# neevparikh/rpt

Hardware: AMD Instinct MI355X
Metric: Msamples/sec (higher is better)
Workload: dtype f32; 1 GPU; C3 lampshade-in-fog path trace 1024x1024x256spp; scene=examples/volumetric_pathtrace_lampshade.rs, parallelism=tile-shard x1, streams=2

## Files before the change

### include/rpt_hip.h

```cpp
#ifndef RPT_HIP_H
#define RPT_HIP_H

#include <stdint.h>

#ifdef __cplusplus
extern "C" {
#endif

#define RPT_OK 0
#define RPT_ERR_INVALID (-1)
#define RPT_ERR_STATE (-2)
#define RPT_ERR_DEVICE (-3)
#define RPT_ERR_UNSUPPORTED (-4)

typedef struct rpt_scene rpt_scene;

enum { RPT_SHAPE_SPHERE = 0, RPT_SHAPE_CUBE = 1, RPT_SHAPE_PLANE = 2, RPT_SHAPE_MESH = 3,
       RPT_SHAPE_GROUP = 4,
       RPT_SHAPE_MONOMIAL = 5  };

typedef struct rpt_shape_desc {
    int32_t kind;
    int32_t has_transform;
    double transform[16];
// ... 59 lines not shown
                            int32_t* object, double* normal);

int rpt_scene_stats(rpt_scene*, uint64_t out[16]);
int rpt_get_counters(rpt_scene*, uint64_t out[8]);
int rpt_debug_section_counters(rpt_scene*, uint64_t out[56]);
int rpt_scan_cull_counters(rpt_scene*, uint64_t out[16]);
int rpt_scan_cull_groups(rpt_scene*, float out_boxes[36], uint64_t out_masks[5], uint32_t* n_groups, uint32_t* enabled);
int rpt_get_timing(rpt_scene*, double* render_ms, double* resolve_ms, int32_t* grid_blocks);
int rpt_get_timing_mean(rpt_scene*, double* render_ms, double* resolve_ms, int32_t* launches);
int rpt_render_chunking(uint32_t iterations, uint32_t* chunk_spp, uint32_t* n_chunks);
int rpt_scene_render_chunking(rpt_scene*, uint32_t iterations, uint32_t* chunk_spp, uint32_t* n_chunks);
int rpt_set_option(const char* name, int64_t value);
int rpt_scene_set_option(rpt_scene*, const char* name, int64_t value);

typedef struct rpt_buffer rpt_buffer;
rpt_buffer* rpt_buffer_create(int device, uint32_t width, uint32_t height, uint32_t filter_radius);
void rpt_buffer_destroy(rpt_buffer*);
int rpt_buffer_add_samples(rpt_buffer*, const double* rgb );
int rpt_buffer_add_samples_device(rpt_buffer*, const void* d_rgb, void* hip_stream);
int rpt_buffer_image(rpt_buffer*, uint8_t* out_rgb8 );
int rpt_buffer_variance(rpt_buffer*, double* out);
int rpt_buffer_batches(rpt_buffer*, uint32_t* n);
int rpt_render_into_buffer(rpt_scene*, const rpt_camera*, const rpt_render_params*, uint32_t iterations,
                           uint64_t seed, uint32_t sample_offset, rpt_buffer*);

enum { RPT_PHOTON_MAP = 0, RPT_PHOTON_POINT_BEAM = 1, RPT_PHOTON_BEAM_BEAM = 2 };
int rpt_photon_map_build(rpt_scene*, uint64_t photon_count, int32_t kind, double watts, uint64_t seed);
#define RPT_PHOTON_RECORD_BYTES 48
int rpt_photon_shoot(rpt_scene*, uint64_t photon_count, int32_t kind, double watts, uint64_t seed,
                     uint32_t shard_rank, uint32_t shard_count, uint64_t n_out[2]);
int rpt_photon_records(rpt_scene*, int32_t which , void** d_records, uint64_t* n);
int rpt_photon_map_from_records(rpt_scene*, uint64_t photon_count, int32_t kind, const void* d_surface,
                                uint64_t n_surface, const void* d_volume, uint64_t n_volume);
int rpt_photon_map_stats(rpt_scene*, uint64_t out[8]);
int rpt_photon_map_download(rpt_scene*, int32_t which, float* out, uint64_t capacity_photons);
int rpt_photon_render_sample(rpt_scene*, const rpt_camera*, const rpt_render_params*, uint64_t gather_size,
                             uint64_t gather_size_volume, uint32_t num_samples, uint64_t seed,
                             uint32_t sample_offset, double* out_rgb);
int rpt_photon_render_sample_device(rpt_scene*, const rpt_camera*, const rpt_render_params*, uint64_t gather_size,
                                    uint64_t gather_size_volume, uint32_t num_samples, uint64_t seed,
                                    uint32_t sample_offset, void* d_out_rgb, void* hip_stream);

typedef struct rpt_comm rpt_comm;
#define RPT_COMM_ID_BYTES 128
int rpt_comm_unique_id(void* id_out);
int rpt_comm_create(const void* id, int rank, int n_ranks, int device, rpt_comm** out);
void rpt_comm_destroy(rpt_comm*);
int rpt_comm_rank(const rpt_comm*, int* rank, int* n_ranks);
#define RPT_GATHER_LOOPBACK 1u
int rpt_gather_frame_device(rpt_comm*, uint32_t width, uint32_t height, const void* d_shard, void* d_frame,
                            uint32_t flags, void* hip_stream);
int rpt_allgather_records_device(rpt_comm*, const void* d_local, uint64_t n_local, void* d_out, uint64_t capacity,
                                 uint64_t* n_per_rank, uint64_t* n_total, void* hip_stream);
int rpt_frame_pack_layout(uint32_t width, uint32_t height, uint32_t n_ranks, uint64_t* tile_offsets);
int rpt_frame_pack_device(uint32_t width, uint32_t height, uint32_t rank, uint32_t n_ranks, const void* d_frame,
                          void* d_packed, void* hip_stream);
int rpt_frame_unpack_device(uint32_t width, uint32_t height, uint32_t rank, uint32_t n_ranks, const void* d_packed,
                            void* d_frame, void* hip_stream);

int rpt_debug_epsilon_counters(rpt_scene*, uint64_t out[12]);

int rpt_debug_rng_u32(uint64_t seed, uint32_t pixel, uint32_t sample, uint32_t n, uint32_t* out);
int rpt_debug_material_sample_f(const rpt_material*, uint64_t n, const float* normals, const float* wos,
                                uint64_t seed, float* wi, float* pdf, int32_t* some);
int rpt_debug_material_bsdf(const rpt_material*, uint64_t n, const float* normals, const float* wos,
                            const float* wis, float* out_rgb);
int rpt_debug_radix_sort(uint64_t n, const uint64_t* keys, uint64_t* keys_out, uint32_t* order_out);
int rpt_debug_exclusive_scan2(uint64_t n, const uint32_t* a, const uint32_t* b, uint32_t* out_a, uint32_t* out_b, uint64_t totals[2]);
int rpt_debug_photon_positions64(rpt_scene*, double* out, uint64_t capacity);
int rpt_debug_photon_selections(rpt_scene*, uint32_t* out, uint64_t capacity_words, uint64_t dims[3]);
int rpt_debug_camera_rays(const rpt_camera*, const rpt_render_params*, uint64_t seed, uint32_t sample,
                          float* origins, float* dirs);
int rpt_debug_camera_sample(const rpt_camera*, const rpt_render_params*, uint64_t seed, uint32_t sample,
                            float* origins, float* dirs, uint32_t* next_word);
int rpt_debug_camera_sample_f64(const rpt_camera*, const rpt_render_params*, uint64_t seed, uint32_t sample,
                                double* origins, double* dirs, uint32_t* next_word);
int rpt_debug_light_sample(rpt_scene*, uint32_t light, uint64_t n, const float* positions, uint64_t seed, float* v, float* nrm,
                           float* pdf, float* intensity, float* wi, float* dist, uint32_t* next_word);
int rpt_debug_light_sample_f64(rpt_scene*, uint32_t light, uint64_t n, const double* positions, uint64_t seed, double* v, double* nrm,
                               double* pdf, double* intensity, double* wi, double* dist, uint32_t* next_word);
int rpt_debug_env_color(rpt_scene*, uint64_t n, const float* dirs, float* rgb);
int rpt_debug_env_color_f64(rpt_scene*, uint64_t n, const double* dirs, double* rgb);
int rpt_debug_medium_distance(rpt_scene*, uint64_t n, uint64_t seed, float* dmed, float* t_limit);

int rpt_debug_bounce(const rpt_material* m, uint32_t max_bounces, uint32_t depth, int32_t in_medium, int32_t medium_event,
                     float albedo_med, const float* medium_color, uint64_t n, const float* normals, const float* rds, uint64_t seed,
                     int32_t* flag, float* wi, float* k, uint32_t* next_word);
int rpt_debug_material_f64(const rpt_material* m, uint64_t n, const double* normals, const double* wos, uint64_t seed, int32_t* some,
                           double* wi, double* pdf, double* f, uint32_t* next_word);
int rpt_debug_material_bsdf_f64(const rpt_material* m, uint64_t n, const double* normals, const double* wos, const double* wis,
                                double* f);
#ifdef __cplusplus
}
#endif
#endif
```

### rpt_amd/_lib.py

```python
import ctypes as C
import os
import sys

_HERE = os.path.dirname(os.path.abspath(__file__))
LIB_PATH = os.environ.get("RPT_LIB", os.path.join(_HERE, "librpt_hip.so"))


class RptError(RuntimeError):
    """Raised for every non-zero return code of the C ABI (message from rpt_last_error)."""


class ShapeDesc(C.Structure):
    pass


ShapeDesc._fields_ = [
    ("kind", C.c_int32),
    ("has_transform", C.c_int32),
    ("transform", C.c_double * 16),
    ("plane_normal", C.c_double * 3),
    ("plane_value", C.c_double),
    ("tris", C.POINTER(C.c_double)),
    ("n_tris", C.c_uint64),
    ("children", C.POINTER(ShapeDesc)),
# ... 40 lines not shown
    ("rpt_device_count", C.c_int, []),
    ("rpt_last_error", C.c_char_p, []),
    ("rpt_shard_tiles", C.c_int64, [C.c_uint32, C.c_uint32, C.c_uint32, C.c_uint32, _P, C.c_uint64]),
    ("rpt_scene_create", _P, []),
    ("rpt_scene_destroy", None, [_P]),
    ("rpt_scene_add_object", C.c_int, [_P, C.POINTER(ShapeDesc), C.POINTER(MaterialDesc)]),
    ("rpt_scene_add_light_point", C.c_int, [_P, _D3, _D3]),
    ("rpt_scene_add_light_ambient", C.c_int, [_P, _D3]),
    ("rpt_scene_add_light_directional", C.c_int, [_P, _D3, _D3]),
    ("rpt_scene_add_light_object", C.c_int, [_P, C.POINTER(ShapeDesc), C.POINTER(MaterialDesc)]),
    ("rpt_scene_add_medium", C.c_int, [_P, C.c_int32, C.c_double, C.c_double]),
    ("rpt_scene_set_environment_color", C.c_int, [_P, _D3]),
    ("rpt_scene_set_environment_hdri", C.c_int, [_P, C.c_uint32, C.c_uint32, _D3]),
    ("rpt_scene_commit", C.c_int, [_P, C.c_int]),
    ("rpt_render_sample", C.c_int,
     [_P, C.POINTER(CameraDesc), C.POINTER(RenderParams), C.c_uint32, C.c_uint64, C.c_uint32, _P]),
    ("rpt_render_sample_device", C.c_int,
     [_P, C.POINTER(CameraDesc), C.POINTER(RenderParams), C.c_uint32, C.c_uint64, C.c_uint32, _P, _P]),
    ("rpt_intersect_batch", C.c_int, [_P, C.c_uint64, _P, _P, _P, _P, _P]),
    ("rpt_intersect_batch_f64", C.c_int, [_P, C.c_uint64, _P, _P, _P, _P, _P]),
    ("rpt_intersect_segments", C.c_int, [_P, C.c_uint64, _P, _P, _P, _P, _P]),
    ("rpt_scan_cull_counters", C.c_int, [_P, C.POINTER(C.c_uint64)]),
    ("rpt_scan_cull_groups", C.c_int, [_P, C.POINTER(C.c_float), C.POINTER(C.c_uint64), C.POINTER(C.c_uint32), C.POINTER(C.c_uint32)]),
    ("rpt_scene_stats", C.c_int, [_P, C.POINTER(C.c_uint64)]),
    ("rpt_get_counters", C.c_int, [_P, C.POINTER(C.c_uint64)]),
    ("rpt_debug_section_counters", C.c_int, [_P, C.POINTER(C.c_uint64)]),
    ("rpt_get_timing", C.c_int, [_P, C.POINTER(C.c_double), C.POINTER(C.c_double), C.POINTER(C.c_int32)]),
    ("rpt_get_timing_mean", C.c_int, [_P, C.POINTER(C.c_double), C.POINTER(C.c_double), C.POINTER(C.c_int32)]),
    ("rpt_render_chunking", C.c_int, [C.c_uint32, C.POINTER(C.c_uint32), C.POINTER(C.c_uint32)]),
    ("rpt_scene_render_chunking", C.c_int, [_P, C.c_uint32, C.POINTER(C.c_uint32), C.POINTER(C.c_uint32)]),
    ("rpt_set_option", C.c_int, [C.c_char_p, C.c_int64]),
    ("rpt_scene_set_option", C.c_int, [_P, C.c_char_p, C.c_int64]),
    ("rpt_buffer_create", _P, [C.c_int, C.c_uint32, C.c_uint32, C.c_uint32]),
    ("rpt_buffer_destroy", None, [_P]),
    ("rpt_buffer_add_samples", C.c_int, [_P, _P]),
    ("rpt_buffer_add_samples_device", C.c_int, [_P, _P, _P]),
    ("rpt_buffer_image", C.c_int, [_P, _P]),
    ("rpt_buffer_variance", C.c_int, [_P, C.POINTER(C.c_double)]),
    ("rpt_buffer_batches", C.c_int, [_P, C.POINTER(C.c_uint32)]),
    ("rpt_render_into_buffer", C.c_int,
     [_P, C.POINTER(CameraDesc), C.POINTER(RenderParams), C.c_uint32, C.c_uint64, C.c_uint32, _P]),
    ("rpt_photon_map_build", C.c_int, [_P, C.c_uint64, C.c_int32, C.c_double, C.c_uint64]),
    ("rpt_photon_shoot", C.c_int,
     [_P, C.c_uint64, C.c_int32, C.c_double, C.c_uint64, C.c_uint32, C.c_uint32, C.POINTER(C.c_uint64)]),
    ("rpt_photon_records", C.c_int, [_P, C.c_int32, C.POINTER(C.c_void_p), C.POINTER(C.c_uint64)]),
    ("rpt_photon_map_from_records", C.c_int, [_P, C.c_uint64, C.c_int32, _P, C.c_uint64, _P, C.c_uint64]),
    ("rpt_photon_map_stats", C.c_int, [_P, C.POINTER(C.c_uint64)]),
    ("rpt_photon_map_download", C.c_int, [_P, C.c_int32, _P, C.c_uint64]),
    ("rpt_photon_render_sample", C.c_int,
     [_P, C.POINTER(CameraDesc), C.POINTER(RenderParams), C.c_uint64, C.c_uint64, C.c_uint32, C.c_uint64, C.c_uint32, _P]),
    ("rpt_photon_render_sample_device", C.c_int,
     [_P, C.POINTER(CameraDesc), C.POINTER(RenderParams), C.c_uint64, C.c_uint64, C.c_uint32, C.c_uint64, C.c_uint32, _P, _P]),
    ("rpt_comm_unique_id", C.c_int, [_P]),
    ("rpt_comm_create", C.c_int, [_P, C.c_int, C.c_int, C.c_int, C.POINTER(C.c_void_p)]),
    ("rpt_comm_destroy", None, [_P]),
    ("rpt_comm_rank", C.c_int, [_P, C.POINTER(C.c_int), C.POINTER(C.c_int)]),
    ("rpt_gather_frame_device", C.c_int, [_P, C.c_uint32, C.c_uint32, _P, _P, C.c_uint32, _P]),
    ("rpt_allgather_records_device", C.c_int, [_P, _P, C.c_uint64, _P, C.c_uint64, C.POINTER(C.c_uint64), C.POINTER(C.c_uint64), _P]),
    ("rpt_frame_pack_layout", C.c_int, [C.c_uint32, C.c_uint32, C.c_uint32, C.POINTER(C.c_uint64)]),
    ("rpt_frame_pack_device", C.c_int, [C.c_uint32, C.c_uint32, C.c_uint32, C.c_uint32, _P, _P, _P]),
    ("rpt_frame_unpack_device", C.c_int, [C.c_uint32, C.c_uint32, C.c_uint32, C.c_uint32, _P, _P, _P]),
    ("rpt_debug_epsilon_counters", C.c_int, [_P, C.POINTER(C.c_uint64)]),
    ("rpt_debug_rng_u32", C.c_int, [C.c_uint64, C.c_uint32, C.c_uint32, C.c_uint32, _P]),
    ("rpt_debug_material_sample_f", C.c_int,
     [C.POINTER(MaterialDesc), C.c_uint64, _P, _P, C.c_uint64, _P, _P, _P]),
    ("rpt_debug_material_bsdf", C.c_int, [C.POINTER(MaterialDesc), C.c_uint64, _P, _P, _P, _P]),
    ("rpt_debug_radix_sort", C.c_int, [C.c_uint64, _P, _P, _P]),
    ("rpt_debug_exclusive_scan2", C.c_int, [C.c_uint64, _P, _P, _P, _P, C.POINTER(C.c_uint64)]),
    ("rpt_debug_photon_positions64", C.c_int, [_P, _P, C.c_uint64]),
    ("rpt_debug_photon_selections", C.c_int, [_P, _P, C.c_uint64, C.POINTER(C.c_uint64)]),
    ("rpt_debug_camera_rays", C.c_int,
     [C.POINTER(CameraDesc), C.POINTER(RenderParams), C.c_uint64, C.c_uint32, _P, _P]),
    ("rpt_debug_light_sample", C.c_int, [_P, C.c_uint32, C.c_uint64, _P, C.c_uint64, _P, _P, _P, _P, _P, _P, _P]),
    ("rpt_debug_light_sample_f64", C.c_int, [_P, C.c_uint32, C.c_uint64, _P, C.c_uint64, _P, _P, _P, _P, _P, _P, _P]),
    ("rpt_debug_env_color", C.c_int, [_P, C.c_uint64, _P, _P]),
    ("rpt_debug_env_color_f64", C.c_int, [_P, C.c_uint64, _P, _P]),
    ("rpt_debug_medium_distance", C.c_int, [_P, C.c_uint64, C.c_uint64, _P, _P]),
    ("rpt_debug_camera_sample", C.c_int,
     [C.POINTER(CameraDesc), C.POINTER(RenderParams), C.c_uint64, C.c_uint32, _P, _P, _P]),
    ("rpt_debug_camera_sample_f64", C.c_int,
     [C.POINTER(CameraDesc), C.POINTER(RenderParams), C.c_uint64, C.c_uint32, _P, _P, _P]),
    ("rpt_debug_bounce", C.c_int, [C.POINTER(MaterialDesc), C.c_uint32, C.c_uint32, C.c_int32, C.c_int32, C.c_float, _P,
                                   C.c_uint64, _P, _P, C.c_uint64, _P, _P, _P, _P]),
    ("rpt_debug_material_f64", C.c_int, [C.POINTER(MaterialDesc), C.c_uint64, _P, _P, C.c_uint64, _P, _P, _P, _P, _P]),
    ("rpt_debug_material_bsdf_f64", C.c_int, [C.POINTER(MaterialDesc), C.c_uint64, _P, _P, _P, _P]),
]

_lib = None


def vp(a):
    return a.ctypes.data_as(C.c_void_p)


def load():
    global _lib
    if _lib is not None:
        return _lib
    if not os.path.exists(LIB_PATH):
        raise RptError(
            f"{LIB_PATH} is missing: build it with `python -c 'import __graft_entry__ as g; g.build()'` "
            "(hipcc --offload-arch=gfx950).  There is no CPU fallback.")
    if "torch" not in sys.modules and os.environ.get("RPT_IMPORT_TORCH", "0") == "1":
        import torch
    lib = C.CDLL(LIB_PATH, mode=C.RTLD_GLOBAL)
    for name, res, args in SYMBOLS:
        fn = getattr(lib, name)
        fn.restype = res
        fn.argtypes = args
    _lib = lib
    return lib


def check(rc):
    if rc < 0:
        msg = load().rpt_last_error()
        raise RptError(f"rpt error {rc}: {msg.decode() if msg else ''}")
    return rc
```

### rpt_amd/api.py

```python
import ctypes as C
import math
import weakref

import numpy as np

from . import _lib
from ._lib import RptError, vp as _vp

def shard_pixels(width, height, rank, count):
    lib = _lib.load()
    n = _lib.check(lib.rpt_shard_tiles(width, height, rank, count, None, 0))
    tiles = np.zeros(max(n, 1), dtype=np.uint32)
    _lib.check(lib.rpt_shard_tiles(width, height, rank, count, tiles.ctypes.data_as(C.c_void_p), n))
    tiles_x = (width + 31) // 32
    ys, xs = np.mgrid[0:32, 0:32]
    out = []
    for t in tiles[:n]:
        x = (int(t) % tiles_x) * 32 + xs
        y = (int(t) // tiles_x) * 32 + ys
        m = (x < width) & (y < height)
        out.append((y[m] * width + x[m]).astype(np.uint32))
    return np.sort(np.concatenate(out)) if out else np.zeros(0, dtype=np.uint32)


# ... 808 lines not shown
            self.gather_size_volume_, int(num_samples), C.c_uint64(self.seed_), self._sample_offset,
            C.c_void_p(d_out_ptr), C.c_void_p(stream_ptr)))
        self._sample_offset += int(num_samples)

    def photon_render(self, photon_count, kind):
        self.photon_map_build(photon_count, kind)
        buffer = Buffer(self.width_, self.height_, self.filter_)
        self._sample_offset = 0
        buffer.add_samples(self.photon_sample_array(self.num_samples_))
        return buffer.image()

    def photon_point_query_beam_render(self, photon_count):
        return self.photon_render(photon_count, Renderer.PHOTON_POINT_BEAM)

    def photon_beam_query_beam_render(self, photon_count):
        return self.photon_render(photon_count, Renderer.PHOTON_BEAM_BEAM)

    def photon_map_render(self, photon_count):
        return self.photon_render(photon_count, Renderer.PHOTON_MAP)

    def counters(self):
        out = (C.c_uint64 * 8)()
        _lib.check(_lib.load().rpt_get_counters(self.scene._handle, out))
        names = ["samples", "rays", "vertices", "wave_trips", "prim_tests", "bvh_nodes", "bvh_tris", "stack_overflows"]
        return dict(zip(names, [int(v) for v in out]))

    def get_closest_hit(self, origins, dirs):
        lib = _lib.load()
        h = self.scene._commit(self.device_)
        o = np.ascontiguousarray(origins, dtype=np.float32).reshape(-1, 3)
        d = np.ascontiguousarray(dirs, dtype=np.float32).reshape(-1, 3)
        n = o.shape[0]
        t = np.empty(n, dtype=np.float32)
        obj = np.empty(n, dtype=np.int32)
        nrm = np.empty((n, 3), dtype=np.float32)
        _lib.check(lib.rpt_intersect_batch(h, n, o.ctypes.data_as(C.c_void_p), d.ctypes.data_as(C.c_void_p),
                                           t.ctypes.data_as(C.c_void_p), obj.ctypes.data_as(C.c_void_p),
                                           nrm.ctypes.data_as(C.c_void_p)))
        return t, obj, nrm

    def get_closest_hit_f64(self, origins, dirs):
        lib = _lib.load()
        h = self.scene._commit(self.device_)
        o = np.ascontiguousarray(origins, dtype=np.float64).reshape(-1, 3)
        d = np.ascontiguousarray(dirs, dtype=np.float64).reshape(-1, 3)
        n = o.shape[0]
        t = np.empty(n, dtype=np.float64)
        obj = np.empty(n, dtype=np.int32)
        nrm = np.empty((n, 3), dtype=np.float64)
        _lib.check(lib.rpt_intersect_batch_f64(h, n, o.ctypes.data_as(C.c_void_p), d.ctypes.data_as(C.c_void_p),
                                               t.ctypes.data_as(C.c_void_p), obj.ctypes.data_as(C.c_void_p),
                                               nrm.ctypes.data_as(C.c_void_p)))
        return t, obj, nrm

    def debug_light_sample(self, light_index, positions, seed=0, f64=False):
        lib = _lib.load()
        h = self.scene._commit(self.device_)
        ft = np.float64 if f64 else np.float32
        pos = np.ascontiguousarray(positions, dtype=ft).reshape(-1, 3)
        n = pos.shape[0]
        out = {"v": np.empty((n, 3), ft), "nrm": np.empty((n, 3), ft), "p": np.empty(n, ft), "intensity": np.empty((n, 3), ft),
               "wi": np.empty((n, 3), ft), "dist": np.empty(n, ft), "next_word": np.empty(n, np.uint32)}
        fn = lib.rpt_debug_light_sample_f64 if f64 else lib.rpt_debug_light_sample
        _lib.check(fn(h, light_index, n, pos.ctypes.data_as(C.c_void_p), seed,
                      *[out[k].ctypes.data_as(C.c_void_p) for k in ("v", "nrm", "p", "intensity", "wi", "dist", "next_word")]))
        return out

    def debug_env_color(self, dirs, f64=False):
        lib = _lib.load()
        h = self.scene._commit(self.device_)
        d = np.ascontiguousarray(dirs, dtype=np.float64 if f64 else np.float32).reshape(-1, 3)
        out = np.empty_like(d)
        fn = lib.rpt_debug_env_color_f64 if f64 else lib.rpt_debug_env_color
        _lib.check(fn(h, d.shape[0], d.ctypes.data_as(C.c_void_p), out.ctypes.data_as(C.c_void_p)))
        return out

    def debug_medium_distance(self, n, seed=0):
        lib = _lib.load()
        h = self.scene._commit(self.device_)
        dmed, lim = np.empty(n, np.float32), np.empty(n, np.float32)
        _lib.check(lib.rpt_debug_medium_distance(h, n, seed, dmed.ctypes.data_as(C.c_void_p), lim.ctypes.data_as(C.c_void_p)))
        return dmed, lim


def debug_bounce(material, normals, rds, max_bounces=3, depth=0, seed=0, in_medium=False, medium_event=False, albedo_med=0.0,
                 medium_color=(0.0, 0.0, 0.0)):
    nrm = np.ascontiguousarray(normals, dtype=np.float32).reshape(-1, 3)
    rd = np.ascontiguousarray(rds, dtype=np.float32).reshape(-1, 3)
    n = nrm.shape[0]
    if rd.shape[0] != n:
        raise ValueError("normals and rds differ in length")
    mcol = np.ascontiguousarray(medium_color, dtype=np.float32).reshape(3)
    out = {"flag": np.empty(n, np.int32), "wi": np.empty((n, 3), np.float32), "k": np.empty((n, 3), np.float32),
           "next_word": np.empty(n, np.uint32)}
    md = material_desc(material, _lib.MaterialDesc)
    _lib.check(_lib.load().rpt_debug_bounce(C.byref(md), max_bounces, depth, int(bool(in_medium)), int(bool(medium_event)),
                                            float(albedo_med), _vp(mcol), n, _vp(nrm), _vp(rd), seed,
                                            *[_vp(out[k]) for k in ("flag", "wi", "k", "next_word")]))
    return out


def debug_material_f64(material, normals, wos, seed=0):
    nrm = np.ascontiguousarray(normals, dtype=np.float64).reshape(-1, 3)
    wo = np.ascontiguousarray(wos, dtype=np.float64).reshape(-1, 3)
    n = nrm.shape[0]
    if wo.shape[0] != n:
        raise ValueError("normals and wos differ in length")
    out = {"some": np.empty(n, np.int32), "wi": np.empty((n, 3)), "pdf": np.empty(n), "f": np.empty((n, 3)),
           "next_word": np.empty(n, np.uint32)}
    md = material_desc(material, _lib.MaterialDesc)
    _lib.check(_lib.load().rpt_debug_material_f64(C.byref(md), n, _vp(nrm), _vp(wo), seed,
                                                  *[_vp(out[k]) for k in ("some", "wi", "pdf", "f", "next_word")]))
    return out


def debug_material_bsdf_f64(material, normals, wos, wis):
    arrs = [np.ascontiguousarray(a, dtype=np.float64).reshape(-1, 3) for a in (normals, wos, wis)]
    n = arrs[0].shape[0]
    if any(a.shape[0] != n for a in arrs):
        raise ValueError("normals, wos and wis differ in length")
    f = np.empty((n, 3))
    md = material_desc(material, _lib.MaterialDesc)
    _lib.check(_lib.load().rpt_debug_material_bsdf_f64(C.byref(md), n, *[_vp(a) for a in arrs], _vp(f)))
    return f


def debug_camera_sample(camera, width, height, sample=0, seed=0, f64=False):
    ft = np.float64 if f64 else np.float32
    n = width * height
    out = {"o": np.empty((n, 3), ft), "d": np.empty((n, 3), ft), "next_word": np.empty(n, np.uint32)}
    prm = _lib.RenderParams(width, height, 0.0, 0, 0, 1)
    lib = _lib.load()
    fn = lib.rpt_debug_camera_sample_f64 if f64 else lib.rpt_debug_camera_sample
    _lib.check(fn(C.byref(camera_desc(camera, _lib.CameraDesc)), C.byref(prm), seed, sample,
                  *[_vp(out[k]) for k in ("o", "d", "next_word")]))
    return out
```

### rpt_amd/csrc/device_core.h

```cpp
#pragma once
#include <hip/hip_runtime.h>
#include "gpu_layout.h"

namespace rptg {

#define RPT_DEV __device__ __forceinline__

static constexpr float kPi = 3.14159265358979323846f;
static constexpr float kInvPi = 0.31830988618379067154f;
static constexpr float kInf = __builtin_huge_valf();

struct V {
    float x, y, z;
};
RPT_DEV V mk(float x, float y, float z) { return V{x, y, z}; }
RPT_DEV V operator+(V a, V b) { return V{a.x + b.x, a.y + b.y, a.z + b.z}; }
RPT_DEV V operator-(V a, V b) { return V{a.x - b.x, a.y - b.y, a.z - b.z}; }
RPT_DEV V operator-(V a) { return V{-a.x, -a.y, -a.z}; }
RPT_DEV V operator*(float s, V a) { return V{s * a.x, s * a.y, s * a.z}; }
RPT_DEV V operator*(V a, float s) { return V{s * a.x, s * a.y, s * a.z}; }
RPT_DEV V operator*(V a, V b) { return V{a.x * b.x, a.y * b.y, a.z * b.z}; }
RPT_DEV float dot(V a, V b) { return fmaf(a.x, b.x, fmaf(a.y, b.y, a.z * b.z)); }
RPT_DEV V cross(V a, V b) {
    return V{a.y * b.z - a.z * b.y, a.z * b.x - a.x * b.z, a.x * b.y - a.y * b.x};
}
RPT_DEV V fma3(float s, V a, V b) { return V{fmaf(s, a.x, b.x), fmaf(s, a.y, b.y), fmaf(s, a.z, b.z)}; }
RPT_DEV V fma3(V s, V a, V b) { return V{fmaf(s.x, a.x, b.x), fmaf(s.y, a.y, b.y), fmaf(s.z, a.z, b.z)}; }
RPT_DEV float rsq(float x) { return __builtin_amdgcn_rsqf(x); }
RPT_DEV float rcp(float x) { return __builtin_amdgcn_rcpf(x); }
RPT_DEV float sqrt1(float x) { return __builtin_amdgcn_sqrtf(x); }
RPT_DEV V normalize(V a) { return rsq(dot(a, a)) * a; }
RPT_DEV V vmin(V a, V b) { return V{fminf(a.x, b.x), fminf(a.y, b.y), fminf(a.z, b.z)}; }
RPT_DEV float max3(float a, float b, float c) { return fmaxf(fmaxf(a, b), c); }
RPT_DEV float min3(float a, float b, float c) { return fminf(fminf(a, b), c); }
RPT_DEV V xyz(const F4& f) { return V{f.x, f.y, f.z}; }
RPT_DEV float dot3w(const F4& r, V p) { return fmaf(r.x, p.x, fmaf(r.y, p.y, fmaf(r.z, p.z, r.w))); }
RPT_DEV float dot3(const F4& r, V p) { return fmaf(r.x, p.x, fmaf(r.y, p.y, r.z * p.z)); }
RPT_DEV bool is_zero(V a) { return a.x == 0.f && a.y == 0.f && a.z == 0.f; }

template <class T>
RPT_DEV T uload(const T* p) {
    static_assert(sizeof(T) % 16 == 0, "scene records are 16-byte multiples");
    typedef uint32_t u4v __attribute__((ext_vector_type(4)));
    typedef const __attribute__((address_space(4))) u4v* CP;
    CP q = (CP)(uintptr_t)p;
    u4v raw[sizeof(T) / 16];
#pragma unroll
    for (unsigned i = 0; i < sizeof(T) / 16; i++) raw[i] = q[i];
    T out;
    __builtin_memcpy(&out, raw, sizeof(T));
    return out;
}

typedef const __attribute__((address_space(4))) SceneView* KernargView;
RPT_DEV KernargView kernarg_scene() {
    KernargView kv = (KernargView)__builtin_amdgcn_kernarg_segment_ptr();
    asm volatile("" : "+s"(kv));
    return kv;
}
template <class T>
RPT_DEV T kernarg_load(const __attribute__((address_space(4))) T* p) {
    static_assert(sizeof(T) % 4 == 0, "kernel-argument structs are dword multiples");
    typedef const __attribute__((address_space(4))) uint32_t* Q;
    Q q = (Q)p;
    uint32_t raw[sizeof(T) / 4];
#pragma unroll
    for (unsigned i = 0; i < sizeof(T) / 4; i++) raw[i] = q[i];
    T out;
    __builtin_memcpy(&out, raw, sizeof(T));
    return out;
}
template <class T>
RPT_DEV const __attribute__((address_space(4))) T* kernarg_args() {
    typedef const __attribute__((address_space(4))) T* P;
    P p = (P)__builtin_amdgcn_kernarg_segment_ptr();
    asm volatile("" : "+s"(p));
    return p;
}

RPT_DEV uint64_t mix64(uint64_t x) {
    x ^= x >> 30;
    x *= 0xBF58476D1CE4E5B9ULL;
    x ^= x >> 27;
    x *= 0x94D049BB133111EBULL;
    x ^= x >> 31;
    return x;
}
struct Rng {
    uint32_t s0, s1, s2, s3;
    RPT_DEV void seed(uint64_t a, uint32_t pixel, uint32_t sample) {
        const uint64_t G = 0x9E3779B97F4A7C15ULL;
        uint64_t z = a ^ ((uint64_t(sample) << 32) | uint64_t(pixel));
        uint64_t r0 = mix64(z + G), r1 = mix64(z + 2 * G);
        s0 = uint32_t(r0);
        s1 = uint32_t(r0 >> 32);
        s2 = uint32_t(r1);
        s3 = uint32_t(r1 >> 32);
    }
    RPT_DEV uint32_t next() {
        uint32_t r = s0 + s3;
        uint32_t t = s1 << 9;
        s2 ^= s0;
        s3 ^= s1;
        s1 ^= s2;
        s0 ^= s3;
        s2 ^= t;
        s3 = __builtin_rotateleft32(s3, 11);
        return r;
    }
    RPT_DEV float uniform() { return float(((next() >> 9) << 1) | 1u) * 0x1p-24f; }
    RPT_DEV float range(float a, float b) { return fmaf(b - a, uniform(), a); }
    RPT_DEV uint32_t index(uint32_t n) { return __umulhi(next(), n); }
    RPT_DEV void unit_disc(float& x, float& y) {
        for (;;) {
            x = range(-1.f, 1.f);
            y = range(-1.f, 1.f);
            if (fmaf(x, x, y * y) <= 1.f) return;
        }
    }
};


RPT_DEV bool sphere_closer(V ol, V dl, float tmin, float tbest, float& t);
RPT_DEV float hit_sphere(V ol, V dl, float tmin) {
    float t;
    return sphere_closer(ol, dl, tmin, __builtin_inff(), t) ? t : -1.f;
}
RPT_DEV bool sphere_closer(V ol, V dl, float tmin, float tbest, float& t) {
#pragma clang fp contract(off)
    float a = dot(dl, dl);
    float inv_a = rcp(a);
    float bb = dot(dl, ol) * inv_a;
    V l = fma3(-bb, dl, ol);
    float sq = sqrt1((1.f - dot(l, l)) * inv_a);
    float t0 = -bb - sq;
    t = (t0 < tmin) ? -bb + sq : t0;
    return t >= tmin && t < tbest;
}
RPT_DEV bool slabs_closer(float x1, float x2, float y1, float y2, float z1, float z2, float tmin, float tbest, float& t) {
#pragma clang fp contract(off)
    const float start = max3(fminf(x1, x2), fminf(y1, y2), fminf(z1, z2));
    const float end = min3(fmaxf(x1, x2), fmaxf(y1, y2), fmaxf(z1, z2));
    t = start < tmin ? end : start;
    return !(start > end) && !(end < tmin) && t < tbest;
}
RPT_DEV bool cube_closer(V ol, V dl, float tmin, float tbest, float& t) {
#pragma clang fp contract(off)
    float ix = rcp(dl.x), iy = rcp(dl.y), iz = rcp(dl.z);
    return slabs_closer((-0.5f - ol.x) * ix, (0.5f - ol.x) * ix, (-0.5f - ol.y) * iy, (0.5f - ol.y) * iy, (-0.5f - ol.z) * iz,
                        (0.5f - ol.z) * iz, tmin, tbest, t);
}
RPT_DEV bool aabb_closer(const F4& lo, const F4& hi, V o, V inv, float tmin, float tbest, float& t) {
#pragma clang fp contract(off)
    return slabs_closer((lo.x - o.x) * inv.x, (hi.x - o.x) * inv.x, (lo.y - o.y) * inv.y, (hi.y - o.y) * inv.y,
                        (lo.z - o.z) * inv.z, (hi.z - o.z) * inv.z, tmin, tbest, t);
}
RPT_DEV float hit_cube(V ol, V dl, float tmin) {
    float t;
    return cube_closer(ol, dl, tmin, __builtin_inff(), t) ? t : -1.f;
}
RPT_DEV float hit_plane(const F4& nv, V o, V d, float tmin) {
    float c = dot3(nv, d);
    if (fabsf(c) < 1e-8f) return -1.f;
    float t = (nv.w - dot3(nv, o)) * rcp(c);
    return (t >= tmin) ? t : -1.f;
}
RPT_DEV float hit_tri(const F4& pn, const F4& A, const F4& B, V o, V d, float tmin, float tmax) {
    float c = dot3(pn, d);
    float t = (pn.w - dot3(pn, o)) * rcp(c);
    V p = fma3(t, d, o);
    float v = dot3w(A, p), w = dot3w(B, p);
    float u = 1.f - v - w;
    bool ok = fabsf(c) >= 1e-8f && t >= tmin && t < tmax && u >= 0.f && v >= 0.f && w >= 0.f;
    return ok ? t : -1.f;
}
RPT_DEV float hit_aabb(const F4& lo, const F4& hi, V o, V inv, float tmin) {
    float t;
    return aabb_closer(lo, hi, o, inv, tmin, __builtin_inff(), t) ? t : -1.f;
}
RPT_DEV float hit_rect(const F4& a, float vmax, float oa, float ia, float ou, float du, float ov, float dv,
                       float tmin, float tmax) {
    float t = (a.x - oa) * ia;
    float pu = fmaf(t, du, ou), pv = fmaf(t, dv, ov);
    bool ok = t >= tmin && t < tmax && pu >= a.y && pu <= a.z && pv >= a.w && pv <= vmax;
    return ok ? t : -1.f;
}
RPT_DEV void hit_shell(const ShellScan& s, V o, V inv, float tmin, float& tbest, uint32_t& code) {
    float x1 = (s.lo.x - o.x) * inv.x, x2 = (s.hi.x - o.x) * inv.x;
    float y1 = (s.lo.y - o.y) * inv.y, y2 = (s.hi.y - o.y) * inv.y;
    float z1 = (s.lo.z - o.z) * inv.z, z2 = (s.hi.z - o.z) * inv.z;
    bool sx = x1 > x2, sy = y1 > y2, sz = z1 > z2;
    float xl = sx ? x2 : x1, xh = sx ? x1 : x2;
    float yl = sy ? y2 : y1, yh = sy ? y1 : y2;
    float zl = sz ? z2 : z1, zh = sz ? z1 : z2;
    float start = max3(xl, yl, zl), end = min3(xh, yh, zh);
    uint32_t in_x = sx ? s.face[1] : s.face[0], out_x = sx ? s.face[0] : s.face[1];
    uint32_t in_y = sy ? s.face[3] : s.face[2], out_y = sy ? s.face[2] : s.face[3];
    uint32_t in_z = sz ? s.face[5] : s.face[4], out_z = sz ? s.face[4] : s.face[5];
    uint32_t c_in = (xl > yl && xl > zl) ? in_x : (yl > zl ? in_y : in_z);
    uint32_t c_out = (xh < yh && xh < zh) ? out_x : (yh < zh ? out_y : out_z);
    bool box = start <= end;
    bool use_in = box && start >= tmin && c_in != CODE_MISS;
    bool use_out = box && end >= tmin && c_out != CODE_MISS;
    float t = use_in ? start : end;
    if ((use_in || use_out) && t < tbest) { tbest = t; code = use_in ? c_in : c_out; }
}
RPT_DEV void to_local(const XfScan& x, V o, V d, V& ol, V& dl) {
    ol = mk(dot3w(x.r0, o), dot3w(x.r1, o), dot3w(x.r2, o));
    dl = mk(dot3(x.r0, d), dot3(x.r1, d), dot3(x.r2, d));
}
RPT_DEV void to_local_y(const XfScan& x, V o, V d, V& ol, V& dl) {
    ol = mk(fmaf(x.r0.x, o.x, fmaf(x.r0.z, o.z, x.r0.w)), fmaf(x.r1.y, o.y, x.r1.w), fmaf(x.r2.x, o.x, fmaf(x.r2.z, o.z, x.r2.w)));
    dl = mk(fmaf(x.r0.x, d.x, x.r0.z * d.z), x.r1.y * d.y, fmaf(x.r2.x, d.x, x.r2.z * d.z));
}
RPT_DEV void aabb_pair_closer(const AabbScan& b0, const AabbScan& b1, uint32_t shared, V o, V inv, float tmin, float& tbest,
                              uint32_t& code, uint32_t i) {
#pragma clang fp contract(off)
    const float x1 = (b0.lo.x - o.x) * inv.x, x2 = (b0.hi.x - o.x) * inv.x;
    const float y1 = (b0.lo.y - o.y) * inv.y, y2 = (b0.hi.y - o.y) * inv.y;
    const float z1 = (b0.lo.z - o.z) * inv.z, z2 = (b0.hi.z - o.z) * inv.z;
    float xl = fminf(x1, x2), xh = fmaxf(x1, x2), yl = fminf(y1, y2), yh = fmaxf(y1, y2), zl = fminf(z1, z2), zh = fmaxf(z1, z2);
    float start = max3(xl, yl, zl), end = min3(xh, yh, zh);
    asm volatile("" : "+v"(start), "+v"(end));
    float t = start < tmin ? end : start;
    if (!(start > end) && !(end < tmin) && t < tbest) { tbest = t; code = (K_AABB << 28) | i; }
    if (!(shared & 1u)) { const float u1 = (b1.lo.x - o.x) * inv.x, u2 = (b1.hi.x - o.x) * inv.x; xl = fminf(u1, u2); xh = fmaxf(u1, u2); }
    if (!(shared & 2u)) { const float u1 = (b1.lo.y - o.y) * inv.y, u2 = (b1.hi.y - o.y) * inv.y; yl = fminf(u1, u2); yh = fmaxf(u1, u2); }
    if (!(shared & 4u)) { const float u1 = (b1.lo.z - o.z) * inv.z, u2 = (b1.hi.z - o.z) * inv.z; zl = fminf(u1, u2); zh = fmaxf(u1, u2); }
    start = max3(xl, yl, zl), end = min3(xh, yh, zh);
    t = start < tmin ? end : start;
    if (!(start > end) && !(end < tmin) && t < tbest) { tbest = t; code = (K_AABB << 28) | (i + 1u); }
}
RPT_DEV bool mono_closer(V ol, V dl, const F4& hb, float tmin, float tbest, float& t) {
#pragma clang fp contract(off)
    const float ix = rcp(dl.x), iy = rcp(dl.y), iz = rcp(dl.z);
    const float x1 = (-1.f - ol.x) * ix, x2 = (1.f - ol.x) * ix;
    const float y1 = (hb.y - ol.y) * iy, y2 = (hb.z - ol.y) * iy;
    const float z1 = (-1.f - ol.z) * iz, z2 = (1.f - ol.z) * iz;
    const float b_min = max3(fminf(x1, x2), fminf(y1, y2), fminf(z1, z2));
    const float b_max = min3(fmaxf(x1, x2), fmaxf(y1, y2), fmaxf(z1, z2));
    const bool in_box = !(fmaxf(b_min, tmin) > fminf(b_max, tbest));
    if (__ballot(in_box) == 0ull) return false;
    if (!in_box) return false;
    const float h = hb.x;
    auto dist = [&](float s) {
        const float x = fmaf(s, dl.x, ol.x), y = fmaf(s, dl.y, ol.y), z = fmaf(s, dl.z, ol.z);
        const float r2 = fmaf(x, x, z * z);
        return fmaf(-h, r2 * r2, y);
    };
    const float c0 = fmaf(ol.x, ol.x, ol.z * ol.z), c1 = 2.f * fmaf(ol.x, dl.x, ol.z * dl.z), c2 = fmaf(dl.x, dl.x, dl.z * dl.z);
    const float A = 2.f * c0 * c1, B = 2.f * fmaf(c1, c1, 2.f * c0 * c2), Cq = 6.f * c1 * c2, Dq = 4.f * c2 * c2;
    const float d_tmin = dist(tmin);
    const bool maximize = d_tmin < 0.f;
    float t_max = 10000.f;
    if (maximize) {
        float cur = 0.5f * (b_min + b_max);
        for (int k = 0; k < 10; k++) {
            if (dist(cur) > 0.f) break;
            const float der = fmaf(-h, fmaf(cur, fmaf(cur, fmaf(cur, Dq, Cq), B), A), dl.y);
            const float der2 = -h * fmaf(cur, fmaf(cur, 3.f * Dq, 2.f * Cq), B);
            cur -= der / der2;
        }
        t_max = cur;
        if (t_max < tmin) return false;
    }
    if (maximize == (dist(t_max) < 0.f)) return false;
    float l = tmin, r = t_max;
    for (int k = 0; k < 60; k++) {
        const float m = (l + r) * 0.5f;
        if ((dist(m) >= 0.f) == maximize) r = m;
        else l = m;
    }
    if (r > tbest || !(fabsf(r) < __builtin_huge_valf())) return false;
    const float px = fmaf(r, dl.x, ol.x), pz = fmaf(r, dl.z, ol.z);
    if (fmaf(px, px, pz * pz) > 1.f) return false;
    t = r;
    return true;
}

RPT_DEV void slab2(const float lo[3], const float hi[3], V o, V inv, float& tn, float& tf) {
    float x1 = (lo[0] - o.x) * inv.x, x2 = (hi[0] - o.x) * inv.x;
    float y1 = (lo[1] - o.y) * inv.y, y2 = (hi[1] - o.y) * inv.y;
    float z1 = (lo[2] - o.z) * inv.z, z2 = (hi[2] - o.z) * inv.z;
    tn = max3(fminf(x1, x2), fminf(y1, y2), fminf(z1, z2));
    tf = min3(fmaxf(x1, x2), fmaxf(y1, y2), fmaxf(z1, z2));
}
struct AnyHit {
    float t_block;
    uint32_t tw_lo, tw_hi;
    RPT_DEV bool blocks(float t, uint32_t code) const { return t < t_block && !(code >= tw_lo && code <= tw_hi); }
};
template <bool COUNT, bool PRIMS, bool ANY = false, bool MONO = false>
RPT_DEV void bvh_traverse(const SceneView& sc, uint32_t root, V o, V d, float tmin, float& tbest, uint32_t& code,
                          uint32_t& inst, uint32_t* stk, uint32_t stride, uint32_t cap, uint32_t& c_nodes,
                          uint32_t& c_tris, AnyHit any = AnyHit{-kInf, 1u, 0u});

template <bool COUNT, bool MONO = false>
RPT_DEV void hit_prim(const SceneView& scene_, uint32_t pc, V o, V d, V inv, float tmin, float& tbest, uint32_t& code,
                      uint32_t& inst, uint32_t* stk, uint32_t stride, uint32_t cap, uint32_t& c_nodes,
                      uint32_t& c_tris) {
    const auto& sc = *kernarg_scene();
    const uint32_t kind = pc >> 28, i = pc & 0x0FFFFFFFu;
    float t = -1.f;
    if (MONO && kind == K_MONO) {
        const MonoScan m = sc.mono[i];
        V ol, dl;
        to_local(XfScan{m.r0, m.r1, m.r2}, o, d, ol, dl);
        if (mono_closer(ol, dl, m.h, tmin, tbest, t)) { tbest = t; code = pc; }
        return;
    }
    if (kind == K_INST) {
        const InstRec r = sc.inst[i];
        const V ol = mk(dot3w(r.r0, o), dot3w(r.r1, o), dot3w(r.r2, o));
        const V dl = mk(dot3(r.r0, d), dot3(r.r1, d), dot3(r.r2, d));
// ... 27 lines not shown
        t = hit_tri(tr.pn, tr.A, tr.B, o, d, tmin, tbest);
    }
    if (t >= 0.f && t < tbest) { tbest = t; code = pc; }
}

template <bool COUNT, bool PRIMS, bool ANY, bool MONO>
RPT_DEV void bvh_traverse(const SceneView& scene_, uint32_t root, V o, V d, float tmin, float& tbest, uint32_t& code,
                          uint32_t& inst, uint32_t* stk, uint32_t stride, uint32_t cap, uint32_t& c_nodes,
                          uint32_t& c_tris, AnyHit any) {
    const auto& sc = *kernarg_scene();
    const BvhNode* nodes = sc.nodes;
    const V inv = mk(rcp(d.x), rcp(d.y), rcp(d.z));
    const uint32_t kDone = 0xFFFFFFFFu;
    uint32_t sp = 0;
    uint32_t cur = root;
    while (cur != kDone) {
        while (!(cur & BVH_LEAF)) {
            const BvhNode nd = nodes[cur];
            if (COUNT) c_nodes++;
            float n0, f0, n1, f1;
            slab2(nd.lo0, nd.hi0, o, inv, n0, f0);
            slab2(nd.lo1, nd.hi1, o, inv, n1, f1);
            const bool h0 = fmaxf(n0, tmin) <= fminf(f0, tbest);
            const bool h1 = fmaxf(n1, tmin) <= fminf(f1, tbest);
            if (h0 && h1) {
                const bool first0 = n0 <= n1;
                if (sp < cap) { stk[sp * stride] = first0 ? nd.e1 : nd.e0; sp++; }
                else if (COUNT && sc.stack_overflows) atomicAdd(sc.stack_overflows, 1ull);
                cur = first0 ? nd.e0 : nd.e1;
            } else if (h0 || h1) {
                cur = h0 ? nd.e0 : nd.e1;
            } else if (sp) {
                sp--;
                cur = stk[sp * stride];
            } else {
                cur = kDone;
            }
        }
        if (cur != kDone) {
            const uint32_t first = cur & BVH_INDEX_MASK;
            const uint32_t count = ((cur >> 26) & 31u) + 1u;
            if (PRIMS && (cur & BVH_PRIMS)) {
                for (uint32_t i = 0; i < count; i++) {
                    if (COUNT) c_tris++;
                    hit_prim<COUNT, MONO>(scene_, sc.pleaf[first + i], o, d, inv, tmin, tbest, code, inst, stk + sp * stride, stride,
                                    cap - sp, c_nodes, c_tris);
                }
            } else {
                for (uint32_t i = 0; i < count; i++) {
                    const TriScan tr = sc.btri[first + i];
                    if (COUNT) c_tris++;
                    float t = hit_tri(tr.pn, tr.A, tr.B, o, d, tmin, tbest);
                    if (t >= 0.f) { tbest = t; code = (K_BVHTRI << 28) | (first + i); }
                }
            }
            if (ANY && code != CODE_MISS && any.blocks(tbest, code)) sp = 0;
            if (sp) {
                sp--;
                cur = stk[sp * stride];
            } else {
                cur = kDone;
            }
        }
    }
}

template <bool SHELL>
RPT_DEV bool interval_meets_box(const SceneView::ScanBox& b, V o, V inv, float tmin, float tbest) {
#pragma clang fp contract(off)
    const float x1 = (b.lo[0] - o.x) * inv.x, x2 = (b.hi[0] - o.x) * inv.x;
    const float y1 = (b.lo[1] - o.y) * inv.y, y2 = (b.hi[1] - o.y) * inv.y;
    const float z1 = (b.lo[2] - o.z) * inv.z, z2 = (b.hi[2] - o.z) * inv.z;
    float start, end;
    if (SHELL) {
        const bool sx = x1 > x2, sy = y1 > y2, sz = z1 > z2;
        start = max3(sx ? x2 : x1, sy ? y2 : y1, sz ? z2 : z1);
        end = min3(sx ? x1 : x2, sy ? y1 : y2, sz ? z1 : z2);
    } else {
        start = max3(fminf(x1, x2), fminf(y1, y2), fminf(z1, z2));
        end = min3(fmaxf(x1, x2), fmaxf(y1, y2), fmaxf(z1, z2));
    }
    return !(fmaxf(start, tmin) > fminf(end, tbest));
}
template <bool MASKED = false, bool MONO = false, bool TAIL = false>
RPT_DEV void scan_prims(const SceneView& scene, V o, V d, float tmin, float& tbest, uint32_t& code, uint64_t mask = ~0ull,
                        bool* tail_skipped = nullptr) {
    static_assert(!(TAIL && MASKED), "one cull at a time");
    const auto& sc = *kernarg_scene();
    (void)scene;
    uint32_t bit = 0;
    auto on = [&](uint32_t i) { return !MASKED || ((mask >> ((bit + i) & 63u)) & 1ull) != 0ull; };
    const uint64_t sph_yrot = MASKED ? 0ull : sc.sph_yrot, cub_yrot = MASKED ? 0ull : sc.cub_yrot;
    for (uint32_t i = 0; i < sc.n_sph; i++) {
        if (!on(i)) continue;
        const XfScan x = uload(&sc.sph[i]);
        V ol, dl;
        if (!MASKED && ((sph_yrot >> (i & 63u)) & 1ull)) to_local_y(x, o, d, ol, dl);
        else to_local(x, o, d, ol, dl);
        float t;
        if (sphere_closer(ol, dl, tmin, tbest, t)) { tbest = t; code = (K_SPHERE << 28) | i; }
    }
    bit += sc.n_sph;
    {
        uint32_t i = 0;
        if (!MASKED)
            for (; i + 1u < sc.n_cub; i += 2u) {
                const XfScan x0 = uload(&sc.cub[i]), x1 = uload(&sc.cub[i + 1u]);
                V ol0, dl0, ol1, dl1;
                float t0, t1;
                if (((cub_yrot >> (i & 63u)) & 3ull) == 3ull) {
                    to_local_y(x0, o, d, ol0, dl0);
                    to_local_y(x1, o, d, ol1, dl1);
                } else {
                    to_local(x0, o, d, ol0, dl0);
                    to_local(x1, o, d, ol1, dl1);
                }
                if (cube_closer(ol0, dl0, tmin, tbest, t0)) { tbest = t0; code = (K_CUBE << 28) | i; }
                if (cube_closer(ol1, dl1, tmin, tbest, t1)) { tbest = t1; code = (K_CUBE << 28) | (i + 1u); }
            }
        for (; i < sc.n_cub; i++) {
            if (!on(i)) continue;
            const XfScan x = uload(&sc.cub[i]);
            V ol, dl;
            if (!MASKED && ((cub_yrot >> (i & 63u)) & 1ull)) to_local_y(x, o, d, ol, dl);
            else to_local(x, o, d, ol, dl);
            float t;
            if (cube_closer(ol, dl, tmin, tbest, t)) { tbest = t; code = (K_CUBE << 28) | i; }
        }
    }
    bit += sc.n_cub;
    for (uint32_t i = 0; i < sc.n_pln; i++) {
        const F4 nv = uload(&sc.pln[i]).nv;
        float t = hit_plane(nv, o, d, tmin);
        if (t >= 0.f && t < tbest) { tbest = t; code = (K_PLANE << 28) | i; }
    }
    const uint32_t n_rect = sc.n_rect_x + sc.n_rect_y + sc.n_rect_z;
    if (sc.n_aabb + n_rect + sc.has_shell != 0) {
        const V inv = mk(rcp(d.x), rcp(d.y), rcp(d.z));
        if (sc.has_shell) hit_shell(uload(sc.shell), o, inv, tmin, tbest, code);
        if constexpr (TAIL) {
            if (sc.scan_cull) {
                const SceneView::ScanBox tb = kernarg_load(&sc.scan_tail);
                if (__ballot(interval_meets_box<false>(tb, o, inv, tmin, tbest)) == 0ull) {
                    if (tail_skipped) *tail_skipped = true;
                    return;
                }
            }
        }
        {
            uint32_t i = 0;
            if (!MASKED)
                for (; i + 1u < sc.n_aabb; i += 2u) {
                    const AabbScan b0 = uload(&sc.aabb[i]), b1 = uload(&sc.aabb[i + 1u]);
                    aabb_pair_closer(b0, b1, __float_as_uint(b0.hi.w), o, inv, tmin, tbest, code, i);
                }
            for (; i < sc.n_aabb; i++) {
                if (!on(i)) continue;
                const AabbScan b = uload(&sc.aabb[i]);
                float t;
                if (aabb_closer(b.lo, b.hi, o, inv, tmin, tbest, t)) { tbest = t; code = (K_AABB << 28) | i; }
            }
        }
        bit += sc.n_aabb;
        uint32_t i = 0;
        for (uint32_t e = sc.n_rect_x; i < e; i++) {
            if (!on(i)) continue;
            const RectScan r = uload(&sc.rect[i]);
            float t = hit_rect(r.a, r.b.x, o.x, inv.x, o.y, d.y, o.z, d.z, tmin, tbest);
            if (t >= 0.f) { tbest = t; code = (K_RECT << 28) | i; }
        }
        for (uint32_t e = sc.n_rect_x + sc.n_rect_y; i < e; i++) {
            if (!on(i)) continue;
            const RectScan r = uload(&sc.rect[i]);
            float t = hit_rect(r.a, r.b.x, o.y, inv.y, o.z, d.z, o.x, d.x, tmin, tbest);
            if (t >= 0.f) { tbest = t; code = (K_RECT << 28) | i; }
        }
        for (uint32_t e = n_rect; i < e; i++) {
            if (!on(i)) continue;
            const RectScan r = uload(&sc.rect[i]);
            float t = hit_rect(r.a, r.b.x, o.z, inv.z, o.x, d.x, o.y, d.y, tmin, tbest);
            if (t >= 0.f) { tbest = t; code = (K_RECT << 28) | i; }
        }
        bit += n_rect;
    } else {
        bit += sc.n_aabb + n_rect;
    }
    for (uint32_t i = 0; i < sc.n_tri; i++) {
        if (!on(i)) continue;
        const TriScan tr = uload(&sc.tri[i]);
        float t = hit_tri(tr.pn, tr.A, tr.B, o, d, tmin, tbest);
        if (t >= 0.f) { tbest = t; code = (K_TRI << 28) | i; }
    }
    if constexpr (MONO) {
        static_assert(!MASKED && !TAIL, "scan_mask_for_ball and the tail cull do not cover the monomial surfaces");
        for (uint32_t i = 0; i < sc.n_mono; i++) {
            const MonoScan m = uload(&sc.mono[i]);
            V ol, dl;
            to_local(XfScan{m.r0, m.r1, m.r2}, o, d, ol, dl);
            float t;
            if (mono_closer(ol, dl, m.h, tmin, tbest, t)) { tbest = t; code = (K_MONO << 28) | i; }
        }
    }
}
RPT_DEV uint64_t scan_mask_for_ball(const SceneView& scene_, bool live, V c, float r, bool* touched = nullptr) {
    const auto& sc = *kernarg_scene();
    const uint32_t n = sc.n_sph + sc.n_cub + sc.n_aabb + sc.n_rect_x + sc.n_rect_y + sc.n_rect_z + sc.n_tri;
    if (touched) *touched = n != 0u;
    if (n > 64u) return ~0ull;
    bool mine = false;
    const float r2 = r * r;
    uint64_t mask = 0ull;
    auto reaches = [&](const AabbScan& b) {
        const float dx = fmaxf(fmaxf(b.lo.x - c.x, c.x - b.hi.x), 0.f);
        const float dy = fmaxf(fmaxf(b.lo.y - c.y, c.y - b.hi.y), 0.f);
        const float dz = fmaxf(fmaxf(b.lo.z - c.z, c.z - b.hi.z), 0.f);
        const bool t = live && fmaf(dx, dx, fmaf(dy, dy, dz * dz)) <= r2;
        mine = mine || t;
        return __any(t);
    };
    uint32_t i = 0;
    for (; i + 4u <= n; i += 4u) {
        const AabbScan b0 = uload(&sc.pbox[i]), b1 = uload(&sc.pbox[i + 1u]), b2 = uload(&sc.pbox[i + 2u]), b3 = uload(&sc.pbox[i + 3u]);
        if (reaches(b0)) mask |= 1ull << i;
        if (reaches(b1)) mask |= 2ull << i;
        if (reaches(b2)) mask |= 4ull << i;
        if (reaches(b3)) mask |= 8ull << i;
    }
    for (; i < n; i++)
        if (reaches(uload(&sc.pbox[i]))) mask |= 1ull << i;
    if (touched) *touched = mine;
    return mask;
}
template <bool COUNT>
RPT_DEV void scan_primary(const SceneView& scene, V o, V d, float tmin, float& tbest, uint32_t& code, unsigned long long* cnt) {
    if constexpr (COUNT) {
        const auto& sc = *kernarg_scene();
        const SceneView::ScanBox bound = kernarg_load(&sc.scan_bound);
        const bool first = cnt && uint32_t(__builtin_ctzll(__ballot(true))) == (threadIdx.x & 63u);
        if (!(bound.lo[0] > bound.hi[0])) {
            const V inv = mk(rcp(d.x), rcp(d.y), rcp(d.z));
            const bool need = interval_meets_box<true>(bound, o, inv, tmin, tbest);
            const uint32_t n_need = uint32_t(__popcll(__ballot(need)));
            if (first) atomicAdd(&cnt[n_need == 0u ? 0 : n_need <= 2u ? 1 : n_need <= 4u ? 2 : n_need <= 8u ? 3 : 4], 1ull);
            if (n_need != 0u)
                for (uint32_t g = 0; g < sc.n_scan_groups; g++) {
                    const SceneView::ScanGroup grp = kernarg_load(&sc.scan_groups[g]);
                    const bool reach = need && interval_meets_box<false>(grp.box, o, inv, tmin, tbest);
                    if (__ballot(reach) == 0ull && first) atomicAdd(&cnt[5u + g], 1ull);
                }
        }
        bool skipped = false;
        scan_prims<false, false, true>(scene, o, d, tmin, tbest, code, ~0ull, &skipped);
        if (skipped && first) atomicAdd(&cnt[9], 1ull);
    } else {
        scan_prims<false, false, true>(scene, o, d, tmin, tbest, code);
    }
}

RPT_DEV bool mesh_roots_hit(const SceneView& scene_, V o, V d, float tmin, float tbest) {
    const auto& sc = *kernarg_scene();
    const V inv = mk(rcp(d.x), rcp(d.y), rcp(d.z));
    bool need = false;
    for (uint32_t i = 0; i < sc.n_mesh; i++) {
        const MeshRef m = uload(&sc.meshes[i]);
        const BvhNode nd = uload(&sc.nodes[m.root]);
        float n0, f0, n1, f1;
        slab2(nd.lo0, nd.hi0, o, inv, n0, f0);
        slab2(nd.lo1, nd.hi1, o, inv, n1, f1);
        need = need || fmaxf(n0, tmin) <= fminf(f0, tbest) || fmaxf(n1, tmin) <= fminf(f1, tbest);
    }
    return need;
}
template <bool COUNT, bool ANY>
RPT_DEV void walk_meshes(const SceneView& scene_, V o, V d, float tmin, float& tbest, uint32_t& code, uint32_t& inst,
                         uint32_t* stk, uint32_t stride, uint32_t& c_nodes, uint32_t& c_tris, AnyHit any, uint32_t cap = 32u) {
    const auto& sc = *kernarg_scene();
    for (uint32_t i = 0; i < sc.n_mesh; i++) {
        const MeshRef m = uload(&sc.meshes[i]);
        if (ANY && code != CODE_MISS && any.blocks(tbest, code)) break;
        bvh_traverse<COUNT, false, ANY>(scene_, m.root, o, d, tmin, tbest, code, inst, stk, stride, cap, c_nodes, c_tris, any);
    }
}
static const uint32_t kWalkDone = 0xFFFFFFFFu;
struct WalkState {
    uint32_t cur, sp, mesh;
// ... 225 lines not shown
RPT_DEV V mat_color(const Mat& m) { return (m.kind <= 1u) ? m.albedo : mk(0.f, 0.f, 0.f); }
RPT_DEV float mat_emit(const Mat& m) { return (m.kind <= 1u) ? m.emit : 0.f; }

RPT_DEV V rotate_from_y(V b, V v, bool pi_fallback_x) {
    float s2 = fmaf(b.x, b.x, b.z * b.z);
    if (s2 > 0x1p-104f) {
        float is = rsq(s2);
        float s = s2 * is;
        float kx = b.z * is, kz = -b.x * is;
        float kv = kx * v.x + kz * v.z;
        V kxv = mk(-kz * v.y, kz * v.x - kx * v.z, kx * v.y);
        float c = b.y;
        float omc = 1.f - c;
        return mk(fmaf(c, v.x, fmaf(s, kxv.x, omc * kv * kx)), fmaf(c, v.y, s * kxv.y),
                  fmaf(c, v.z, fmaf(s, kxv.z, omc * kv * kz)));
    }
    if (b.y < 0.f && pi_fallback_x) return mk(v.x, -v.y, -v.z);
    return v;
}
RPT_DEV V reflect_neg(V w, V n) { return fma3(2.f * dot(n, w), n, -w); }

RPT_DEV bool sample_f(const Mat& m, V n, V wo, Rng& rng, V& wi, float& pdf) {
    if (m.kind == M_LAMBERTIAN) {
        float r1 = rng.uniform(), r2 = rng.uniform();
        float ct = sqrt1(r2);
        float st = sqrt1(1.f - r2);
        pdf = ct * kInvPi;
        V dir = mk(st * __builtin_amdgcn_cosf(r1), ct, st * __builtin_amdgcn_sinf(r1));
        wi = normalize(rotate_from_y(n, dir, true));
        return true;
    } else if (m.kind == M_PHONG) {
        float r1 = rng.uniform(), r2 = rng.uniform();
        float ct = __powf(r2, rcp(m.shin + 1.f));
        float st = sqrt1(fmaxf(1.f - ct * ct, 0.f));
        pdf = (m.shin + 1.f) * (0.5f * kInvPi) * __powf(ct, m.shin);
        V dir = mk(st * __builtin_amdgcn_cosf(r1), ct, st * __builtin_amdgcn_sinf(r1));
        V refl = reflect_neg(wo, n);
        wi = normalize(rotate_from_y(normalize(refl), dir, false));
        return true;
    } else if (m.kind == M_MIRROR) {
        wi = reflect_neg(wo, normalize(n));
        pdf = 1.f;
        return true;
    } else {
        bool inside = dot(n, wo) < 0.f;
        V nn = inside ? -n : n;
        float ci = fminf(fmaxf(dot(wo, nn), 0.f), 1.f);
        float ni = inside ? m.ior : 1.f, nt = inside ? 1.f : m.ior;
        float r0 = (ni - nt) * rcp(ni + nt);
        r0 *= r0;
        float mm = 1.f - ci;
        float m2 = mm * mm;
        float sr = fminf(fmaxf(fmaf(1.f - r0, m2 * m2 * mm, r0), 0.f), 1.f);
        pdf = 1.f;
        if (rng.uniform() < sr) {
            wi = reflect_neg(wo, n);
            return true;
        }
        float eta = ni * rcp(nt);
        float k = 1.f - eta * eta * (1.f - ci * ci);
        if (k < 0.f) return false;
        float cost = sqrt1(k);
        wi = fma3(eta * ci - cost, nn, -eta * wo);
        return true;
    }
}
RPT_DEV V bsdf(const Mat& m, V n, V wo, V wi) {
    float nwi = dot(n, wi), nwo = dot(n, wo);
    if (__builtin_signbit(nwi) || __builtin_signbit(nwo)) return mk(0.f, 0.f, 0.f);
    if (m.kind == M_LAMBERTIAN) return kInvPi * m.albedo;
    if (m.kind == M_PHONG) {
        V r = -normalize(fma3(-2.f * dot(n, wi), n, wi));
        float c = fminf(fmaxf(dot(r, wo), 0.f), 1.f);
        float shin = m.shin;
        asm volatile("" : "+v"(shin));
        float pw = (c > 0.f) ? __powf(c, shin) : (shin == 0.f ? 1.f : 0.f);
        return ((shin + 2.f) * (0.5f * kInvPi) * pw) * m.albedo;
    }
    return mk(1.f, 1.f, 1.f);
}

template <bool UNIFORM> struct LightXfRows;
template <> struct LightXfRows<true> {
    LightXf x;
    RPT_DEV explicit LightXfRows(const LightXf* p) : x(uload(p)) {}
    RPT_DEV F4 fwd(int r) const { return x.fwd[r]; }
    RPT_DEV F4 inv(int r) const { return x.inv[r]; }
    RPT_DEV F4 nrm(int r) const { return x.nrm[r]; }
    RPT_DEV F4 lin(int r) const { return x.lin[r]; }
};
template <> struct LightXfRows<false> {
    const LightXf* p;
    RPT_DEV explicit LightXfRows(const LightXf* q) : p(q) {}
    RPT_DEV F4 fwd(int r) const { return p->fwd[r]; }
    RPT_DEV F4 inv(int r) const { return p->inv[r]; }
    RPT_DEV F4 nrm(int r) const { return p->nrm[r]; }
    RPT_DEV F4 lin(int r) const { return p->lin[r]; }
};
template <bool UNIFORM>
RPT_DEV void sample_light_leaf(const SceneView& scene_, uint32_t shape, uint32_t first, uint32_t count, const LightXf* xp,
                               V pos, Rng& rng, V& v, V& n, float& p, const LdsTables& tab = LdsTables{}) {
    const auto& sc = *kernarg_scene();
    V vl, nl;
    const LightXfRows<UNIFORM> x(xp);
    const bool xf = x.nrm(1).w != 0.f;
    const bool mesh = shape == LS_MESH;
    if (mesh) {
        uint32_t idx = rng.index(count);
        LightTri tr;
        if (first + idx < tab.n_ltris) {
            const F4* q = tab.ltris + 6u * (first + idx);
            tr.v1 = q[0]; tr.v2 = q[1]; tr.v3 = q[2]; tr.n1 = q[3]; tr.n2 = q[4]; tr.n3 = q[5];
        } else {
            tr = sc.ltris[first + idx];
        }
        uint32_t ku = rng.next() >> 9, kv = rng.next() >> 9;
        while (ku + kv >= (1u << 23)) {
            ku = rng.next() >> 9;
            kv = rng.next() >> 9;
        }
        const float u = float((ku << 1) | 1u) * 0x1p-24f, vv = float((kv << 1) | 1u) * 0x1p-24f;
        float w = 1.f - u - vv;
        vl = u * xyz(tr.v1) + vv * xyz(tr.v2) + w * xyz(tr.v3);
        nl = normalize(u * xyz(tr.n1) + vv * xyz(tr.n2) + w * xyz(tr.n3));
        p = tr.v1.w * rcp(float(count));
    } else if (shape == LS_SPHERE) {
        V tl = xf ? mk(dot3w(x.inv(0), pos), dot3w(x.inv(1), pos), dot3w(x.inv(2), pos)) : pos;
        float dx, dy;
        rng.unit_disc(dx, dy);
        float z = sqrt1(fmaxf(1.f - dx * dx - dy * dy, 0.f));
        V nn = normalize(tl);
        bool normal_x = fabsf(nn.x) >= 1.17549435e-38f && fabsf(nn.x) < kInf;
        V n1 = normal_x ? normalize(mk(nn.y, -nn.x, 0.f)) : normalize(mk(0.f, -nn.z, nn.y));
        V n2 = cross(n1, nn);
        vl = dx * n1 + dy * n2 + z * nn;
        nl = vl;
        p = z * kInvPi;
    } else {
        float a = rng.uniform() - 0.5f, b = rng.uniform() - 0.5f;
        uint32_t f = rng.index(6);
        switch (f) {
            case 0: vl = mk(a, b, 0.5f); nl = mk(0, 0, 1); break;
            case 1: vl = mk(a, b, -0.5f); nl = mk(0, 0, -1); break;
            case 2: vl = mk(a, 0.5f, b); nl = mk(0, 1, 0); break;
            case 3: vl = mk(a, -0.5f, b); nl = mk(0, -1, 0); break;
            case 4: vl = mk(0.5f, a, b); nl = mk(1, 0, 0); break;
            default: vl = mk(-0.5f, a, b); nl = mk(-1, 0, 0); break;
        }
        p = 1.f / 6.f;
    }
    if (xf) {
        n = normalize(mk(dot3(x.nrm(0), nl), dot3(x.nrm(1), nl), dot3(x.nrm(2), nl)));
        V ln = mk(dot3(x.lin(0), nl), dot3(x.lin(1), nl), dot3(x.lin(2), nl));
        float height = dot(ln, n);
        float base = x.nrm(0).w * rcp(height);
        v = mesh ? vl : mk(dot3w(x.fwd(0), vl), dot3w(x.fwd(1), vl), dot3w(x.fwd(2), vl));
        p = p * rcp(base);
    } else {
        v = vl;
        n = nl;
    }
}
template <bool GROUPS>
RPT_DEV void sample_light_shape(const SceneView& scene_, const Light& L, V pos, Rng& rng, V& v, V& n, float& p,
                                const LdsTables& tab = LdsTables{}) {
    const auto& sc = *kernarg_scene();
    if (!GROUPS || L.shape != LS_GROUP) {
        sample_light_leaf<true>(scene_, L.shape, L.first, L.count, &sc.lxf[L.xf], pos, rng, v, n, p, tab);
        return;
    }
    uint32_t shape = LS_GROUP, first = L.first, count = L.count, xfi = 0;
    float pick = 1.f;
    while (shape == LS_GROUP) {
        const uint32_t idx = rng.index(count);
        pick *= rcp(float(count));
        const LightPart part = sc.lparts[first + idx];
        shape = part.shape; first = part.first; count = part.count; xfi = part.xf;
    }
    sample_light_leaf<false>(scene_, shape, first, count, &sc.lxf[xfi], pos, rng, v, n, p, tab);
    p *= pick;
}
template <bool GROUPS>
RPT_DEV void illuminate_object(const SceneView& sc, const Light& L, V pos, Rng& rng, V& intensity, V& wi,
                               float& dist, const LdsTables& tab = LdsTables{}) {
    V v, n;
    float p;
    sample_light_shape<GROUPS>(sc, L, pos, rng, v, n, p, tab);
    V disp = v - pos;
    float len2 = dot(disp, disp);
    float ilen = rsq(len2);
    float cosine = fmaxf(-dot(disp, n), 0.f) * ilen;
    float surface_area = cosine * rcp(len2);
    intensity = (surface_area * rcp(p)) * xyz(L.color);
    wi = ilen * disp;
    dist = len2 * ilen;
}

RPT_DEV V env_color(const SceneView& scene_, V dir) {
    const auto& sc = *kernarg_scene();
    if (sc.hdri_w == 0) return mk(sc.env[0], sc.env[1], sc.env[2]);
    const V d = normalize(dir);
    const float azimuth = atan2f(d.z, d.x) + kPi;
    const float polar = acosf(fminf(fmaxf(d.y, -1.f), 1.f));
    const float x = azimuth * (0.5f * kInvPi) * float(sc.hdri_w - 1u);
    const float y = polar * kInvPi * float(sc.hdri_h - 1u);
    const uint32_t x0 = min(uint32_t(x), sc.hdri_w - 1u), y0 = min(uint32_t(y), sc.hdri_h - 1u);
    const float ax = x - float(x0), ay = y - float(y0);
    const uint32_t x1 = min(x0 + 1u, sc.hdri_w - 1u), y1 = min(y0 + 1u, sc.hdri_h - 1u);
    const V c00 = xyz(sc.hdri[y0 * sc.hdri_w + x0]), c01 = xyz(sc.hdri[y0 * sc.hdri_w + x1]);
    const V c10 = xyz(sc.hdri[y1 * sc.hdri_w + x0]), c11 = xyz(sc.hdri[y1 * sc.hdri_w + x1]);
    const V top = (1.f - ax) * c00 + ax * c01, bot = (1.f - ax) * c10 + ax * c11;
    return (1.f - ay) * top + ay * bot;
}

RPT_DEV float pixel_xn(uint32_t x, uint32_t w, float inv_dim) { return (float(2u * x + 1u) - float(w)) * inv_dim; }
RPT_DEV float pixel_yn(uint32_t y, uint32_t h, float inv_dim) { return (float(2u * (h - y) - 1u) - float(h)) * inv_dim; }
RPT_DEV void cast_ray(const CameraG& c, float x, float y, Rng& rng, V& o, V& d) {
    V right = mk(c.right[0], c.right[1], c.right[2]), up = mk(c.up[0], c.up[1], c.up[2]);
    o = mk(c.eye[0], c.eye[1], c.eye[2]);
    V nd = mk(c.ddir[0], c.ddir[1], c.ddir[2]) + x * right + y * up;
    if (c.aperture > 0.f) {
        V focal = fma3(c.focal_distance, normalize(nd), o);
        float dx, dy;
        rng.unit_disc(dx, dy);
        o = o + c.aperture * (dx * right + dy * up);
        nd = focal - o;
    }
    d = normalize(nd);
}

}
```

### rpt_amd/csrc/kernels.h

```cpp
#pragma once
#include <hip/hip_runtime_api.h>
#include <stddef.h>
#include <stdint.h>
#include "gpu_layout.h"

namespace rptg {

struct RenderArgs {
    SceneView sc;
    CameraG cam;
    uint32_t width, height;
    float inv_dim;
    uint32_t max_bounces;
    uint32_t iterations;
    uint32_t sample_offset;
    uint32_t chunk_spp;
    uint32_t n_chunks;
    uint64_t seed_mixed;
    const uint32_t* tiles;
    uint32_t n_tiles, tiles_x;
    uint32_t n_owned;
    uint32_t n_items;
    float* slab;
    float* slab2;
    unsigned long long* queue;
    unsigned long long* counters;
    uint32_t lds_stack;
    uint32_t defer_lanes;
    uint32_t defer_stop;
    uint32_t walk_leaf_quarters;
    uint32_t detach;
    uint32_t pull_batch;
    uint32_t detach_trigger;
    uint32_t stream_backlog;
    uint32_t stream_contexts;
    uint32_t n_twin_lights;
    uint32_t* stream_scratch;
};

static_assert(offsetof(RenderArgs, sc) == 0, "RenderArgs must begin with the SceneView");

struct KernelInfo {
    int vgprs, sgprs, lds, max_blocks_per_cu;
};

hipError_t launch_render(const RenderArgs& a, int n_blocks, hipStream_t stream);
hipError_t render_occupancy(bool medium, int bvh, int* blocks_per_cu, int detach = 0);
size_t stream_scratch_bytes_per_block();
int bvh_mode(const SceneView& sc);
hipError_t launch_buffer_add(uint32_t n_pixels, const double* d_batch, double* d_sum, double* d_sumsq, hipStream_t st);
hipError_t launch_buffer_image(uint32_t w, uint32_t h, uint32_t radius, uint32_t n_batches, const double* d_sum, uint8_t* d_out,
                               hipStream_t st);
hipError_t launch_buffer_variance(uint32_t n_pixels, uint32_t n_batches, const double* d_sum, const double* d_sumsq, double* d_out,
                                  hipStream_t st);
hipError_t launch_resolve(const RenderArgs& a, double scale, double* d_out, hipStream_t stream);
hipError_t launch_frame_pack(const double* d_frame, double* d_packed, const uint32_t* d_tiles, uint32_t n_tiles, uint32_t tiles_x,
                             uint32_t width, uint32_t height, hipStream_t st);
hipError_t launch_frame_unpack(const double* d_packed, double* d_frame, const uint32_t* d_tiles, uint32_t n_tiles, uint32_t tiles_x,
                               uint32_t width, uint32_t height, hipStream_t st);
__attribute__((weak)) hipError_t launch_intersect_segments(const SceneView& sc, uint64_t n, const float* d_o, const float* d_d, const float* d_tmax,
                                                           float* d_t, uint32_t* d_code, hipStream_t stream);
hipError_t launch_intersect(const SceneView& sc, uint64_t n, const float* d_o, const float* d_d, float* d_t,
                            int32_t* d_obj, float* d_n, bool bvh, hipStream_t stream);
hipError_t launch_debug_rng(uint64_t seed_mixed, uint32_t pixel, uint32_t sample, uint32_t n, uint32_t* d_out,
                            hipStream_t stream);
hipError_t launch_debug_sample_f(const Material& m, uint64_t n, const float* d_n, const float* d_wo,
                                 uint64_t seed_mixed, float* d_wi, float* d_pdf, int32_t* d_some, hipStream_t s);
hipError_t launch_debug_bsdf(const Material& m, uint64_t n, const float* d_n, const float* d_wo, const float* d_wi,
                             float* d_out, hipStream_t s);
__attribute__((weak)) hipError_t launch_debug_camera_sample(const CameraG& cam, uint32_t w, uint32_t h, float inv_dim, uint64_t seed_mixed,
                                                            uint32_t sample, float* d_o, float* d_d, uint32_t* d_next_word ,
                                                            hipStream_t s);
struct LightSampleArgs {
    uint32_t light;
    uint32_t pad_;
    uint64_t n;
    uint64_t seed_mixed;
    const float* pos;
    float *v, *nrm, *pdf;
    float *intensity, *wi, *dist;
    uint32_t* next_word;
};
__attribute__((weak)) hipError_t launch_debug_light_sample(const SceneView& sc, const LightSampleArgs& q, hipStream_t s);
__attribute__((weak)) hipError_t launch_debug_env_color(const SceneView& sc, uint64_t n, const float* d_dirs, float* d_rgb, hipStream_t s);
__attribute__((weak)) hipError_t launch_debug_medium_distance(const SceneView& sc, uint64_t n, uint64_t seed_mixed, float* d_dmed,
                                                              float* d_limit, hipStream_t s);
struct BounceArgs {
    Material m;
    uint32_t max_bounces, depth;
    uint32_t in_medium;
    uint32_t medium_event;
    float albedo_med;
    float mcol[3];
    uint64_t n;
    uint64_t seed_mixed;
    const float *nrm, *rd;
    int32_t* flag;
    float *wi, *k;
    uint32_t* next_word;
};
__attribute__((weak)) hipError_t launch_debug_bounce(const BounceArgs& q, hipStream_t s);

}
namespace rpt64 { struct Args; struct ShootArgs64; struct SurfArgs64; }
namespace rptg {
hipError_t launch_render_f64(const rpt64::Args& a, int n_blocks, hipStream_t stream);
hipError_t launch_resolve_f64(const rpt64::Args& a, double scale, double* d_out, hipStream_t stream);
hipError_t render_f64_occupancy(bool medium, int* blocks_per_cu);
hipError_t launch_photon_shoot_f64(const rpt64::ShootArgs64& a, int n_blocks, hipStream_t stream);
hipError_t launch_photon_surface_f64(const rpt64::SurfArgs64& a, int n_blocks, hipStream_t stream);
hipError_t launch_resolve_photon_f64(const rpt64::Args& a, const void* slab32, uint32_t n_chunks32, double scale_over_total, bool accumulate,
                                     double* d_out, hipStream_t stream);
}
```

### rpt_amd/csrc/kernels.hip

```cpp
#include "device_core.h"
#include "kernels.h"

namespace rptg {

RPT_DEV uint32_t mbcnt64(uint64_t m) {
    return __builtin_amdgcn_mbcnt_hi(uint32_t(m >> 32), __builtin_amdgcn_mbcnt_lo(uint32_t(m), 0u));
}
template <bool MONO = false>
RPT_DEV uint32_t code_object(const SceneView& sc, uint32_t code, uint32_t inst) {
    uint32_t kind = code >> 28, idx = code & 0x0FFFFFFFu;
    float w;
    if (MONO && kind == K_MONO) w = sc.mono_sh[idx].r0.w;
    else if (kind == K_INSTTRI) w = sc.inst[inst].n0.w;
    else if (kind == K_SPHERE) w = sc.sph_sh[idx].r0.w;
    else if (kind == K_CUBE) w = sc.cub_sh[idx].r0.w;
    else if (kind == K_PLANE) w = sc.pln_sh[idx].unit_n_obj.w;
    else if (kind == K_TRI) w = sc.tri_sh[idx].n1.w;
    else if (kind == K_AABB) w = sc.aabb[idx].lo.w;
    else if (kind == K_RECT) w = sc.rect_sh[idx].n_obj.w;
    else w = sc.btri_sh[idx].n1.w;
    return __float_as_uint(w);
}
RPT_DEV float ray_tmin(V o) { return 2e-5f * (1.f + max3(fabsf(o.x), fabsf(o.y), fabsf(o.z))); }

// ... 10 lines not shown
#endif
#ifndef RPT_MIN_WAVES_MESH
#define RPT_MIN_WAVES_MESH 4
#endif
#ifndef RPT_MIN_WAVES_SCENE_MESH
#define RPT_MIN_WAVES_SCENE_MESH 3
#endif
#ifndef RPT_MIN_WAVES_STREAM
#define RPT_MIN_WAVES_STREAM 4
#endif
#ifndef RPT_MIN_WAVES_SCAN
#define RPT_MIN_WAVES_SCAN 6
#endif
#ifndef RPT_MIN_WAVES_SCAN_GROUPS
#define RPT_MIN_WAVES_SCAN_GROUPS 5
#endif
static constexpr uint32_t kDetachStackRows = 20u;
static constexpr uint32_t kQCap = 32u;
static constexpr uint32_t kQFields = 11u;
static constexpr uint32_t kQWaveDwords = 16u + kQFields * kQCap;
static_assert(kQCap == 32u, "one mask bit per slot");
static constexpr uint32_t kTabDwords = (2u * 32u + 6u * 8u) * 4u;
static constexpr uint32_t kDetachPendBase = (kDetachStackRows + 5u) * 256u + kTabDwords;
static constexpr uint32_t kDetachAccBase = kDetachPendBase + 256u;
static constexpr uint32_t kDetachQBase = kDetachAccBase + 3u * 256u * 2u;
static constexpr uint32_t kDetachDwords = kDetachQBase + 4u * kQWaveDwords;
static_assert(kDetachAccBase % 2u == 0u, "the 64-bit accumulators are 8-byte aligned");
#ifndef RPT_STREAM_RING
#define RPT_STREAM_RING 512
#endif
static constexpr uint32_t kRingEntries = RPT_STREAM_RING;
static constexpr uint32_t kRingDwords = 12u;
static constexpr uint32_t kCtxMax = 6u;
static constexpr uint32_t kCtxFields = 20u;
static constexpr uint32_t kWaveScratchDwords = kRingEntries * kRingDwords + kCtxMax * kCtxFields * 64u;
typedef float f4v __attribute__((ext_vector_type(4)));
typedef uint32_t u4v __attribute__((ext_vector_type(4)));
static_assert(kDetachDwords * 4u * 4u <= 160u * 1024u, "four blocks per CU");
RPT_DEV unsigned long long to_fixed(float v) {
    v = fminf(fmaxf(v, 0.f), 4294967040.f);
    const uint32_t hi = uint32_t(v);
    const uint32_t lo = uint32_t((v - float(hi)) * 4294967296.f);
    return ((unsigned long long)hi << 32) | lo;
}
RPT_DEV float from_fixed(unsigned long long x) { return float(double(x) * 0x1p-32); }

static constexpr uint32_t kCullCounters = 64u;
#ifdef RPT_MARKERS
#define RPT_MARK(k) asm volatile("; SECT " #k ::: "memory")
#else
#define RPT_MARK(k)
#endif
#ifdef RPT_SECT_CLOCKS
#define SECT(k) do { } while (0)
#else
#define SECT(k)                                                                                  \
    do {                                                                                         \
        RPT_MARK(k);                                                                             \
        if (COUNT) {                                                                             \
            const uint64_t m_ = __ballot(true);                                                  \
            if (mbcnt64(m_) == 0) {                                                              \
                atomicAdd(&a.counters[8 + 2 * (k)], 1ull);                                       \
                atomicAdd(&a.counters[9 + 2 * (k)], (unsigned long long)__popcll(m_));           \
            }                                                                                    \
        }                                                                                        \
    } while (0)
#endif
#ifdef RPT_SECT_CLOCKS
#define SECTK(k)                                                                                 \
    do {                                                                                         \
        if (COUNT) {                                                                             \
            const uint64_t now_ = __builtin_amdgcn_s_memtime();                                  \
            if (mbcnt64(__ballot(true)) == 0) {                                                  \
                sect_lds_[threadIdx.x >> 6][2 * (k)] += 1ull;                                    \
                sect_lds_[threadIdx.x >> 6][2 * sect_prev_ + 1] += now_ - sect_clk_;             \
            }                                                                                    \
            sect_prev_ = (k);                                                                    \
            sect_clk_ = now_;                                                                    \
        }                                                                                        \
    } while (0)
#else
#define SECTK(k) SECT(k)
#endif
template <bool MEDIUM>
RPT_DEV void stage_distance(Rng& rng, float inv_sigma_t, float& dmed, float& t) {
    dmed = kInf;
    if (MEDIUM) {
        float xi = rng.range(0.f, 1.f);
        dmed = -__logf(xi) * inv_sigma_t;
    }
    t = (MEDIUM && dmed < 400.f) ? dmed * (1.f + 1e-6f) : kInf;
}
template <bool COUNT, bool MONO = false>
RPT_DEV void stage_event(const RenderArgs& a, const LdsTables& tab, V ro, V rd, uint32_t depth, bool medium, float dmed, float t,
                         uint32_t code, uint32_t inst, V& x, V& n, V& mcol, Mat& mat, V& E) {
    const SceneView& sc = a.sc;
    if (medium) {
        SECT(5);
        x = fma3(dmed, rd, ro);
        bool hi = sc.medium_kind == 1u && x.y > 250.f;
        mcol = hi ? mk(sc.medium_color_hi[0], sc.medium_color_hi[1], sc.medium_color_hi[2])
                  : mk(sc.medium_color[0], sc.medium_color[1], sc.medium_color[2]);
        E = (depth == 0) ? sc.medium_emission * mcol : mk(0, 0, 0);
    } else {
        uint32_t obj;
        SECT(6);
        finalize_hit<MONO>(sc, ro, rd, ray_tmin(ro), t, code, inst, n, obj);
        mat = load_mat(sc, obj, tab);
        x = fma3(t, rd, ro);
        E = (depth == 0) ? mat_emit(mat) * mat_color(mat) : mk(0, 0, 0);
    }
}
template <bool MONO = false>
RPT_DEV void stage_light_term(const SceneView& sc, const Light& L, float albedo_med, V rd, bool medium, float ts, uint32_t cs,
                              uint32_t is, float dist, V I, V wi, V n, V mcol, const Mat& mat, V& E) {
    const bool twin = (L.twin_lo <= L.twin_hi) ? (cs >= L.twin_lo && cs <= L.twin_hi)
                                               : (cs != CODE_MISS && code_object<MONO>(sc, cs, is) == uint32_t(L.twin_object));
    if (cs != CODE_MISS && ts >= dist * (1.f - 1e-3f) && twin) {
        if (medium) {
            E = fma3(albedo_med * sc.medium_phase, I * mcol, E);
        } else {
            V f = bsdf(mat, n, -normalize(rd), wi);
            E = fma3(dot(wi, n), f * I, E);
        }
    }
}
template <bool MEDIUM, bool COUNT>
RPT_DEV bool stage_bounce(const RenderArgs& a, float albedo_med, V rd, uint32_t depth, bool medium, V n, V mcol, const Mat& mat,
                          Rng& rng, V& wi, V& k) {
    bool bounce;
    SECT(10);
    if (medium) {
        SECT(11);
        bounce = rng.uniform() < 0.8f;
        if (bounce) {
            float ax = rng.range(-1.f, 1.f), ay = rng.range(-1.f, 1.f), az = rng.range(-1.f, 1.f);
            wi = normalize(mk(ax, ay, az));
            k = (albedo_med * 1.25f) * mcol;
        }
    } else {
        SECT(12);
        bounce = MEDIUM ? (rng.uniform() < 0.8f) : (depth < a.max_bounces);
        if (bounce) {
            float pdf;
            SECT(13);
            const V wo = -normalize(rd);
            bounce = sample_f(mat, n, wo, rng, wi, pdf);
            if (bounce) {
                V f = bsdf(mat, n, wo, wi);
                float wgt = fabsf(dot(wi, n)) * rcp(MEDIUM ? pdf * 0.8f : pdf);
                k = wgt * f;
            }
        }
    }
    return bounce && !is_zero(k);
}

template <bool MEDIUM, int BVH, bool COUNT, bool GROUPS = false, int DETACH = 0, bool MONO = false>
__global__ __launch_bounds__(256, BVH == 0 ? ((GROUPS || COUNT || MONO) ? RPT_MIN_WAVES_SCAN_GROUPS : RPT_MIN_WAVES_SCAN) : BVH == 3 ? RPT_MIN_WAVES_SCENE_MESH : BVH == 1 ? (DETACH == 2 ? RPT_MIN_WAVES_STREAM : RPT_MIN_WAVES_MESH) : RPT_MIN_WAVES)
void render_kernel(const RenderArgs a) {
#ifdef RPT_SECT_CLOCKS
    __shared__ unsigned long long sect_lds_[4][56];
    if ((threadIdx.x & 63u) < 56u) sect_lds_[threadIdx.x >> 6][threadIdx.x & 63u] = 0ull;
    uint64_t sect_clk_ = __builtin_amdgcn_s_memtime();
    uint32_t sect_prev_ = 27u;
#endif
    static_assert(DETACH == 0 || (MEDIUM && BVH == 1 && !GROUPS), "detached tree walks: per-mesh-tree kernels in a medium only");
    static_assert(DETACH == 0 || !MONO, "no detached tree walks in scenes with monomial surfaces");
    extern __shared__ uint32_t dyn_lds[];
    const SceneView& sc = a.sc;
    uint32_t* stk = BVH ? (dyn_lds + threadIdx.x) : nullptr;
    const uint32_t stride = 256;

    const float sigma_t = sc.sigma_a + sc.sigma_s;
    const float inv_sigma_t = MEDIUM ? 1.f / sigma_t : 0.f;
    const float albedo_med = MEDIUM ? sc.sigma_s / sigma_t : 0.f;

    Rng rng;
    rng.s0 = rng.s1 = rng.s2 = rng.s3 = 0;
    V ro = mk(0, 0, 0), rd = mk(0, 0, 1);
    V P = mk(0, 0, 0), Q = mk(1, 1, 1), Rc = mk(kInf, kInf, kInf);
    constexpr uint32_t kStackRows = BVH == 1 ? (DETACH ? kDetachStackRows : 21u) : 32u;
    constexpr uint32_t kStateBase = BVH ? kStackRows * 256u : 0u;
    uint32_t* const ls = dyn_lds + kStateBase + threadIdx.x;
    enum { S_SLAB = 0, S_END = 1, S_PIX = 2, S_XN = 3, S_YN = 4, S_S = 5, S_ACC = 6, S_P = 9, S_Q = 12, S_RC = 15, S_ROWS = 18 };
    static_assert(S_RC + 3 == S_ROWS, "the staged tables begin right behind the state rows");
    constexpr uint32_t kTabBase = kStateBase + (BVH == 0 ? uint32_t(S_ROWS) : 5u) * 256u;
    LdsTables tab;
    {
        const F4* const t4 = reinterpret_cast<const F4*>(dyn_lds + kTabBase);
        F4* const w4 = reinterpret_cast<F4*>(dyn_lds + kTabBase);
        const uint32_t nm = sc.n_obj <= kLdsMats ? sc.n_obj : 0u, nl = sc.n_ltris <= kLdsLtris ? sc.n_ltris : 0u;
        for (uint32_t i = threadIdx.x; i < 2u * nm; i += 256u) w4[i] = reinterpret_cast<const F4*>(sc.mats)[i];
        for (uint32_t i = threadIdx.x; i < 6u * nl; i += 256u) w4[2u * kLdsMats + i] = reinterpret_cast<const F4*>(sc.ltris)[i];
        __syncthreads();
        tab.mats = t4; tab.n_mats = nm;
        tab.ltris = t4 + 2u * kLdsMats; tab.n_ltris = nl;
    }
    auto in_lds = [](int k) { return BVH == 0 || k <= S_YN; };
    V acc_r = mk(0, 0, 0);
    uint32_t slab_idx_r = 0, s_r = 0, s_end_r = 0, pix_r = 0;
    float xn_r = 0.f, yn_r = 0.f;
    auto ldu = [&](int k, uint32_t reg) { return in_lds(k) ? ls[k * 256] : reg; };
    auto ldf = [&](int k, float reg) { return in_lds(k) ? __uint_as_float(ls[k * 256]) : reg; };
    auto stu = [&](int k, uint32_t& reg, uint32_t v) { if (in_lds(k)) ls[k * 256] = v; else reg = v; };
    auto stf = [&](int k, float& reg, float v) { if (in_lds(k)) ls[k * 256] = __float_as_uint(v); else reg = v; };
    volatile uint32_t* const ls_pend = dyn_lds + (DETACH ? kDetachPendBase : 0u);
    unsigned long long* const acc64 = reinterpret_cast<unsigned long long*>(dyn_lds + (DETACH ? kDetachAccBase : 0u));
// ... 788 lines not shown
                    acc_add(vmin(P, Rc));
                    need_path = true;
                }
                phase = PH_NEW;
            }
            const bool waiting = alive && phase >= PH_WAITP;
            const uint64_t wm = __ballot(waiting);
            const bool idle = __ballot(alive && !waiting && !(need_path && item_done)) == 0;
            if (wm != 0 && (uint32_t(__popcll(wm)) >= a.defer_lanes || idle)) {
                if (COUNT) c_wave[0] = c_wave[1] = 0;
                if (waiting) {
                    SECTK(15);
                    const bool shadow = phase == PH_WAITS;
                    const V qo = shadow ? v_x : ro, qd = shadow ? v_wi : rd;
                    AnyHit any{-kInf, 1u, 0u};
                    if (shadow) {
                        const uint32_t lo = sc.lights[v_li].twin_lo, hi = sc.lights[v_li].twin_hi;
                        any = AnyHit{lo <= hi ? v_dist * (1.f - 1e-3f) : -kInf, lo, hi};
                    }
                    walk_meshes_resumable<COUNT>(sc, qo, qd, ray_tmin(qo), q_t, q_code, stk, stride, walk,
                                                 idle ? 1u : a.defer_stop, any, c_nodes, c_btris, kStackRows, a.walk_leaf_quarters, c_wave);
                    if (walk.cur == kWalkDone) {
                        phase = shadow ? PH_HAVES : PH_HAVEP;
                        SECTK(16);
                        if ((q_code >> 28) == K_BVHTRI) { SECTK(17); }
                        if (shadow) { SECTK(18); }
                    }
                }
                if (COUNT) {
                    for (int k = 0; k < 2; k++) {
                        uint32_t v = c_wave[k];
                        for (int off = 32; off; off >>= 1) v = max(v, uint32_t(__shfl_xor(int(v), off)));
                        w_tot[k] += v;
                    }
                }
            }
            continue;
        }
        if (!alive || need_path) continue;

        if (COUNT) c_vertices++;
        SECTK(2);
        float dmed, t;
        stage_distance<MEDIUM>(rng, inv_sigma_t, dmed, t);
        const float tmin = ray_tmin(ro);
        uint32_t code = CODE_MISS, inst = 0;
        if constexpr (MEDIUM && BVH == 0 && !MONO)
            scan_primary<COUNT>(sc, ro, rd, tmin, t, code, COUNT ? a.counters + kCullCounters : nullptr);
        else
            closest_hit<BVH, COUNT, false, MONO>(sc, ro, rd, tmin, t, code, inst, stk, stride, c_nodes, c_btris);
        if (COUNT) c_rays++;
        SECTK(3);
        const bool hit = code != CODE_MISS;

        const bool ev_medium = MEDIUM && (dmed < (hit ? t : 400.f));
        const bool ev_surface = !ev_medium && hit;
        if (!ev_medium && !ev_surface) {
            SECTK(4);
            if constexpr (BVH == 0) {
                const V v = fma3(ldv(S_Q, Q), env_color(sc, rd), ldv(S_P, P));
                acc_add(MEDIUM ? v : vmin(v, ldv(S_RC, Rc)));
            } else {
                acc_add(vmin(fma3(Q, env_color(sc, rd), P), Rc));
            }
            need_path = true;
            continue;
        }

        V x, n = mk(0, 1, 0), mcol = mk(0, 0, 0), E;
        Mat mat = Mat{mk(0, 0, 0), 0.f, 0u, 0.f, 0.f};
        stage_event<COUNT, MONO>(a, tab, ro, rd, depth, ev_medium, dmed, t, code, inst, x, n, mcol, mat, E);

        for (uint32_t li = 0; li < sc.n_lights; li++) {
            const Light L = uload(&sc.lights[li]);
            if (L.kind == L_AMBIENT) {
                E = fma3(xyz(L.color), ev_medium ? mcol : mat_color(mat), E);
            } else if (L.kind == L_OBJECT) {
                V I, wi;
                float dist;
                SECTK(7);
                illuminate_object<GROUPS>(sc, L, x, rng, I, wi, dist, tab);
                if (L.twin_object >= 0) {
                    SECTK(8);
                    float ts = dist * (1.f + 1e-3f);
                    uint32_t cs = CODE_MISS, is = 0;
                    const bool range = L.twin_lo <= L.twin_hi;
                    closest_hit<BVH, COUNT, BVH != 0, MONO>(sc, x, wi, ray_tmin(x), ts, cs, is, stk, stride, c_nodes, c_btris,
                                                     AnyHit{range ? dist * (1.f - 1e-3f) : -kInf, L.twin_lo, L.twin_hi});
                    if (COUNT) c_rays++;
                    SECTK(9);
                    stage_light_term<MONO>(sc, L, albedo_med, rd, ev_medium, ts, cs, is, dist, I, wi, n, mcol, mat, E);
                }
            }
        }

        V wi = mk(0, 0, 1), k = mk(0, 0, 0);
        const bool cont = stage_bounce<MEDIUM, COUNT>(a, albedo_med, rd, depth, ev_medium, n, mcol, mat, rng, wi, k);
        SECTK(14);
        if constexpr (BVH == 0) {
            const V q = ldv(S_Q, Q);
            const V pn = fma3(q, E, ldv(S_P, P));
            if (cont) {
                stv(S_P, P, pn);
                if (!MEDIUM) stv(S_RC, Rc, vmin(ldv(S_RC, Rc), fma3(100.f, q, pn)));
                stv(S_Q, Q, q * k);
                ro = x;
                rd = wi;
                depth++;
            } else {
                acc_add(MEDIUM ? pn : vmin(pn, ldv(S_RC, Rc)));
                need_path = true;
            }
        } else {
            P = fma3(Q, E, P);
            if (cont) {
                if (!MEDIUM) Rc = vmin(Rc, fma3(100.f, Q, P));
                Q = Q * k;
                ro = x;
                rd = wi;
                depth++;
            } else {
                acc_add(vmin(P, Rc));
                need_path = true;
            }
        }
    }

    if (COUNT) {
#ifdef RPT_SECT_CLOCKS
        if ((threadIdx.x & 63u) < 56u) atomicAdd(&a.counters[8 + (threadIdx.x & 63u)], sect_lds_[threadIdx.x >> 6][threadIdx.x & 63u]);
#endif
        atomicAdd(&a.counters[0], (unsigned long long)c_samples);
        atomicAdd(&a.counters[1], (unsigned long long)c_rays);
        atomicAdd(&a.counters[2], (unsigned long long)c_vertices);
        if ((threadIdx.x & 63u) == 0) atomicAdd(&a.counters[3], (unsigned long long)c_trips);
        if ((threadIdx.x & 63u) == 0) { atomicAdd(&a.counters[46], (unsigned long long)w_tot[0]); atomicAdd(&a.counters[47], (unsigned long long)w_tot[1]); }
        atomicAdd(&a.counters[5], (unsigned long long)c_nodes);
        if (c_nodes_primary) atomicAdd(&a.counters[61], (unsigned long long)c_nodes_primary);
        atomicAdd(&a.counters[6], (unsigned long long)c_btris);
    }
}

__global__ __launch_bounds__(256) void resolve_kernel(const RenderArgs a, double scale, double* __restrict__ out) {
    uint32_t p = blockIdx.x * 256u + threadIdx.x;
    if (p >= a.n_owned) return;
    uint32_t x, y;
    item_pixel(a, p, x, y);
    if (x >= a.width || y >= a.height) return;
    double r = 0.0, g = 0.0, b = 0.0;
    const float4* slab = reinterpret_cast<const float4*>(a.slab);
    for (uint32_t c = 0; c < a.n_chunks; c++) {
        float4 v = slab[size_t(c) * a.n_owned + p];
        r += double(v.x);
        g += double(v.y);
        b += double(v.z);
        if (a.slab2) {
            const float4 w = reinterpret_cast<const float4*>(a.slab2)[size_t(c) * a.n_owned + p];
            r += double(w.x);
            g += double(w.y);
            b += double(w.z);
        }
    }
    size_t o = (size_t(y) * a.width + x) * 3;
    double inv = scale / double(a.iterations);
    out[o] = r * inv;
    out[o + 1] = g * inv;
    out[o + 2] = b * inv;
}

__global__ __launch_bounds__(256) void buffer_add_kernel(uint32_t n_pixels, const double* __restrict__ batch,
                                                         double* __restrict__ sum, double* __restrict__ sumsq) {
    uint32_t p = blockIdx.x * 256u + threadIdx.x;
    if (p >= n_pixels) return;
    double r = batch[3 * size_t(p)], g = batch[3 * size_t(p) + 1], b = batch[3 * size_t(p) + 2];
// ... 104 lines not shown
    r.seed(seed_mixed, uint32_t(i), 0);
    V w = mk(0, 0, 0);
    float p = 0.f;
    bool ok = sample_f(mat_from(m), mk(nrm[3 * i], nrm[3 * i + 1], nrm[3 * i + 2]),
                       mk(wo[3 * i], wo[3 * i + 1], wo[3 * i + 2]), r, w, p);
    wi[3 * i] = w.x; wi[3 * i + 1] = w.y; wi[3 * i + 2] = w.z;
    pdf[i] = p;
    some[i] = ok ? 1 : 0;
}
__global__ void debug_bsdf_kernel(const Material m, uint64_t n, const float* nrm, const float* wo, const float* wi,
                                  float* out) {
    uint64_t i = uint64_t(blockIdx.x) * blockDim.x + threadIdx.x;
    if (i >= n) return;
    V f = bsdf(mat_from(m), mk(nrm[3 * i], nrm[3 * i + 1], nrm[3 * i + 2]), mk(wo[3 * i], wo[3 * i + 1], wo[3 * i + 2]),
               mk(wi[3 * i], wi[3 * i + 1], wi[3 * i + 2]));
    out[3 * i] = f.x; out[3 * i + 1] = f.y; out[3 * i + 2] = f.z;
}
__global__ void debug_camera_kernel(const CameraG cam, uint32_t w, uint32_t h, float inv_dim, uint64_t seed_mixed, uint32_t sample,
                                    float* o, float* d, uint32_t* next_word) {
    uint32_t i = blockIdx.x * blockDim.x + threadIdx.x;
    if (i >= w * h) return;
    uint32_t x = i % w, y = i / w;
    float xn = pixel_xn(x, w, inv_dim);
    float yn = pixel_yn(y, h, inv_dim);
    Rng r;
    r.seed(seed_mixed, i, sample);
    float dx = r.range(-inv_dim, inv_dim);
    float dy = r.range(-inv_dim, inv_dim);
    V ro, rd;
    cast_ray(cam, xn + dx, yn + dy, r, ro, rd);
    o[3 * i] = ro.x; o[3 * i + 1] = ro.y; o[3 * i + 2] = ro.z;
    d[3 * i] = rd.x; d[3 * i + 1] = rd.y; d[3 * i + 2] = rd.z;
    if (next_word) next_word[i] = r.next();
}
template <bool GROUPS>
__global__ __launch_bounds__(256) void debug_light_sample_kernel(const SceneView sc, const LightSampleArgs q) {
    __shared__ F4 lds_ltris[6u * kLdsLtris];
    LdsTables tab;
    {
        const uint32_t nl = sc.n_ltris <= kLdsLtris ? sc.n_ltris : 0u;
        for (uint32_t i = threadIdx.x; i < 6u * nl; i += 256u) lds_ltris[i] = reinterpret_cast<const F4*>(sc.ltris)[i];
        __syncthreads();
        tab.ltris = lds_ltris; tab.n_ltris = nl;
    }
    const uint64_t i = uint64_t(blockIdx.x) * 256u + threadIdx.x;
    if (i >= q.n) return;
    const Light L = uload(&sc.lights[q.light]);
    const V pos = mk(q.pos[3 * i], q.pos[3 * i + 1], q.pos[3 * i + 2]);
    Rng r;
    r.seed(q.seed_mixed, uint32_t(i), 0);
    Rng r2 = r;
    V v, n, I, wi;
    float p, dist;
    sample_light_shape<GROUPS>(sc, L, pos, r, v, n, p, tab);
    illuminate_object<GROUPS>(sc, L, pos, r2, I, wi, dist, tab);
    q.v[3 * i] = v.x; q.v[3 * i + 1] = v.y; q.v[3 * i + 2] = v.z;
    q.nrm[3 * i] = n.x; q.nrm[3 * i + 1] = n.y; q.nrm[3 * i + 2] = n.z;
    q.pdf[i] = p;
    q.intensity[3 * i] = I.x; q.intensity[3 * i + 1] = I.y; q.intensity[3 * i + 2] = I.z;
    q.wi[3 * i] = wi.x; q.wi[3 * i + 1] = wi.y; q.wi[3 * i + 2] = wi.z;
    q.dist[i] = dist;
    q.next_word[i] = r2.next();
}
__global__ __launch_bounds__(256) void debug_env_color_kernel(const SceneView sc, uint64_t n, const float* __restrict__ dirs,
                                                              float* __restrict__ rgb) {
    const uint64_t i = uint64_t(blockIdx.x) * 256u + threadIdx.x;
    if (i >= n) return;
    const V c = env_color(sc, mk(dirs[3 * i], dirs[3 * i + 1], dirs[3 * i + 2]));
    rgb[3 * i] = c.x; rgb[3 * i + 1] = c.y; rgb[3 * i + 2] = c.z;
}
__global__ __launch_bounds__(256) void debug_medium_distance_kernel(const SceneView sc, uint64_t n, uint64_t seed_mixed,
                                                                    float* __restrict__ dmed, float* __restrict__ limit) {
    const uint64_t i = uint64_t(blockIdx.x) * 256u + threadIdx.x;
    if (i >= n) return;
    const float sigma_t = sc.sigma_a + sc.sigma_s;
    const float inv_sigma_t = 1.f / sigma_t;
    Rng r;
    r.seed(seed_mixed, uint32_t(i), 0);
    float d, t;
    stage_distance<true>(r, inv_sigma_t, d, t);
    dmed[i] = d;
    limit[i] = t;
}
template <bool MEDIUM>
__global__ __launch_bounds__(256) void debug_bounce_kernel(const RenderArgs a, const BounceArgs q) {
    const uint64_t i = uint64_t(blockIdx.x) * 256u + threadIdx.x;
    if (i >= q.n) return;
    Rng r;
    r.seed(q.seed_mixed, uint32_t(i), 0);
    V wi = mk(0.f, 0.f, 0.f), k = mk(0.f, 0.f, 0.f);
    const bool go = stage_bounce<MEDIUM, false>(a, q.albedo_med, mk(q.rd[3 * i], q.rd[3 * i + 1], q.rd[3 * i + 2]), q.depth,
                                                MEDIUM && q.medium_event != 0u, mk(q.nrm[3 * i], q.nrm[3 * i + 1], q.nrm[3 * i + 2]),
                                                mk(q.mcol[0], q.mcol[1], q.mcol[2]), mat_from(q.m), r, wi, k);
    q.flag[i] = go ? 1 : 0;
    q.wi[3 * i] = wi.x; q.wi[3 * i + 1] = wi.y; q.wi[3 * i + 2] = wi.z;
    q.k[3 * i] = k.x; q.k[3 * i + 1] = k.y; q.k[3 * i + 2] = k.z;
    q.next_word[i] = r.next();
}

static constexpr size_t kStackBytes = 32u * 256u * sizeof(uint32_t);
static constexpr size_t kTabBytes = (2u * 32u + 6u * 8u) * 16u;
static constexpr size_t kStateBytes = 18u * 256u * sizeof(uint32_t) + kTabBytes;
static constexpr size_t kStateBytesBvh = 5u * 256u * sizeof(uint32_t) + kTabBytes;
static constexpr size_t kMeshTreeBytes = (21u + 5u) * 256u * sizeof(uint32_t) + kTabBytes;
static constexpr size_t kDetachBytes = kDetachDwords * sizeof(uint32_t);
static_assert(kTabBytes == kTabDwords * 4u, "one table layout");

template <bool M, int B, bool C>
static hipError_t launch_render_t(const RenderArgs& a, int n_blocks, hipStream_t stream) {
    const size_t lds = B == 1 ? kMeshTreeBytes : B ? kStackBytes + kStateBytesBvh : kStateBytes;
    if (a.sc.n_mono) {
        if (a.sc.n_lparts) hipLaunchKernelGGL((render_kernel<M, B, false, true, 0, true>), dim3(n_blocks), dim3(256), lds, stream, a);
        else hipLaunchKernelGGL((render_kernel<M, B, false, false, 0, true>), dim3(n_blocks), dim3(256), lds, stream, a);
        return hipGetLastError();
    }
    if constexpr (M && B == 1) {
#ifdef RPT_EXPERIMENTS
        if (a.detach == 2 && !a.sc.n_lparts) {
            hipLaunchKernelGGL((render_kernel<true, 1, C, false, 2>), dim3(n_blocks), dim3(256), kDetachBytes, stream, a);
            return hipGetLastError();
        }
#endif
        if (a.detach && !a.sc.n_lparts) {
            hipLaunchKernelGGL((render_kernel<true, 1, C, false, 1>), dim3(n_blocks), dim3(256), kDetachBytes, stream, a);
            return hipGetLastError();
        }
    }
    if (a.sc.n_lparts) hipLaunchKernelGGL((render_kernel<M, B, false, true>), dim3(n_blocks), dim3(256), lds, stream, a);
    else hipLaunchKernelGGL((render_kernel<M, B, C>), dim3(n_blocks), dim3(256), lds, stream, a);
    return hipGetLastError();
}
template <bool M, bool C>
static hipError_t launch_render_b(const RenderArgs& a, int bvh, int n_blocks, hipStream_t stream) {
    if (bvh == 3) return launch_render_t<M, 3, C>(a, n_blocks, stream);
    if (bvh == 2) return launch_render_t<M, 2, C>(a, n_blocks, stream);
    if (bvh == 1) return launch_render_t<M, 1, C>(a, n_blocks, stream);
    return launch_render_t<M, 0, C>(a, n_blocks, stream);
}
int bvh_mode(const SceneView& sc) { return sc.scene_bvh ? ((sc.mesh_deferred && sc.n_mesh) ? 3 : 2) : (sc.n_nodes ? 1 : 0); }
hipError_t launch_render(const RenderArgs& a, int n_blocks, hipStream_t stream) {
    const bool m = a.sc.has_medium != 0, c = a.counters != nullptr;
    const int b = bvh_mode(a.sc);
    if (m) return c ? launch_render_b<true, true>(a, b, n_blocks, stream) : launch_render_b<true, false>(a, b, n_blocks, stream);
    return c ? launch_render_b<false, true>(a, b, n_blocks, stream) : launch_render_b<false, false>(a, b, n_blocks, stream);
}
size_t stream_scratch_bytes_per_block() { return size_t(kWaveScratchDwords) * 4u * 4u; }
hipError_t render_occupancy(bool medium, int bvh, int* blocks_per_cu, int detach) {
#ifdef RPT_EXPERIMENTS
    if (detach == 2 && medium && bvh == 1)
        return hipOccupancyMaxActiveBlocksPerMultiprocessor(blocks_per_cu, (const void*)render_kernel<true, 1, false, false, 2>, 256, kDetachBytes);
#endif
    if (detach && medium && bvh == 1)
        return hipOccupancyMaxActiveBlocksPerMultiprocessor(blocks_per_cu, (const void*)render_kernel<true, 1, false, false, 1>, 256, kDetachBytes);
    const void* f;
    if (bvh == 3) return hipOccupancyMaxActiveBlocksPerMultiprocessor(blocks_per_cu, medium ? (const void*)render_kernel<true, 3, false> : (const void*)render_kernel<false, 3, false>,
                                                                      256, kStackBytes + kStateBytesBvh);
    if (medium) f = bvh == 2 ? (const void*)render_kernel<true, 2, false> : bvh == 1 ? (const void*)render_kernel<true, 1, false> : (const void*)render_kernel<true, 0, false>;
    else f = bvh == 2 ? (const void*)render_kernel<false, 2, false> : bvh == 1 ? (const void*)render_kernel<false, 1, false> : (const void*)render_kernel<false, 0, false>;
    return hipOccupancyMaxActiveBlocksPerMultiprocessor(blocks_per_cu, f, 256, bvh == 1 ? kMeshTreeBytes : bvh ? kStackBytes + kStateBytesBvh : kStateBytes);
}
hipError_t launch_resolve(const RenderArgs& a, double scale, double* d_out, hipStream_t stream) {
    uint32_t blocks = (a.n_owned + 255u) / 256u;
    hipLaunchKernelGGL(resolve_kernel, dim3(blocks), dim3(256), 0, stream, a, scale, d_out);
    return hipGetLastError();
}
hipError_t launch_buffer_add(uint32_t n_pixels, const double* d_batch, double* d_sum, double* d_sumsq, hipStream_t st) {
    hipLaunchKernelGGL(buffer_add_kernel, dim3((n_pixels + 255) / 256), dim3(256), 0, st, n_pixels, d_batch, d_sum, d_sumsq);
    return hipGetLastError();
}
hipError_t launch_buffer_image(uint32_t w, uint32_t h, uint32_t radius, uint32_t n_batches, const double* d_sum, uint8_t* d_out,
                               hipStream_t st) {
    hipLaunchKernelGGL(buffer_image_kernel, dim3((w * h + 255) / 256), dim3(256), 0, st, w, h, radius, n_batches, d_sum, d_out);
    return hipGetLastError();
}
hipError_t launch_buffer_variance(uint32_t n_pixels, uint32_t n_batches, const double* d_sum, const double* d_sumsq, double* d_out,
                                  hipStream_t st) {
    hipLaunchKernelGGL(buffer_variance_kernel, dim3((n_pixels + 255) / 256), dim3(256), 0, st, n_pixels, n_batches, d_sum, d_sumsq,
                       d_out);
    return hipGetLastError();
}
hipError_t launch_frame_pack(const double* d_frame, double* d_packed, const uint32_t* d_tiles, uint32_t n_tiles, uint32_t tiles_x,
                             uint32_t width, uint32_t height, hipStream_t st) {
    if (!n_tiles) return hipSuccess;
    hipLaunchKernelGGL(frame_tiles_kernel<true>, dim3(n_tiles * 12u), dim3(256), 0, st, d_frame, d_packed, d_tiles, n_tiles, tiles_x, width, height);
    return hipGetLastError();
}
hipError_t launch_frame_unpack(const double* d_packed, double* d_frame, const uint32_t* d_tiles, uint32_t n_tiles, uint32_t tiles_x,
                               uint32_t width, uint32_t height, hipStream_t st) {
    if (!n_tiles) return hipSuccess;
    hipLaunchKernelGGL(frame_tiles_kernel<false>, dim3(n_tiles * 12u), dim3(256), 0, st, d_packed, d_frame, d_tiles, n_tiles, tiles_x, width, height);
    return hipGetLastError();
}
hipError_t launch_intersect(const SceneView& sc, uint64_t n, const float* d_o, const float* d_d, float* d_t,
                            int32_t* d_obj, float* d_n, bool bvh, hipStream_t stream) {
    uint32_t blocks = uint32_t((n + 255) / 256);
    if (sc.n_mono) {
        if (bvh) hipLaunchKernelGGL((intersect_kernel<2, true>), dim3(blocks), dim3(256), kStackBytes, stream, sc, n, d_o, d_d, d_t, d_obj, d_n);
        else hipLaunchKernelGGL((intersect_kernel<0, true>), dim3(blocks), dim3(256), 0, stream, sc, n, d_o, d_d, d_t, d_obj, d_n);
        return hipGetLastError();
    }
    if (bvh) hipLaunchKernelGGL(intersect_kernel<2>, dim3(blocks), dim3(256), kStackBytes, stream, sc, n, d_o, d_d, d_t, d_obj, d_n);
    else hipLaunchKernelGGL(intersect_kernel<0>, dim3(blocks), dim3(256), 0, stream, sc, n, d_o, d_d, d_t, d_obj, d_n);
    return hipGetLastError();
}
hipError_t launch_intersect_segments(const SceneView& sc, uint64_t n, const float* d_o, const float* d_d, const float* d_tmax, float* d_t,
                                     uint32_t* d_code, hipStream_t stream) {
    hipLaunchKernelGGL(intersect_segments_kernel, dim3(uint32_t((n + 255) / 256)), dim3(256), 0, stream, sc, n, d_o, d_d, d_tmax, d_t, d_code);
    return hipGetLastError();
}
hipError_t launch_debug_rng(uint64_t seed_mixed, uint32_t pixel, uint32_t sample, uint32_t n, uint32_t* d_out,
                            hipStream_t stream) {
    hipLaunchKernelGGL(debug_rng_kernel, dim3(1), dim3(64), 0, stream, seed_mixed, pixel, sample, n, d_out);
    return hipGetLastError();
}
hipError_t launch_debug_sample_f(const Material& m, uint64_t n, const float* d_n, const float* d_wo,
                                 uint64_t seed_mixed, float* d_wi, float* d_pdf, int32_t* d_some, hipStream_t s) {
    hipLaunchKernelGGL(debug_sample_f_kernel, dim3(uint32_t((n + 255) / 256)), dim3(256), 0, s, m, n, d_n, d_wo, seed_mixed,
                       d_wi, d_pdf, d_some);
    return hipGetLastError();
}
hipError_t launch_debug_bsdf(const Material& m, uint64_t n, const float* d_n, const float* d_wo, const float* d_wi,
                             float* d_out, hipStream_t s) {
    hipLaunchKernelGGL(debug_bsdf_kernel, dim3(uint32_t((n + 255) / 256)), dim3(256), 0, s, m, n, d_n, d_wo, d_wi, d_out);
    return hipGetLastError();
}
hipError_t launch_debug_camera_sample(const CameraG& cam, uint32_t w, uint32_t h, float inv_dim, uint64_t seed_mixed, uint32_t sample,
                                      float* d_o, float* d_d, uint32_t* d_next_word, hipStream_t s) {
    hipLaunchKernelGGL(debug_camera_kernel, dim3((w * h + 255) / 256), dim3(256), 0, s, cam, w, h, inv_dim, seed_mixed, sample, d_o, d_d,
                       d_next_word);
    return hipGetLastError();
}
hipError_t launch_debug_light_sample(const SceneView& sc, const LightSampleArgs& q, hipStream_t s) {
    const dim3 grid(uint32_t((q.n + 255) / 256));
    if (sc.n_lparts) hipLaunchKernelGGL(debug_light_sample_kernel<true>, grid, dim3(256), 0, s, sc, q);
    else hipLaunchKernelGGL(debug_light_sample_kernel<false>, grid, dim3(256), 0, s, sc, q);
    return hipGetLastError();
}
hipError_t launch_debug_env_color(const SceneView& sc, uint64_t n, const float* d_dirs, float* d_rgb, hipStream_t s) {
    hipLaunchKernelGGL(debug_env_color_kernel, dim3(uint32_t((n + 255) / 256)), dim3(256), 0, s, sc, n, d_dirs, d_rgb);
    return hipGetLastError();
}
hipError_t launch_debug_medium_distance(const SceneView& sc, uint64_t n, uint64_t seed_mixed, float* d_dmed, float* d_limit,
                                        hipStream_t s) {
    hipLaunchKernelGGL(debug_medium_distance_kernel, dim3(uint32_t((n + 255) / 256)), dim3(256), 0, s, sc, n, seed_mixed, d_dmed, d_limit);
    return hipGetLastError();
}
hipError_t launch_debug_bounce(const BounceArgs& q, hipStream_t s) {
    RenderArgs a{};
    a.max_bounces = q.max_bounces;
    const dim3 grid(uint32_t((q.n + 255) / 256));
    if (q.in_medium) hipLaunchKernelGGL(debug_bounce_kernel<true>, grid, dim3(256), 0, s, a, q);
    else hipLaunchKernelGGL(debug_bounce_kernel<false>, grid, dim3(256), 0, s, a, q);
    return hipGetLastError();
}

}
```

### rpt_amd/csrc/rpt_capi.cpp

```cpp
#include <hip/hip_runtime_api.h>

#include <algorithm>
#include <cfloat>
#include <cmath>
#include <cstdio>
#include <cstring>
#include <functional>
#include <limits>
#include <memory>
#include <mutex>
#include <string>
#include <unordered_map>
#include <vector>

#include "../../include/rpt_hip.h"
#include "host_internal.h"
#include "kernels.h"
#include "f64_layout.h"

using namespace rptg;

static thread_local std::string g_err;
namespace rpti {
int fail(int code, const std::string& msg) {
    g_err = msg;
    return code;
}
}
using rpti::fail;
namespace rpti {
uint64_t seed_mix(uint64_t seed) {
    uint64_t x = seed + 0x9E3779B97F4A7C15ULL;
    x ^= x >> 30;
    x *= 0xBF58476D1CE4E5B9ULL;
    x ^= x >> 27;
    x *= 0x94D049BB133111EBULL;
    x ^= x >> 31;
    return x;
}
}
#define HIP_TRY(expr)                                                                              \
    do {                                                                                           \
        hipError_t e__ = (expr);                                                                   \
        if (e__ != hipSuccess)                                                                     \
            return fail(RPT_ERR_DEVICE, std::string(#expr) + ": " + hipGetErrorString(e__));       \
    } while (0)

struct rpt_options {
    int64_t counters = 0;
    int64_t chunk_spp = 0;
    int64_t blocks_per_cu = 0;
    int64_t max_blocks = 0;
    int64_t timing = 0;
    int64_t room_shell = 1;
    int64_t scan_specialise = 1;
    int64_t scan_cull = 1;
    int64_t photon_skip = 0;
    int64_t photon_block_lists = 1;
    int64_t photon_coop_gather = 1;
    int64_t photon_split = 0;
    int64_t photon_parts = 4;
    int64_t instancing = 1;
    int64_t bvh_leaf_max = 4;
    int64_t bvh_max_depth = 20;
    int64_t bvh_sweep_below = 4096;
    int64_t defer_stop = 16;
    int64_t walk_leaf_quarters = 6;
    int64_t defer_lanes = 32;
    int64_t detach_shadows = 1;
    int64_t stream_backlog = 48;
    int64_t stream_contexts = 1;
    int64_t detach_lanes = 44;
    int64_t pull_batch = 2;
    int64_t detach_trigger = 28;
    int64_t scene_bvh_min = 64;
    int64_t scene_tree_meshes = 0;
    int64_t f64_cull = 1;
    int64_t f64_photon_slice = 0;
    int64_t f64_surf_batch = 8;
    int64_t epsilon_policy = 0;
};
static rpt_options g_defaults;
static std::mutex g_defaults_mutex;
static int set_option_in(rpt_options& o, const char* name, int64_t value) {
    if (!name) return fail(RPT_ERR_INVALID, "null option name");
    const std::string s(name);
    if (s == "counters") o.counters = value;
    else if (s == "chunk_spp") { if (value < 0) return fail(RPT_ERR_INVALID, "chunk_spp must be >= 0 (0 = auto)"); o.chunk_spp = value; }
    else if (s == "blocks_per_cu") o.blocks_per_cu = value;
    else if (s == "max_blocks") { if (value < 0 || value > (1 << 20)) return fail(RPT_ERR_INVALID, "max_blocks must be 0..2^20 (0 = no cap)"); o.max_blocks = value; }
    else if (s == "timing") o.timing = value;
    else if (s == "room_shell") o.room_shell = value;
    else if (s == "scan_specialise") o.scan_specialise = value;
    else if (s == "scan_cull") o.scan_cull = value;
    else if (s == "photon_skip") o.photon_skip = value;
    else if (s == "photon_block_lists") o.photon_block_lists = value;
    else if (s == "photon_parts") o.photon_parts = value;
    else if (s == "photon_split") {
#ifndef RPT_EXPERIMENTS
        if (value != 0) return fail(RPT_ERR_UNSUPPORTED, "photon_split: a rejected prototype, built with -DRPT_EXPERIMENTS only");
#endif
        o.photon_split = value;
    }
    else if (s == "photon_coop_gather") o.photon_coop_gather = value;
    else if (s == "instancing") o.instancing = value;
    else if (s == "defer_lanes") { if (value < 1 || value > 64) return fail(RPT_ERR_INVALID, "defer_lanes must be 1..64"); o.defer_lanes = value; }
    else if (s == "bvh_leaf_max") { if (value < 1 || value > 16) return fail(RPT_ERR_INVALID, "bvh_leaf_max must be 1..16"); o.bvh_leaf_max = value; }
    else if (s == "bvh_sweep_below") { if (value < 0) return fail(RPT_ERR_INVALID, "bvh_sweep_below must be >= 0"); o.bvh_sweep_below = value; }
    else if (s == "bvh_max_depth") { if (value < 1 || value > 20) return fail(RPT_ERR_INVALID, "bvh_max_depth must be 1..20"); o.bvh_max_depth = value; }
    else if (s == "walk_leaf_quarters") { if (value < 0 || value > 256) return fail(RPT_ERR_INVALID, "walk_leaf_quarters must be 0..256"); o.walk_leaf_quarters = value; }
    else if (s == "detach_shadows") {
        if (value < 0 || value > 2) return fail(RPT_ERR_INVALID, "detach_shadows must be 0, 1 or 2");
#ifndef RPT_EXPERIMENTS
        if (value == 2) return fail(RPT_ERR_UNSUPPORTED, "detach_shadows = 2 (streamed walks): a rejected prototype, built with -DRPT_EXPERIMENTS only");
#endif
        o.detach_shadows = value;
    }
    else if (s == "stream_contexts") { if (value < 1 || value > 6) return fail(RPT_ERR_INVALID, "stream_contexts must be 1..6"); o.stream_contexts = value; }
    else if (s == "stream_backlog") { if (value < 1 || value > 256) return fail(RPT_ERR_INVALID, "stream_backlog must be 1..256"); o.stream_backlog = value; }
    else if (s == "detach_lanes") { if (value < 1 || value > 96) return fail(RPT_ERR_INVALID, "detach_lanes must be 1..96"); o.detach_lanes = value; }
    else if (s == "pull_batch") { if (value < 1 || value > 64) return fail(RPT_ERR_INVALID, "pull_batch must be 1..64"); o.pull_batch = value; }
    else if (s == "detach_trigger") { if (value < 1 || value > 32) return fail(RPT_ERR_INVALID, "detach_trigger must be 1..32"); o.detach_trigger = value; }
    else if (s == "defer_stop") { if (value < 1 || value > 64) return fail(RPT_ERR_INVALID, "defer_stop must be 1..64"); o.defer_stop = value; }
    else if (s == "f64_cull") { if (value < 0 || value > 2) return fail(RPT_ERR_INVALID, "f64_cull must be 0, 1 or 2"); o.f64_cull = value; }
    else if (s == "f64_photon_slice") { if (value < 0 || value > (1 << 20)) return fail(RPT_ERR_INVALID, "f64_photon_slice must be 0..2^20"); o.f64_photon_slice = value; }
    else if (s == "f64_surf_batch") { if (value < 1 || value > 64) return fail(RPT_ERR_INVALID, "f64_surf_batch must be 1..64"); o.f64_surf_batch = value; }
    else if (s == "epsilon_policy") { if (value < 0 || value > 1) return fail(RPT_ERR_INVALID, "epsilon_policy must be 0 or 1"); o.epsilon_policy = value; }
    else if (s == "scene_tree_meshes") o.scene_tree_meshes = value;
    else if (s == "scene_bvh_min") { if (value < 0) return fail(RPT_ERR_INVALID, "scene_bvh_min must be >= 0"); o.scene_bvh_min = value; }
    else return fail(RPT_ERR_INVALID, "unknown option: " + s);
    return RPT_OK;
}

namespace {
struct D3 {
    double x, y, z;
};
inline D3 operator+(D3 a, D3 b) { return {a.x + b.x, a.y + b.y, a.z + b.z}; }
inline D3 operator-(D3 a, D3 b) { return {a.x - b.x, a.y - b.y, a.z - b.z}; }
inline D3 operator*(double s, D3 a) { return {s * a.x, s * a.y, s * a.z}; }
inline double dot(D3 a, D3 b) { return a.x * b.x + a.y * b.y + a.z * b.z; }
inline D3 cross(D3 a, D3 b) { return {a.y * b.z - a.z * b.y, a.z * b.x - a.x * b.z, a.x * b.y - a.y * b.x}; }
inline D3 normalize(D3 a) {
    double l = std::sqrt(dot(a, a));
    return {a.x / l, a.y / l, a.z / l};
}
inline D3 d3(const double* p) { return {p[0], p[1], p[2]}; }
inline double comp(const D3& v, int a) { return a == 0 ? v.x : (a == 1 ? v.y : v.z); }
inline F4 f4(D3 v, double w) { return F4{float(v.x), float(v.y), float(v.z), float(w)}; }
inline float bits_f(uint32_t u) {
    float f;
    std::memcpy(&f, &u, 4);
    return f;
}
inline uint32_t bits_u(float f) {
    uint32_t u;
    std::memcpy(&u, &f, 4);
    return u;
}

struct Xf {
    bool has = false;
    double M[4][4], Minv[4][4], L[3][3], N[3][3], det = 1.0;
    D3 point(D3 p) const { return {M[0][0] * p.x + M[0][1] * p.y + M[0][2] * p.z + M[0][3], M[1][0] * p.x + M[1][1] * p.y + M[1][2] * p.z + M[1][3], M[2][0] * p.x + M[2][1] * p.y + M[2][2] * p.z + M[2][3]}; }
    D3 normal(D3 n) const { return {N[0][0] * n.x + N[0][1] * n.y + N[0][2] * n.z, N[1][0] * n.x + N[1][1] * n.y + N[1][2] * n.z, N[2][0] * n.x + N[2][1] * n.y + N[2][2] * n.z}; }
};
bool invert4(const double a[4][4], double out[4][4]) {
    double w[4][8];
    for (int i = 0; i < 4; i++)
        for (int j = 0; j < 4; j++) {
            w[i][j] = a[i][j];
            w[i][4 + j] = i == j ? 1.0 : 0.0;
        }
    for (int c = 0; c < 4; c++) {
        int p = c;
        for (int r = c + 1; r < 4; r++)
            if (std::fabs(w[r][c]) > std::fabs(w[p][c])) p = r;
// ... 245 lines not shown
        if (swept) {
            float parent_cost = area(lo, hi) * float(count);
            if (best_cost >= parent_cost && count <= 8 && leaf_ok) return make_leaf();
            mid = sweep_mid;
        } else if (balanced) {
            int axis = 0;
            for (int a = 1; a < 3; a++)
                if (chi[a] - clo[a] > chi[axis] - clo[axis]) axis = a;
            mid = first + count / 2;
            std::nth_element(t.begin() + first, t.begin() + mid, t.begin() + first + count,
                             [axis](const BTri& p, const BTri& q) { return p.c[axis] < q.c[axis]; });
        } else if (best_axis < 0 || depth >= kMaxDepth) {
            if (count <= 16 && leaf_ok) return make_leaf();
            mid = first + count / 2;
        } else {
            float parent_cost = area(lo, hi) * float(count);
            if (best_cost >= parent_cost && count <= 8 && leaf_ok) return make_leaf();
            float ext = chi[best_axis] - clo[best_axis];
            float scale = float(kBins) / ext;
            auto it = std::partition(t.begin() + first, t.begin() + first + count, [&](const BTri& x) {
                int b = std::min(kBins - 1, int((x.c[best_axis] - clo[best_axis]) * scale));
                return b <= best_bin;
            });
            mid = uint32_t(it - t.begin());
            if (mid == first || mid == first + count) mid = first + count / 2;
        }
        uint32_t left = uint32_t(nodes.size());
        nodes.push_back(TmpNode{});
        nodes.push_back(TmpNode{});
        nodes[node].left_or_first = left;
        nodes[node].count = 0;
        build(left, first, mid - first, depth + 1);
        build(left + 1, mid, first + count - mid, depth + 1);
    }
};

template <class T>
struct DevBuf {
    T* p = nullptr;
    size_t n = 0;
};

}

struct rpt_scene {
    std::vector<HObject> objects;
    std::vector<HLight> lights;
    std::vector<HMedium> media;
    double env[3] = {0, 0, 0};
    uint32_t hdri_w = 0, hdri_h = 0;
    std::vector<float> hdri;
    std::vector<double> hdri64;
    bool committed = false;
    rpt_options opt;
    int device = 0;
    int n_cus = 256;
    SceneView view{};
    struct LaunchSet {
        rpti::DevMem d_slab;
        rpti::DevMem d_queue;
        rpti::DevMem d_stream;
        rpti::Event done;
        rpti::Event launched;
        hipStream_t stream = nullptr;
        bool used = false;
    };
    struct Device {
        rpti::DevMem arena;
        rpti::DevMem arena64;
        rpti::DevMem d_tiles;
        LaunchSet sets[2];
        rpti::DevMem d_counters;
        rpti::DevMem d_out;
        std::vector<rpti::Event> evs;
    } dev;
    int cur_set = 0;
    uint64_t last_counters[64] = {0};
    uint64_t last_cull[12] = {0};
    static constexpr size_t kTimedLaunches = 1024;
    size_t ev_count = 0;
    int last_blocks = 0;
    uint64_t prims_per_ray = 0;
    uint32_t n_twin_lights = 0;
    bool twins_scanned = false;
    uint64_t stats[16] = {0};
    void* photon = nullptr;
    rpt64::Scene view64{};
    double medium_color64[3] = {0, 0, 0}, medium_color_hi64[3] = {0, 0, 0};
    uint64_t last_counters64[64] = {0};
    std::unordered_map<uint64_t, std::vector<std::shared_ptr<const std::vector<double>>>> mesh_pool;
    uint32_t tk_w = 0, tk_h = 0, tk_rank = 0, tk_count = 0, n_tiles = 0, tiles_x = 0;
};

using MeshCallCache = std::unordered_map<const double*, std::pair<uint64_t, std::shared_ptr<const std::vector<double>>>>;
static std::shared_ptr<const std::vector<double>> intern_mesh(rpt_scene* s, const double* p, uint64_t n_tris,
                                                              MeshCallCache& seen) {
    auto it = seen.find(p);
    if (it != seen.end() && it->second.first == n_tris) return it->second.second;
    const size_t n = size_t(n_tris) * 18;
    uint64_t h = 0xCBF29CE484222325ULL ^ n;
    for (size_t i = 0; i < n; i++) {
        uint64_t w;
        std::memcpy(&w, p + i, 8);
        h = (h ^ w) * 0x100000001B3ULL;
        h ^= h >> 29;
    }
    auto& bucket = s->mesh_pool[h];
    for (auto& c : bucket)
        if (c->size() == n && std::memcmp(c->data(), p, n * 8) == 0) { seen[p] = {n_tris, c}; return c; }
    auto m = std::make_shared<const std::vector<double>>(p, p + n);
    bucket.push_back(m);
    seen[p] = {n_tris, m};
    return m;
}
static bool copy_shape(rpt_scene* s, MeshCallCache& seen, const rpt_shape_desc* d, HShape& out, std::string& why,
                       int depth = 0) {
    if (!d) { why = "null shape"; return false; }
    if (d->kind < 0 || d->kind > RPT_SHAPE_MONOMIAL) { why = "unknown shape kind"; return false; }
    if (d->kind == RPT_SHAPE_MONOMIAL && !std::isfinite(d->plane_normal[0])) { why = "MonomialSurface height must be finite"; return false; }
    out.d = *d;
    out.mesh.reset();
    out.children.clear();
    if (d->kind == RPT_SHAPE_MESH) {
        if (d->n_tris == 0 || !d->tris) { why = "mesh without triangles"; return false; }
        out.mesh = intern_mesh(s, d->tris, d->n_tris, seen);
    }
    if (d->kind == RPT_SHAPE_GROUP) {
        if (d->n_children == 0 || !d->children) { why = "group without children"; return false; }
        if (depth >= 16) { why = "groups nested too deeply"; return false; }
        out.children.resize(d->n_children);
        for (uint64_t i = 0; i < d->n_children; i++) {
            if (d->children[i].kind == RPT_SHAPE_PLANE) { why = "Plane is not Bounded and cannot be a KdTree child (src/kdtree.rs:12)"; return false; }
            if (!copy_shape(s, seen, d->children + i, out.children[i], why, depth + 1)) return false;
        }
    }
    out.d.tris = nullptr;
    out.d.children = nullptr;
    Xf x;
    if (!make_xf(*d, x)) { why = "singular transform"; return false; }
    return true;
}
static bool holds_monomial(const HShape& h) {
    if (h.d.kind == RPT_SHAPE_MONOMIAL) return true;
    for (const HShape& c : h.children)
        if (holds_monomial(c)) return true;
    return false;
}
static bool check_material(const rpt_material* m, std::string& why) {
    if (!m) { why = "null material"; return false; }
    if (m->kind < 0 || m->kind > RPT_MAT_TRANSMISSIVE) { why = "unknown material kind"; return false; }
    return true;
}

extern "C" {

const char* rpt_last_error(void) { return g_err.c_str(); }

int rpt_device_count(void) {
    int n = 0;
    if (hipGetDeviceCount(&n) != hipSuccess) return 0;
    return n;
}

int rpt_set_option(const char* name, int64_t value) {
    std::lock_guard<std::mutex> lock(g_defaults_mutex);
    return set_option_in(g_defaults, name, value);
// ... 575 lines not shown
        const size_t n_items_total = sph.size() + cub.size() + aabb.size() + tri.size() + mono.size() + insts.size() + meshes.size() +
                                     rect_axis[0].size() + rect_axis[1].size() + rect_axis[2].size();
        const bool will_bvh = n_items_total >= size_t(std::max<int64_t>(2, s->opt.scene_bvh_min)) || !insts.empty();
        {
            const float inf = std::numeric_limits<float>::infinity();
            float blo[3] = {inf, inf, inf}, bhi[3] = {-inf, -inf, -inf};
            for (int a = 0; a < 3; a++)
                for (const RectScan& r : rect_axis[a]) {
                    const float lo[3] = {r.a.x, r.a.y, r.a.w}, hi[3] = {r.a.x, r.a.z, r.b.x};
                    for (int k = 0; k < 3; k++) {
                        blo[(a + k) % 3] = std::min(blo[(a + k) % 3], lo[k]);
                        bhi[(a + k) % 3] = std::max(bhi[(a + k) % 3], hi[k]);
                    }
                }
            int face_of[3][2] = {{-1, -1}, {-1, -1}, {-1, -1}}, n_faces = 0;
            if (!will_bvh && s->opt.room_shell)
                for (int a = 0; a < 3; a++)
                    for (size_t i = 0; i < rect_axis[a].size(); i++) {
                        const RectScan& r = rect_axis[a][i];
                        const int u = (a + 1) % 3, w = (a + 2) % 3;
                        if (r.a.y != blo[u] || r.a.z != bhi[u] || r.a.w != blo[w] || r.b.x != bhi[w]) continue;
                        for (int side = 0; side < 2; side++)
                            if (r.a.x == (side ? bhi[a] : blo[a]) && face_of[a][side] < 0 && blo[a] < bhi[a]) {
                                face_of[a][side] = int(i);
                                n_faces++;
                                break;
                            }
                    }
            if (n_faces >= 3) {
                has_shell = true;
                shell.lo = F4{blo[0], blo[1], blo[2], 0.f};
                shell.hi = F4{bhi[0], bhi[1], bhi[2], 0.f};
                for (int k = 0; k < 8; k++) shell.face[k] = CODE_MISS;
                size_t n_scanned = 0;
                for (int a = 0; a < 3; a++) n_scanned += rect_axis[a].size();
                n_scanned -= size_t(n_faces);
                for (int a = 0; a < 3; a++) {
                    int order[2] = {0, 1};
                    if (face_of[a][0] >= 0 && face_of[a][1] >= 0 && face_of[a][0] < face_of[a][1]) { order[0] = 1; order[1] = 0; }
                    RectShade keep[2];
                    for (int k = 0; k < 2; k++) {
                        const int side = order[k];
                        if (face_of[a][side] < 0) continue;
                        keep[side] = rect_sh_axis[a][size_t(face_of[a][side])];
                        rect_axis[a].erase(rect_axis[a].begin() + face_of[a][side]);
                        rect_sh_axis[a].erase(rect_sh_axis[a].begin() + face_of[a][side]);
                    }
                    for (int side = 0; side < 2; side++)
                        if (face_of[a][side] >= 0) {
                            shell.face[2 * a + side] = (K_RECT << 28) | uint32_t(n_scanned + shell_sh.size());
                            shell_sh.push_back(keep[side]);
                        }
                }
            }
        }
        for (int a = 0; a < 3; a++) {
            rect.insert(rect.end(), rect_axis[a].begin(), rect_axis[a].end());
            rect_sh.insert(rect_sh.end(), rect_sh_axis[a].begin(), rect_sh_axis[a].end());
        }
        rect_sh.insert(rect_sh.end(), shell_sh.begin(), shell_sh.end());
    }
    void mark_twin_ranges() {
        for (Light& L : lights) {
            L.twin_lo = 1u;
            L.twin_hi = 0u;
            if (L.kind != L_OBJECT || L.twin_object < 0) continue;
            const uint32_t tw = uint32_t(L.twin_object);
            std::vector<uint32_t> codes;
            bool other = false;
            auto same = [&](float w) { return bits_u(w) == tw; };
            for (size_t i = 0; i < sph_sh.size(); i++) if (same(sph_sh[i].r0.w)) codes.push_back((K_SPHERE << 28) | uint32_t(i));
            for (size_t i = 0; i < cub_sh.size(); i++) if (same(cub_sh[i].r0.w)) codes.push_back((K_CUBE << 28) | uint32_t(i));
            for (size_t i = 0; i < pln_sh.size(); i++) if (same(pln_sh[i].unit_n_obj.w)) codes.push_back((K_PLANE << 28) | uint32_t(i));
            for (size_t i = 0; i < tri_sh.size(); i++) if (same(tri_sh[i].n1.w)) codes.push_back((K_TRI << 28) | uint32_t(i));
            for (size_t i = 0; i < aabb.size(); i++) if (same(aabb[i].lo.w)) codes.push_back((K_AABB << 28) | uint32_t(i));
            for (size_t i = 0; i < rect_sh.size(); i++) if (same(rect_sh[i].n_obj.w)) codes.push_back((K_RECT << 28) | uint32_t(i));
            for (const MeshRef& m : meshes) if (m.object == tw) other = true;
            for (const InstRec& r : insts) if (same(r.n0.w)) other = true;
            if (other || codes.empty()) continue;
            bool contiguous = true;
            for (size_t i = 1; i < codes.size(); i++) contiguous = contiguous && codes[i] == codes[i - 1] + 1u;
            if (contiguous) { L.twin_lo = codes.front(); L.twin_hi = codes.back(); }
        }

    }
    int build_scene_tree() {
        {
            std::vector<BTri> items;
            std::vector<uint32_t> codes;
            auto add_item = [&](const float lo[3], const float hi[3], uint32_t code) {
                BTri it;
                for (int a = 0; a < 3; a++) { it.lo[a] = lo[a]; it.hi[a] = hi[a]; it.c[a] = 0.5f * (lo[a] + hi[a]); }
                it.idx = uint32_t(codes.size());
                items.push_back(it);
                codes.push_back(code);
            };
            for (size_t i = 0; i < sph.size(); i++) add_item(box_sph[i].lo, box_sph[i].hi, (K_SPHERE << 28) | uint32_t(i));
            for (size_t i = 0; i < cub.size(); i++) add_item(box_cub[i].lo, box_cub[i].hi, (K_CUBE << 28) | uint32_t(i));
            for (size_t i = 0; i < aabb.size(); i++) {
                float lo[3] = {aabb[i].lo.x, aabb[i].lo.y, aabb[i].lo.z}, hi[3] = {aabb[i].hi.x, aabb[i].hi.y, aabb[i].hi.z};
                add_item(lo, hi, (K_AABB << 28) | uint32_t(i));
            }
            {
                size_t i = 0;
                for (int axis = 0; axis < 3; axis++)
                    for (size_t k = 0; k < rect_axis[axis].size(); k++, i++) {
                        const RectScan& r = rect[i];
                        float lo[3], hi[3];
                        lo[axis] = hi[axis] = r.a.x;
                        lo[(axis + 1) % 3] = r.a.y; hi[(axis + 1) % 3] = r.a.z;
                        lo[(axis + 2) % 3] = r.a.w; hi[(axis + 2) % 3] = r.b.x;
                        add_item(lo, hi, (K_RECT << 28) | uint32_t(i));
                    }
            }
            for (size_t i = 0; i < tri.size(); i++) add_item(box_tri[i].lo, box_tri[i].hi, (K_TRI << 28) | uint32_t(i));
            for (size_t i = 0; i < mono.size(); i++) add_item(box_mono[i].lo, box_mono[i].hi, (K_MONO << 28) | uint32_t(i));
            for (size_t i = 0; i < insts.size(); i++) add_item(box_inst[i].lo, box_inst[i].hi, (K_INST << 28) | uint32_t(i));
            std::vector<uint8_t> solo(items.size(), 0);
            const size_t n_counted = items.size() + meshes.size();
            mesh_deferred = !s->opt.scene_tree_meshes && !meshes.empty() && items.size() >= 2;
            if (!mesh_deferred)
                for (size_t i = 0; i < meshes.size(); i++) {
                    add_item(box_mesh[i].lo, box_mesh[i].hi, (K_BVHTRI << 28) | uint32_t(i));
                    solo.push_back(1);
                }
            if (n_counted >= size_t(std::max<int64_t>(2, s->opt.scene_bvh_min)) || !insts.empty()) {
                scene_bvh = true;
                std::vector<TmpNode> tmp;
                tmp.reserve(2 * items.size());
                for (int attempt = 0; attempt < 2; attempt++) {
                    tmp.assign(1, TmpNode{});
                    BvhBuilder b{items, tmp};
                    b.leaf_max = 2;
                    b.solo = &solo;
                    b.balanced = attempt == 1;
                    b.build(0, 0, uint32_t(items.size()), 0);
                    top_depth = b.max_depth + 1;
                    if (top_depth + mesh_depth <= 31) break;
                }
                if (top_depth + mesh_depth > 31)
                    return fail(RPT_ERR_UNSUPPORTED, "scene tree + mesh tree are deeper than the traversal stack (32 levels)");
                std::vector<uint32_t> remap(tmp.size(), 0);
                uint32_t n_inner = 0;
                for (size_t k = 0; k < tmp.size(); k++)
                    if (tmp[k].count == 0) remap[k] = n_inner++;
                top_root = uint32_t(nodes.size());
                std::vector<BvhNode> local(n_inner);
                auto entry = [&](uint32_t k) -> uint32_t {
                    const TmpNode& c = tmp[k];
                    if (c.count == 0) return top_root + remap[k];
                    const uint32_t c0 = codes[items[c.left_or_first].idx];
                    if ((c0 >> 28) == K_BVHTRI) return meshes[c0 & 0x0FFFFFFFu].root;
                    const uint32_t first = uint32_t(pleaf.size());
                    for (uint32_t i = 0; i < c.count; i++) pleaf.push_back(codes[items[c.left_or_first + i].idx]);
                    return BVH_LEAF | BVH_PRIMS | ((c.count - 1u) << 26) | first;
                };
                for (size_t k = 0; k < tmp.size(); k++) {
                    if (tmp[k].count != 0) continue;
                    BvhNode& w = local[remap[k]];
                    uint32_t l = tmp[k].left_or_first;
                    for (int a = 0; a < 3; a++) {
                        w.lo0[a] = tmp[l].lo[a]; w.hi0[a] = tmp[l].hi[a];
                        w.lo1[a] = tmp[l + 1].lo[a]; w.hi1[a] = tmp[l + 1].hi[a];
                    }
                    w.e0 = entry(l);
                    w.e1 = entry(l + 1);
// ... 182 lines not shown
        put(o_pbox, pbox.data(), pbox.size() * sizeof(AabbScan));
        put(o_pleaf, pleaf.data(), pleaf.size() * sizeof(uint32_t));
        put(o_shell, &shell, sizeof(ShellScan));
        put(o_inst, insts.data(), insts.size() * sizeof(InstRec));
        put(o_rect, rect.data(), rect.size() * sizeof(RectScan));  put(o_rects, rect_sh.data(), rect_sh.size() * sizeof(RectShade));
        put(o_nodes, nodes.data(), nodes.size() * sizeof(BvhNode));
        put(o_btri, btri.data(), btri.size() * sizeof(TriScan));   put(o_btris, btri_sh.data(), btri_sh.size() * sizeof(TriShade));
        put(o_mesh, meshes.data(), meshes.size() * sizeof(MeshRef));
        put(o_mats, mats.data(), mats.size() * sizeof(Material));
        put(o_lights, lights.data(), lights.size() * sizeof(Light));
        put(o_ltris, ltris.data(), ltris.size() * sizeof(LightTri));
        put(o_lxf, lxf.data(), lxf.size() * sizeof(LightXf));
        put(o_lparts, lparts.data(), lparts.size() * sizeof(LightPart));
        put(o_hdri, s->hdri.data(), s->hdri.size() * sizeof(float));
        put(o_mono, mono.data(), mono.size() * sizeof(MonoScan));  put(o_monos, mono_sh.data(), mono_sh.size() * sizeof(XfShade));
        HIP_TRY(s->dev.arena.reserve(off));
        HIP_TRY(hipMemcpy(s->dev.arena.get(), host.data(), off, hipMemcpyHostToDevice));
        char* base = s->dev.arena.get<char>();
        SceneView& v = s->view;
        v.sph = (const XfScan*)(base + o_sph);      v.sph_sh = (const XfShade*)(base + o_sphs);    v.n_sph = uint32_t(sph.size());
        v.cub = (const XfScan*)(base + o_cub);      v.cub_sh = (const XfShade*)(base + o_cubs);    v.n_cub = uint32_t(cub.size());
        v.pln = (const PlaneScan*)(base + o_pln);   v.pln_sh = (const PlaneShade*)(base + o_plns); v.n_pln = uint32_t(pln.size());
        v.tri = (const TriScan*)(base + o_tri);     v.tri_sh = (const TriShade*)(base + o_tris);   v.n_tri = uint32_t(tri.size());
        v.aabb = (const AabbScan*)(base + o_aabb);  v.n_aabb = uint32_t(aabb.size());
        v.rect = (const RectScan*)(base + o_rect);  v.rect_sh = (const RectShade*)(base + o_rects);
        v.n_rect_x = uint32_t(rect_axis[0].size()); v.n_rect_y = uint32_t(rect_axis[1].size()); v.n_rect_z = uint32_t(rect_axis[2].size());
        v.shell = (const ShellScan*)(base + o_shell); v.has_shell = has_shell ? 1u : 0u;
        v.pbox = (const AabbScan*)(base + o_pbox);
        v.nodes = (const BvhNode*)(base + o_nodes); v.btri = (const TriScan*)(base + o_btri);      v.btri_sh = (const TriShade*)(base + o_btris);
        v.meshes = (const MeshRef*)(base + o_mesh); v.n_mesh = uint32_t(meshes.size());
        v.pleaf = (const uint32_t*)(base + o_pleaf); v.n_nodes = uint32_t(nodes.size());
        v.scene_bvh = scene_bvh ? 1u : 0u;          v.top_root = top_root;
        v.mesh_deferred = (scene_bvh && mesh_deferred) ? 1u : 0u;
        v.inst = (const InstRec*)(base + o_inst);   v.n_inst = uint32_t(insts.size());
        v.mono = (const MonoScan*)(base + o_mono);  v.mono_sh = (const XfShade*)(base + o_monos);  v.n_mono = uint32_t(mono.size());
        v.scan_pad_ = 0;  v.sph_yrot = sph_yrot;  v.cub_yrot = cub_yrot;
        v.scan_always = scan_always;
        std::memset(v.scan_groups, 0, sizeof(v.scan_groups));
        for (size_t g = 0; g < scan_groups.size(); g++) {
            for (int a = 0; a < 3; a++) { v.scan_groups[g].box.lo[a] = scan_groups[g].lo[a]; v.scan_groups[g].box.hi[a] = scan_groups[g].hi[a]; }
            v.scan_groups[g].mask = scan_groups[g].mask;
        }
        for (int a = 0; a < 3; a++) { v.scan_bound.lo[a] = scan_lo[a]; v.scan_bound.hi[a] = scan_hi[a]; v.scan_tail.lo[a] = tail_lo[a]; v.scan_tail.hi[a] = tail_hi[a]; }
        v.n_scan_groups = uint32_t(scan_groups.size());
        v.scan_cull = scan_cull ? 1u : 0u;
        v.scan_pad2_[0] = v.scan_pad2_[1] = 0;
        v.mats = (const Material*)(base + o_mats);  v.n_obj = uint32_t(mats.size());
        v.lights = (const Light*)(base + o_lights); v.n_lights = uint32_t(lights.size());
        v.ltris = (const LightTri*)(base + o_ltris); v.lxf = (const LightXf*)(base + o_lxf);
        v.lparts = (const LightPart*)(base + o_lparts); v.n_lparts = uint32_t(lparts.size());
        v.n_ltris = uint32_t(ltris.size());
        v.has_medium = s->media.empty() ? 0u : 1u;
        v.medium_kind = 0;
        v.sigma_a = v.sigma_s = 0.f;
        v.medium_emission = 0.f;
        v.medium_phase = 0.f;
        for (int i = 0; i < 3; i++) v.medium_color[i] = v.medium_color_hi[i] = 0.f;
        if (!s->media.empty()) {
            const HMedium& m = s->media[0];
            v.medium_kind = uint32_t(m.kind);
            v.sigma_a = float(m.absorption);
            v.sigma_s = float(m.scattering);
            const double pi = 3.14159265358979323846;
            if (m.kind == RPT_MEDIUM_HOMOGENEOUS_ISOTROPIC) {
                D3 c = hex_color(0xD2B48C);
                v.medium_color[0] = v.medium_color_hi[0] = float(c.x);
                v.medium_color[1] = v.medium_color_hi[1] = float(c.y);
                v.medium_color[2] = v.medium_color_hi[2] = float(c.z);
                v.medium_emission = 0.f;
                v.medium_phase = float(1.0 / (4.0 * pi));
            } else {
                D3 lo = hex_color(0x0000FF), hi = hex_color(0xFF0000);
                v.medium_color[0] = float(lo.x); v.medium_color[1] = float(lo.y); v.medium_color[2] = float(lo.z);
                v.medium_color_hi[0] = float(hi.x); v.medium_color_hi[1] = float(hi.y); v.medium_color_hi[2] = float(hi.z);
                v.medium_emission = 10.f;
                v.medium_phase = float(1.0 / 4.0 * pi);
            }
        }
        for (int i = 0; i < 3; i++) v.env[i] = float(s->env[i]);
        v.hdri = (const F4*)(base + o_hdri);
        v.hdri_w = s->hdri_w;
        v.hdri_h = s->hdri_h;
        s->prims_per_ray = sph.size() + cub.size() + pln.size() + tri.size() + aabb.size() + rect.size() + (has_shell ? 1 : 0);
        s->twins_scanned = true;
        s->n_twin_lights = 0;
        for (const Light& L : lights) {
            if (L.kind == L_OBJECT && L.twin_object >= 0) s->n_twin_lights++;
            if (L.kind == L_OBJECT && L.twin_object >= 0 && !(L.twin_lo <= L.twin_hi)) s->twins_scanned = false;
        }
        s->stats[0] = sph.size(); s->stats[1] = cub.size(); s->stats[2] = pln.size(); s->stats[3] = tri.size();
        s->stats[4] = aabb.size(); s->stats[5] = rect_sh.size(); s->stats[6] = btri.size(); s->stats[7] = nodes.size();
        s->stats[8] = 48 * (sph.size() + cub.size() + tri.size()) + 16 * pln.size() + 32 * (aabb.size() + rect.size());
        s->stats[9] = off;
        s->stats[10] = scene_bvh ? (mesh_deferred ? 2 : 1) : 0;
        s->stats[11] = pleaf.size();
        s->stats[14] = has_shell ? shell_sh.size() : 0;
        s->stats[15] = uint64_t(top_depth + mesh_depth);
        s->stats[12] = insts.size();
        s->stats[13] = shared.size();

        for (auto& ls : s->dev.sets) {
            HIP_TRY(ls.d_queue.reserve(256));
            HIP_TRY(ls.done.create(hipEventDisableTiming));
            HIP_TRY(ls.launched.create(hipEventDisableTiming));
        }
        HIP_TRY(s->dev.d_counters.reserve(80 * sizeof(unsigned long long)));
        s->view.stack_overflows = s->dev.d_counters.get<unsigned long long>() + 7;
        s->device = device;
        s->committed = true;
        return RPT_OK;
    }
};
}

#pragma clang fp contract(off)
static int check_scene64(const rpt_scene* s) {
    std::function<int(const HShape&)> depth = [&](const HShape& h) {
        int d = 0;
        for (const HShape& c : h.children) d = std::max(d, depth(c));
        return d + (h.d.kind == RPT_SHAPE_GROUP ? 1 : 0);
    };
    for (const auto& o : s->objects)
        if (depth(o.shape) > int(rpt64::kMaxFrames))
            return fail(RPT_ERR_UNSUPPORTED, "epsilon_policy = 1 supports KdTree groups nested at most three deep");
    for (const auto& l : s->lights)
        if (l.kind == int(L_OBJECT) && depth(l.obj.shape) > int(rpt64::kMaxFrames))
            return fail(RPT_ERR_UNSUPPORTED, "epsilon_policy = 1 supports KdTree groups nested at most three deep");
    return RPT_OK;
}
static int fill_shape64(const HShape& hs, rpt64::Shape& o, std::vector<rpt64::Tri>& tris, std::vector<double>& tri_pdf,
                        std::unordered_map<const std::vector<double>*, uint32_t>* shared = nullptr) {
    std::memset(&o, 0, sizeof(o));
    o.kind = hs.d.kind;
    Xf x;
    if (!make_xf(hs.d, x)) return fail(RPT_ERR_INVALID, "singular transform");
    o.has_xf = x.has ? 1 : 0;
    for (int i = 0; i < 3; i++)
        for (int j = 0; j < 4; j++) { o.inv[i * 4 + j] = x.Minv[i][j]; o.fwd[i * 4 + j] = x.M[i][j]; }
    for (int i = 0; i < 3; i++)
        for (int j = 0; j < 3; j++) { o.lin[i * 3 + j] = x.L[i][j]; o.nrm[i * 3 + j] = x.N[i][j]; }
    o.det = x.det;
    for (int k = 0; k < 3; k++) o.plane[k] = hs.d.plane_normal[k];
    o.plane[3] = hs.d.plane_value;
    if (hs.d.kind == RPT_SHAPE_MESH) {
        const std::vector<double>& T = hs.T();
        const auto known = (shared && hs.mesh) ? shared->find(hs.mesh.get()) : decltype(shared->end()){};
        const bool have = shared && hs.mesh && known != shared->end();
        o.tri_first = have ? known->second : uint32_t(tris.size());
        o.tri_count = uint32_t(T.size() / 18);
        if (shared && hs.mesh && !have) (*shared)[hs.mesh.get()] = o.tri_first;
        for (int k = 0; k < 3; k++) { o.bmin[k] = std::numeric_limits<double>::infinity(); o.bmax[k] = -o.bmin[k]; }
        for (size_t t = 0; t < T.size() / 18; t++) {
            rpt64::Tri tr;
            std::memcpy(&tr, T.data() + t * 18, sizeof(tr));
            for (int v = 0; v < 3; v++)
                for (int k = 0; k < 3; k++) {
                    o.bmin[k] = std::min(o.bmin[k], T[t * 18 + v * 3 + k]);
                    o.bmax[k] = std::max(o.bmax[k], T[t * 18 + v * 3 + k]);
                }
            if (have) continue;
            tris.push_back(tr);
            const double e0[3] = {tr.v2[0] - tr.v1[0], tr.v2[1] - tr.v1[1], tr.v2[2] - tr.v1[2]};
            const double e1[3] = {tr.v3[0] - tr.v1[0], tr.v3[1] - tr.v1[1], tr.v3[2] - tr.v1[2]};
            const double cx = e0[1] * e1[2] - e0[2] * e1[1], cy = e0[2] * e1[0] - e0[0] * e1[2], cz = e0[0] * e1[1] - e0[1] * e1[0];
            const double area = 0.5 * std::sqrt(cx * cx + cy * cy + cz * cz);
            tri_pdf.push_back((1.0 / area) / double(o.tri_count));
// ... 990 lines not shown
    if (!launch_debug_camera_sample) return fail(RPT_ERR_UNSUPPORTED, "rpt_debug_camera_sample: built without the kernels");
    const size_t n = size_t(prm->width) * prm->height;
    rpti::DevMem d_o, d_d, d_w;
    HIP_TRY(hook_scratch(d_o, n * 12));
    HIP_TRY(hook_scratch(d_d, n * 12));
    if (next_word) HIP_TRY(hook_scratch(d_w, n * 4));
    HIP_TRY(launch_debug_camera_sample(camera_g(cam), prm->width, prm->height, inv_dim_of(prm), seed_mix(seed), sample, d_o.get<float>(),
                                       d_d.get<float>(), next_word ? d_w.get<uint32_t>() : nullptr, nullptr));
    HIP_TRY(hipMemcpy(origins, d_o.get(), n * 12, hipMemcpyDeviceToHost));
    HIP_TRY(hipMemcpy(dirs, d_d.get(), n * 12, hipMemcpyDeviceToHost));
    if (next_word) HIP_TRY(hipMemcpy(next_word, d_w.get(), n * 4, hipMemcpyDeviceToHost));
    return RPT_OK;
}
int rpt_debug_camera_rays(const rpt_camera* cam, const rpt_render_params* prm, uint64_t seed, uint32_t sample,
                          float* origins, float* dirs) {
    return rpt_debug_camera_sample(cam, prm, seed, sample, origins, dirs, nullptr);
}
extern "C++" int rpti::light_kind(rpt_scene* s, uint32_t light) { return light < s->lights.size() ? int(s->lights[light].kind) : -1; }
int rpt_debug_light_sample(rpt_scene* s, uint32_t light, uint64_t n, const float* positions, uint64_t seed, float* v, float* nrm,
                           float* pdf, float* intensity, float* wi, float* dist, uint32_t* next_word) {
    if (!s || !positions || !v || !nrm || !pdf || !intensity || !wi || !dist || !next_word) return fail(RPT_ERR_INVALID, "null argument");
    if (rpti::light_kind(s, light) != int(L_OBJECT)) return fail(RPT_ERR_INVALID, "rpt_debug_light_sample: not a Light::Object");
    if (!s->committed) return fail(RPT_ERR_STATE, "rpt_scene_commit must be called first");
    if (s->dev.arena64) return fail(RPT_ERR_STATE, "rpt_debug_light_sample: the scene was committed with epsilon_policy = 1 (rpt_debug_light_sample_f64)");
    if (!launch_debug_light_sample) return fail(RPT_ERR_UNSUPPORTED, "rpt_debug_light_sample: built without the kernels");
    if (n == 0) return RPT_OK;
    if (n > 0xFFFFFFFFull) return fail(RPT_ERR_INVALID, "rpt_debug_light_sample: the case number keys a 32-bit stream field");
    HIP_TRY(hipSetDevice(s->device));
    rpti::DevMem d_pos, d_out;
    HIP_TRY(hook_scratch(d_pos, n * 12));
    HIP_TRY(hook_scratch(d_out, n * 60));
    HIP_TRY(hipMemcpy(d_pos.get(), positions, n * 12, hipMemcpyHostToDevice));
    float* const o = d_out.get<float>();
    LightSampleArgs q{};
    q.light = light;
    q.n = n;
    q.seed_mixed = seed_mix(seed);
    q.pos = d_pos.get<float>();
    q.v = o; q.nrm = o + 3 * n; q.intensity = o + 6 * n; q.wi = o + 9 * n;
    q.pdf = o + 12 * n; q.dist = o + 13 * n;
    q.next_word = reinterpret_cast<uint32_t*>(o + 14 * n);
    HIP_TRY(launch_debug_light_sample(s->view, q, nullptr));
    HIP_TRY(hipMemcpy(v, q.v, n * 12, hipMemcpyDeviceToHost));
    HIP_TRY(hipMemcpy(nrm, q.nrm, n * 12, hipMemcpyDeviceToHost));
    HIP_TRY(hipMemcpy(intensity, q.intensity, n * 12, hipMemcpyDeviceToHost));
    HIP_TRY(hipMemcpy(wi, q.wi, n * 12, hipMemcpyDeviceToHost));
    HIP_TRY(hipMemcpy(pdf, q.pdf, n * 4, hipMemcpyDeviceToHost));
    HIP_TRY(hipMemcpy(dist, q.dist, n * 4, hipMemcpyDeviceToHost));
    HIP_TRY(hipMemcpy(next_word, q.next_word, n * 4, hipMemcpyDeviceToHost));
    return RPT_OK;
}
int rpt_debug_env_color(rpt_scene* s, uint64_t n, const float* dirs, float* rgb) {
    if (!s || !dirs || !rgb) return fail(RPT_ERR_INVALID, "null argument");
    if (!s->committed) return fail(RPT_ERR_STATE, "rpt_scene_commit must be called first");
    if (s->dev.arena64) return fail(RPT_ERR_STATE, "rpt_debug_env_color: the scene was committed with epsilon_policy = 1 (rpt_debug_env_color_f64)");
    if (!launch_debug_env_color) return fail(RPT_ERR_UNSUPPORTED, "rpt_debug_env_color: built without the kernels");
    if (n == 0) return RPT_OK;
    HIP_TRY(hipSetDevice(s->device));
    rpti::DevMem d_d, d_c;
    HIP_TRY(hook_scratch(d_d, n * 12));
    HIP_TRY(hook_scratch(d_c, n * 12));
    HIP_TRY(hipMemcpy(d_d.get(), dirs, n * 12, hipMemcpyHostToDevice));
    HIP_TRY(launch_debug_env_color(s->view, n, d_d.get<float>(), d_c.get<float>(), nullptr));
    HIP_TRY(hipMemcpy(rgb, d_c.get(), n * 12, hipMemcpyDeviceToHost));
    return RPT_OK;
}
int rpt_debug_medium_distance(rpt_scene* s, uint64_t n, uint64_t seed, float* dmed, float* t_limit) {
    if (!s || !dmed || !t_limit) return fail(RPT_ERR_INVALID, "null argument");
    if (s->media.empty()) return fail(RPT_ERR_INVALID, "rpt_debug_medium_distance: the scene has no medium");
    if (!s->committed) return fail(RPT_ERR_STATE, "rpt_scene_commit must be called first");
    if (s->dev.arena64) return fail(RPT_ERR_STATE, "rpt_debug_medium_distance: the scene was committed with epsilon_policy = 1");
    if (!launch_debug_medium_distance) return fail(RPT_ERR_UNSUPPORTED, "rpt_debug_medium_distance: built without the kernels");
    if (n == 0) return RPT_OK;
    if (n > 0xFFFFFFFFull) return fail(RPT_ERR_INVALID, "rpt_debug_medium_distance: the case number keys a 32-bit stream field");
    HIP_TRY(hipSetDevice(s->device));
    rpti::DevMem d_m, d_t;
    HIP_TRY(hook_scratch(d_m, n * 4));
    HIP_TRY(hook_scratch(d_t, n * 4));
    HIP_TRY(launch_debug_medium_distance(s->view, n, seed_mix(seed), d_m.get<float>(), d_t.get<float>(), nullptr));
    HIP_TRY(hipMemcpy(dmed, d_m.get(), n * 4, hipMemcpyDeviceToHost));
    HIP_TRY(hipMemcpy(t_limit, d_t.get(), n * 4, hipMemcpyDeviceToHost));
    return RPT_OK;
}

int rpt_debug_bounce(const rpt_material* m, uint32_t max_bounces, uint32_t depth, int32_t in_medium, int32_t medium_event,
                     float albedo_med, const float* medium_color, uint64_t n, const float* normals, const float* rds, uint64_t seed,
                     int32_t* flag, float* wi, float* k, uint32_t* next_word) {
    std::string why;
    if (!check_material(m, why)) return fail(RPT_ERR_INVALID, why);
    if (!medium_color || !normals || !rds || !flag || !wi || !k || !next_word) return fail(RPT_ERR_INVALID, "null argument");
    if (medium_event && !in_medium) return fail(RPT_ERR_INVALID, "rpt_debug_bounce: a medium event needs in_medium");
    if (n > 0xFFFFFFFFull) return fail(RPT_ERR_INVALID, "rpt_debug_bounce: the case number keys a 32-bit stream field");
    if (!launch_debug_bounce) return fail(RPT_ERR_UNSUPPORTED, "rpt_debug_bounce: built without the kernels");
    if (n == 0) return RPT_OK;
    rpti::DevMem d_in, d_out;
    HIP_TRY(hook_scratch(d_in, n * 24));
    HIP_TRY(hook_scratch(d_out, n * 32));
    float* const in = d_in.get<float>();
    float* const o = d_out.get<float>();
    HIP_TRY(hipMemcpy(in, normals, n * 12, hipMemcpyHostToDevice));
    HIP_TRY(hipMemcpy(in + 3 * n, rds, n * 12, hipMemcpyHostToDevice));
    BounceArgs q{};
    q.m = to_gpu_material(m);
    q.max_bounces = max_bounces;
    q.depth = depth;
    q.in_medium = in_medium ? 1u : 0u;
    q.medium_event = medium_event ? 1u : 0u;
    q.albedo_med = albedo_med;
    for (int i = 0; i < 3; i++) q.mcol[i] = medium_color[i];
    q.n = n;
    q.seed_mixed = seed_mix(seed);
    q.nrm = in; q.rd = in + 3 * n;
    q.wi = o; q.k = o + 3 * n;
    q.flag = reinterpret_cast<int32_t*>(o + 6 * n);
    q.next_word = reinterpret_cast<uint32_t*>(o + 7 * n);
    HIP_TRY(launch_debug_bounce(q, nullptr));
    HIP_TRY(hipMemcpy(wi, q.wi, n * 12, hipMemcpyDeviceToHost));
    HIP_TRY(hipMemcpy(k, q.k, n * 12, hipMemcpyDeviceToHost));
    HIP_TRY(hipMemcpy(flag, q.flag, n * 4, hipMemcpyDeviceToHost));
    HIP_TRY(hipMemcpy(next_word, q.next_word, n * 4, hipMemcpyDeviceToHost));
    return RPT_OK;
}

}
```

Measured before the change: 14450 Msamples/s.

## Add a dedicated shadow-ray scan form that tracks light-twin visibility without hit codes

After: 14870 Msamples/s, median of 6. 2.9% higher.

```diff
diff --git a/include/rpt_hip.h b/include/rpt_hip.h
--- a/include/rpt_hip.h
+++ b/include/rpt_hip.h
@@ -165,6 +165,10 @@
 int rpt_debug_env_color(rpt_scene*, uint64_t n, const float* dirs, float* rgb);
 int rpt_debug_env_color_f64(rpt_scene*, uint64_t n, const double* dirs, double* rgb);
 int rpt_debug_medium_distance(rpt_scene*, uint64_t n, uint64_t seed, float* dmed, float* t_limit);
+int rpt_debug_shadow_test(rpt_scene*, uint32_t light, uint64_t n, const float* origins, const float* dirs, const float* dist,
+                          int32_t* out_flag, float* out_t);
+int rpt_shadow_scan_info(rpt_scene*, uint32_t light, uint32_t out[4]);
+int rpt_debug_distance_pair(float sigma_t, uint32_t k0, uint32_t n, float* out_new, float* out_guarded);
 
 int rpt_debug_bounce(const rpt_material* m, uint32_t max_bounces, uint32_t depth, int32_t in_medium, int32_t medium_event,
                      float albedo_med, const float* medium_color, uint64_t n, const float* normals, const float* rds, uint64_t seed,
diff --git a/rpt_amd/_lib.py b/rpt_amd/_lib.py
--- a/rpt_amd/_lib.py
+++ b/rpt_amd/_lib.py
@@ -146,6 +146,9 @@
      [C.POINTER(CameraDesc), C.POINTER(RenderParams), C.c_uint64, C.c_uint32, _P, _P, _P]),
     ("rpt_debug_bounce", C.c_int, [C.POINTER(MaterialDesc), C.c_uint32, C.c_uint32, C.c_int32, C.c_int32, C.c_float, _P,
                                    C.c_uint64, _P, _P, C.c_uint64, _P, _P, _P, _P]),
+    ("rpt_debug_shadow_test", C.c_int, [_P, C.c_uint32, C.c_uint64, _P, _P, _P, _P, _P]),
+    ("rpt_debug_distance_pair", C.c_int, [C.c_float, C.c_uint32, C.c_uint32, _P, _P]),
+    ("rpt_shadow_scan_info", C.c_int, [_P, C.c_uint32, C.POINTER(C.c_uint32)]),
     ("rpt_debug_material_f64", C.c_int, [C.POINTER(MaterialDesc), C.c_uint64, _P, _P, C.c_uint64, _P, _P, _P, _P, _P]),
     ("rpt_debug_material_bsdf_f64", C.c_int, [C.POINTER(MaterialDesc), C.c_uint64, _P, _P, _P, _P]),
 ]
diff --git a/rpt_amd/api.py b/rpt_amd/api.py
--- a/rpt_amd/api.py
+++ b/rpt_amd/api.py
@@ -914,6 +914,30 @@
         _lib.check(lib.rpt_debug_medium_distance(h, n, seed, dmed.ctypes.data_as(C.c_void_p), lim.ctypes.data_as(C.c_void_p)))
         return dmed, lim
 
+    def debug_shadow_test(self, light_index, origins, dirs, dist):
+        lib = _lib.load()
+        h = self.scene._commit(self.device_)
+        o = np.ascontiguousarray(origins, dtype=np.float32).reshape(-1, 3)
+        d = np.ascontiguousarray(dirs, dtype=np.float32).reshape(-1, 3)
+        ds = np.ascontiguousarray(dist, dtype=np.float32).reshape(-1)
+        n = o.shape[0]
+        if d.shape[0] != n or ds.shape[0] != n:
+            raise ValueError("origins, dirs and dist differ in length")
+        flag, t = np.empty(n, np.int32), np.empty(n, np.float32)
+        _lib.check(lib.rpt_debug_shadow_test(h, light_index, n, _vp(o), _vp(d), _vp(ds), _vp(flag), _vp(t)))
+        return flag, t
+
+    def shadow_scan_info(self, light_index):
+        out = (C.c_uint32 * 4)()
+        _lib.check(_lib.load().rpt_shadow_scan_info(self.scene._commit(self.device_), light_index, out))
+        return {"twin_lo": int(out[0]), "twin_hi": int(out[1]), "shadow_form": int(out[2]), "twin_object": int(np.int32(np.uint32(out[3])))}
+
+
+def debug_distance_pair(sigma_t, k0, n):
+    new, guarded = np.empty(n, np.float32), np.empty(n, np.float32)
+    _lib.check(_lib.load().rpt_debug_distance_pair(float(sigma_t), int(k0), int(n), _vp(new), _vp(guarded)))
+    return new, guarded
+
 
 def debug_bounce(material, normals, rds, max_bounces=3, depth=0, seed=0, in_medium=False, medium_event=False, albedo_med=0.0,
                  medium_color=(0.0, 0.0, 0.0)):
diff --git a/rpt_amd/csrc/device_core.h b/rpt_amd/csrc/device_core.h
--- a/rpt_amd/csrc/device_core.h
+++ b/rpt_amd/csrc/device_core.h
@@ -1,5 +1,6 @@
 #pragma once
 #include <hip/hip_runtime.h>
+#include <type_traits>
 #include "gpu_layout.h"
 
 namespace rptg {
@@ -165,27 +166,40 @@
     float t = (nv.w - dot3(nv, o)) * rcp(c);
     return (t >= tmin) ? t : -1.f;
 }
-RPT_DEV float hit_tri(const F4& pn, const F4& A, const F4& B, V o, V d, float tmin, float tmax) {
+RPT_DEV bool plane_closer(const F4& nv, V o, V d, float tmin, float tbest, float& t) {
+    float c = dot3(nv, d);
+    t = (nv.w - dot3(nv, o)) * rcp(c);
+    return !(fabsf(c) < 1e-8f) && t >= tmin && t < tbest;
+}
+RPT_DEV bool tri_closer(const F4& pn, const F4& A, const F4& B, V o, V d, float tmin, float tmax, float& t) {
     float c = dot3(pn, d);
-    float t = (pn.w - dot3(pn, o)) * rcp(c);
+    t = (pn.w - dot3(pn, o)) * rcp(c);
     V p = fma3(t, d, o);
     float v = dot3w(A, p), w = dot3w(B, p);
     float u = 1.f - v - w;
-    bool ok = fabsf(c) >= 1e-8f && t >= tmin && t < tmax && u >= 0.f && v >= 0.f && w >= 0.f;
-    return ok ? t : -1.f;
+    return fabsf(c) >= 1e-8f && t >= tmin && t < tmax && u >= 0.f && v >= 0.f && w >= 0.f;
+}
+RPT_DEV float hit_tri(const F4& pn, const F4& A, const F4& B, V o, V d, float tmin, float tmax) {
+    float t;
+    return tri_closer(pn, A, B, o, d, tmin, tmax, t) ? t : -1.f;
 }
 RPT_DEV float hit_aabb(const F4& lo, const F4& hi, V o, V inv, float tmin) {
     float t;
     return aabb_closer(lo, hi, o, inv, tmin, __builtin_inff(), t) ? t : -1.f;
 }
+RPT_DEV bool rect_closer(const F4& a, float vmax, float oa, float ia, float ou, float du, float ov, float dv,
+                         float tmin, float tmax, float& t) {
+    t = (a.x - oa) * ia;
+    float pu = fmaf(t, du, ou), pv = fmaf(t, dv, ov);
+    return t >= tmin && t < tmax && pu >= a.y && pu <= a.z && pv >= a.w && pv <= vmax;
+}
 RPT_DEV float hit_rect(const F4& a, float vmax, float oa, float ia, float ou, float du, float ov, float dv,
                        float tmin, float tmax) {
-    float t = (a.x - oa) * ia;
-    float pu = fmaf(t, du, ou), pv = fmaf(t, dv, ov);
-    bool ok = t >= tmin && t < tmax && pu >= a.y && pu <= a.z && pv >= a.w && pv <= vmax;
-    return ok ? t : -1.f;
-}
-RPT_DEV void hit_shell(const ShellScan& s, V o, V inv, float tmin, float& tbest, uint32_t& code) {
+    float t;
+    return rect_closer(a, vmax, oa, ia, ou, du, ov, dv, tmin, tmax, t) ? t : -1.f;
+}
+template <class Acc>
+RPT_DEV void shell_closer(const ShellScan& s, V o, V inv, float tmin, float tbest, Acc&& acc) {
     float x1 = (s.lo.x - o.x) * inv.x, x2 = (s.hi.x - o.x) * inv.x;
     float y1 = (s.lo.y - o.y) * inv.y, y2 = (s.hi.y - o.y) * inv.y;
     float z1 = (s.lo.z - o.z) * inv.z, z2 = (s.hi.z - o.z) * inv.z;
@@ -203,7 +217,7 @@
     bool use_in = box && start >= tmin && c_in != CODE_MISS;
     bool use_out = box && end >= tmin && c_out != CODE_MISS;
     float t = use_in ? start : end;
-    if ((use_in || use_out) && t < tbest) { tbest = t; code = use_in ? c_in : c_out; }
+    acc((use_in || use_out) && t < tbest, t, [&] { return use_in ? c_in : c_out; });
 }
 RPT_DEV void to_local(const XfScan& x, V o, V d, V& ol, V& dl) {
     ol = mk(dot3w(x.r0, o), dot3w(x.r1, o), dot3w(x.r2, o));
@@ -213,8 +227,9 @@
     ol = mk(fmaf(x.r0.x, o.x, fmaf(x.r0.z, o.z, x.r0.w)), fmaf(x.r1.y, o.y, x.r1.w), fmaf(x.r2.x, o.x, fmaf(x.r2.z, o.z, x.r2.w)));
     dl = mk(fmaf(x.r0.x, d.x, x.r0.z * d.z), x.r1.y * d.y, fmaf(x.r2.x, d.x, x.r2.z * d.z));
 }
-RPT_DEV void aabb_pair_closer(const AabbScan& b0, const AabbScan& b1, uint32_t shared, V o, V inv, float tmin, float& tbest,
-                              uint32_t& code, uint32_t i) {
+template <class Acc>
+RPT_DEV void aabb_pair_closer(const AabbScan& b0, const AabbScan& b1, uint32_t shared, V o, V inv, float tmin, float& tbest, uint32_t i,
+                              Acc&& acc) {
 #pragma clang fp contract(off)
     const float x1 = (b0.lo.x - o.x) * inv.x, x2 = (b0.hi.x - o.x) * inv.x;
     const float y1 = (b0.lo.y - o.y) * inv.y, y2 = (b0.hi.y - o.y) * inv.y;
@@ -223,13 +238,13 @@
     float start = max3(xl, yl, zl), end = min3(xh, yh, zh);
     asm volatile("" : "+v"(start), "+v"(end));
     float t = start < tmin ? end : start;
-    if (!(start > end) && !(end < tmin) && t < tbest) { tbest = t; code = (K_AABB << 28) | i; }
+    acc(!(start > end) && !(end < tmin) && t < tbest, t, i);
     if (!(shared & 1u)) { const float u1 = (b1.lo.x - o.x) * inv.x, u2 = (b1.hi.x - o.x) * inv.x; xl = fminf(u1, u2); xh = fmaxf(u1, u2); }
     if (!(shared & 2u)) { const float u1 = (b1.lo.y - o.y) * inv.y, u2 = (b1.hi.y - o.y) * inv.y; yl = fminf(u1, u2); yh = fmaxf(u1, u2); }
     if (!(shared & 4u)) { const float u1 = (b1.lo.z - o.z) * inv.z, u2 = (b1.hi.z - o.z) * inv.z; zl = fminf(u1, u2); zh = fmaxf(u1, u2); }
     start = max3(xl, yl, zl), end = min3(xh, yh, zh);
     t = start < tmin ? end : start;
-    if (!(start > end) && !(end < tmin) && t < tbest) { tbest = t; code = (K_AABB << 28) | (i + 1u); }
+    acc(!(start > end) && !(end < tmin) && t < tbest, t, i + 1u);
 }
 RPT_DEV bool mono_closer(V ol, V dl, const F4& hb, float tmin, float tbest, float& t) {
 #pragma clang fp contract(off)
@@ -423,26 +438,56 @@
     }
     return !(fmaxf(start, tmin) > fminf(end, tbest));
 }
-template <bool MASKED = false, bool MONO = false, bool TAIL = false>
+struct ShadowTwin {
+    uint32_t kind, lo, span;
+    RPT_DEV bool has(uint32_t i) const { return i - lo <= span; }
+};
+template <bool MASKED = false, bool MONO = false, bool TAIL = false, bool SHADOW = false>
 RPT_DEV void scan_prims(const SceneView& scene, V o, V d, float tmin, float& tbest, uint32_t& code, uint64_t mask = ~0ull,
-                        bool* tail_skipped = nullptr) {
+                        bool* tail_skipped = nullptr, ShadowTwin twin = ShadowTwin{0u, 1u, 0u}, bool* best_is_twin = nullptr) {
     static_assert(!(TAIL && MASKED), "one cull at a time");
+    static_assert(!(SHADOW && (MASKED || TAIL)), "the shadow form is a plain scan");
     const auto& sc = *kernarg_scene();
     (void)scene;
+    bool flag = false;
+    float t_twin = __builtin_nanf("");
+    auto acc = [&](bool ok, float t, uint32_t c, auto is_twin) {
+        if (ok) tbest = t;
+        asm volatile("" : "+v"(tbest));
+        if constexpr (!SHADOW) { if (ok) code = c; }
+        else if constexpr (std::is_same_v<decltype(is_twin), std::false_type>) flag = flag && !ok;
+        else if (ok && is_twin) t_twin = t;
+    };
+    auto twin_at = [&](auto tw, uint32_t i) {
+        if constexpr (decltype(tw)::value) return twin.has(i);
+        else return std::false_type{};
+    };
+    auto kind_loop = [&](uint32_t kind, auto&& loop) {
+        if constexpr (SHADOW) {
+            if (twin.kind == kind) {
+                loop(std::true_type{});
+                flag = t_twin == tbest;
+                return;
+            }
+        }
+        loop(std::false_type{});
+    };
     uint32_t bit = 0;
     auto on = [&](uint32_t i) { return !MASKED || ((mask >> ((bit + i) & 63u)) & 1ull) != 0ull; };
     const uint64_t sph_yrot = MASKED ? 0ull : sc.sph_yrot, cub_yrot = MASKED ? 0ull : sc.cub_yrot;
-    for (uint32_t i = 0; i < sc.n_sph; i++) {
-        if (!on(i)) continue;
-        const XfScan x = uload(&sc.sph[i]);
-        V ol, dl;
-        if (!MASKED && ((sph_yrot >> (i & 63u)) & 1ull)) to_local_y(x, o, d, ol, dl);
-        else to_local(x, o, d, ol, dl);
-        float t;
-        if (sphere_closer(ol, dl, tmin, tbest, t)) { tbest = t; code = (K_SPHERE << 28) | i; }
-    }
+    kind_loop(K_SPHERE, [&](auto tw) {
+        for (uint32_t i = 0; i < sc.n_sph; i++) {
+            if (!on(i)) continue;
+            const XfScan x = uload(&sc.sph[i]);
+            V ol, dl;
+            if (!MASKED && ((sph_yrot >> (i & 63u)) & 1ull)) to_local_y(x, o, d, ol, dl);
+            else to_local(x, o, d, ol, dl);
+            float t;
+            acc(sphere_closer(ol, dl, tmin, tbest, t), t, (K_SPHERE << 28) | i, twin_at(tw, i));
+        }
+    });
     bit += sc.n_sph;
-    {
+    kind_loop(K_CUBE, [&](auto tw) {
         uint32_t i = 0;
         if (!MASKED)
             for (; i + 1u < sc.n_cub; i += 2u) {
@@ -456,8 +501,8 @@
                     to_local(x0, o, d, ol0, dl0);
                     to_local(x1, o, d, ol1, dl1);
                 }
-                if (cube_closer(ol0, dl0, tmin, tbest, t0)) { tbest = t0; code = (K_CUBE << 28) | i; }
-                if (cube_closer(ol1, dl1, tmin, tbest, t1)) { tbest = t1; code = (K_CUBE << 28) | (i + 1u); }
+                acc(cube_closer(ol0, dl0, tmin, tbest, t0), t0, (K_CUBE << 28) | i, twin_at(tw, i));
+                acc(cube_closer(ol1, dl1, tmin, tbest, t1), t1, (K_CUBE << 28) | (i + 1u), twin_at(tw, i + 1u));
             }
         for (; i < sc.n_cub; i++) {
             if (!on(i)) continue;
@@ -466,19 +511,23 @@
             if (!MASKED && ((cub_yrot >> (i & 63u)) & 1ull)) to_local_y(x, o, d, ol, dl);
             else to_local(x, o, d, ol, dl);
             float t;
-            if (cube_closer(ol, dl, tmin, tbest, t)) { tbest = t; code = (K_CUBE << 28) | i; }
-        }
-    }
+            acc(cube_closer(ol, dl, tmin, tbest, t), t, (K_CUBE << 28) | i, twin_at(tw, i));
+        }
+    });
     bit += sc.n_cub;
     for (uint32_t i = 0; i < sc.n_pln; i++) {
         const F4 nv = uload(&sc.pln[i]).nv;
-        float t = hit_plane(nv, o, d, tmin);
-        if (t >= 0.f && t < tbest) { tbest = t; code = (K_PLANE << 28) | i; }
+        float t;
+        acc(plane_closer(nv, o, d, tmin, tbest, t), t, (K_PLANE << 28) | i, std::false_type{});
     }
     const uint32_t n_rect = sc.n_rect_x + sc.n_rect_y + sc.n_rect_z;
     if (sc.n_aabb + n_rect + sc.has_shell != 0) {
         const V inv = mk(rcp(d.x), rcp(d.y), rcp(d.z));
-        if (sc.has_shell) hit_shell(uload(sc.shell), o, inv, tmin, tbest, code);
+        if (sc.has_shell)
+            shell_closer(uload(sc.shell), o, inv, tmin, tbest, [&](bool ok, float t, auto code_of) {
+                if constexpr (SHADOW) acc(ok, t, 0u, std::false_type{});
+                else { if (ok) { tbest = t; code = code_of(); } }
+            });
         if constexpr (TAIL) {
             if (sc.scan_cull) {
                 const SceneView::ScanBox tb = kernarg_load(&sc.scan_tail);
@@ -488,50 +537,55 @@
                 }
             }
         }
-        {
+        kind_loop(K_AABB, [&](auto tw) {
             uint32_t i = 0;
             if (!MASKED)
                 for (; i + 1u < sc.n_aabb; i += 2u) {
                     const AabbScan b0 = uload(&sc.aabb[i]), b1 = uload(&sc.aabb[i + 1u]);
-                    aabb_pair_closer(b0, b1, __float_as_uint(b0.hi.w), o, inv, tmin, tbest, code, i);
+                    aabb_pair_closer(b0, b1, __float_as_uint(b0.hi.w), o, inv, tmin, tbest, i,
+                                     [&](bool ok, float t, uint32_t k) { acc(ok, t, (K_AABB << 28) | k, twin_at(tw, k)); });
                 }
             for (; i < sc.n_aabb; i++) {
                 if (!on(i)) continue;
                 const AabbScan b = uload(&sc.aabb[i]);
                 float t;
-                if (aabb_closer(b.lo, b.hi, o, inv, tmin, tbest, t)) { tbest = t; code = (K_AABB << 28) | i; }
-            }
-        }
+                acc(aabb_closer(b.lo, b.hi, o, inv, tmin, tbest, t), t, (K_AABB << 28) | i, twin_at(tw, i));
+            }
+        });
         bit += sc.n_aabb;
-        uint32_t i = 0;
-        for (uint32_t e = sc.n_rect_x; i < e; i++) {
-            if (!on(i)) continue;
-            const RectScan r = uload(&sc.rect[i]);
-            float t = hit_rect(r.a, r.b.x, o.x, inv.x, o.y, d.y, o.z, d.z, tmin, tbest);
-            if (t >= 0.f) { tbest = t; code = (K_RECT << 28) | i; }
-        }
-        for (uint32_t e = sc.n_rect_x + sc.n_rect_y; i < e; i++) {
-            if (!on(i)) continue;
-            const RectScan r = uload(&sc.rect[i]);
-            float t = hit_rect(r.a, r.b.x, o.y, inv.y, o.z, d.z, o.x, d.x, tmin, tbest);
-            if (t >= 0.f) { tbest = t; code = (K_RECT << 28) | i; }
-        }
-        for (uint32_t e = n_rect; i < e; i++) {
-            if (!on(i)) continue;
-            const RectScan r = uload(&sc.rect[i]);
-            float t = hit_rect(r.a, r.b.x, o.z, inv.z, o.x, d.x, o.y, d.y, tmin, tbest);
-            if (t >= 0.f) { tbest = t; code = (K_RECT << 28) | i; }
-        }
+        kind_loop(K_RECT, [&](auto tw) {
+            uint32_t i = 0;
+            for (uint32_t e = sc.n_rect_x; i < e; i++) {
+                if (!on(i)) continue;
+                const RectScan r = uload(&sc.rect[i]);
+                float t;
+                acc(rect_closer(r.a, r.b.x, o.x, inv.x, o.y, d.y, o.z, d.z, tmin, tbest, t), t, (K_RECT << 28) | i, twin_at(tw, i));
+            }
+            for (uint32_t e = sc.n_rect_x + sc.n_rect_y; i < e; i++) {
+                if (!on(i)) continue;
+                const RectScan r = uload(&sc.rect[i]);
+                float t;
+                acc(rect_closer(r.a, r.b.x, o.y, inv.y, o.z, d.z, o.x, d.x, tmin, tbest, t), t, (K_RECT << 28) | i, twin_at(tw, i));
+            }
+            for (uint32_t e = n_rect; i < e; i++) {
+                if (!on(i)) continue;
+                const RectScan r = uload(&sc.rect[i]);
+                float t;
+                acc(rect_closer(r.a, r.b.x, o.z, inv.z, o.x, d.x, o.y, d.y, tmin, tbest, t), t, (K_RECT << 28) | i, twin_at(tw, i));
+            }
+        });
         bit += n_rect;
     } else {
         bit += sc.n_aabb + n_rect;
     }
-    for (uint32_t i = 0; i < sc.n_tri; i++) {
-        if (!on(i)) continue;
-        const TriScan tr = uload(&sc.tri[i]);
-        float t = hit_tri(tr.pn, tr.A, tr.B, o, d, tmin, tbest);
-        if (t >= 0.f) { tbest = t; code = (K_TRI << 28) | i; }
-    }
+    kind_loop(K_TRI, [&](auto tw) {
+        for (uint32_t i = 0; i < sc.n_tri; i++) {
+            if (!on(i)) continue;
+            const TriScan tr = uload(&sc.tri[i]);
+            float t;
+            acc(tri_closer(tr.pn, tr.A, tr.B, o, d, tmin, tbest, t), t, (K_TRI << 28) | i, twin_at(tw, i));
+        }
+    });
     if constexpr (MONO) {
         static_assert(!MASKED && !TAIL, "scan_mask_for_ball and the tail cull do not cover the monomial surfaces");
         for (uint32_t i = 0; i < sc.n_mono; i++) {
@@ -539,9 +593,10 @@
             V ol, dl;
             to_local(XfScan{m.r0, m.r1, m.r2}, o, d, ol, dl);
             float t;
-            if (mono_closer(ol, dl, m.h, tmin, tbest, t)) { tbest = t; code = (K_MONO << 28) | i; }
-        }
-    }
+            acc(mono_closer(ol, dl, m.h, tmin, tbest, t), t, (K_MONO << 28) | i, std::false_type{});
+        }
+    }
+    if constexpr (SHADOW) *best_is_twin = flag;
 }
 RPT_DEV uint64_t scan_mask_for_ball(const SceneView& scene_, bool live, V c, float r, bool* touched = nullptr) {
     const auto& sc = *kernarg_scene();
@@ -933,12 +988,16 @@
 
 template <bool UNIFORM> struct LightXfRows;
 template <> struct LightXfRows<true> {
-    LightXf x;
-    RPT_DEV explicit LightXfRows(const LightXf* p) : x(uload(p)) {}
-    RPT_DEV F4 fwd(int r) const { return x.fwd[r]; }
-    RPT_DEV F4 inv(int r) const { return x.inv[r]; }
-    RPT_DEV F4 nrm(int r) const { return x.nrm[r]; }
-    RPT_DEV F4 lin(int r) const { return x.lin[r]; }
+    const LightXf* p;
+    RPT_DEV explicit LightXfRows(const LightXf* q) : p(q) {}
+    RPT_DEV F4 fwd(int r) const { return uload(&p->fwd[r]); }
+    RPT_DEV F4 inv(int r) const { return uload(&p->inv[r]); }
+    RPT_DEV F4 nrm(int r) const { return uload(&p->nrm[r]); }
+    RPT_DEV F4 lin(int r) const { return uload(&p->lin[r]); }
+    RPT_DEV bool has_transform() const {
+        typedef const __attribute__((address_space(4))) float* CF;
+        return *(CF)(uintptr_t)&p->nrm[1].w != 0.f;
+    }
 };
 template <> struct LightXfRows<false> {
     const LightXf* p;
@@ -947,6 +1006,7 @@
     RPT_DEV F4 inv(int r) const { return p->inv[r]; }
     RPT_DEV F4 nrm(int r) const { return p->nrm[r]; }
     RPT_DEV F4 lin(int r) const { return p->lin[r]; }
+    RPT_DEV bool has_transform() const { return p->nrm[1].w != 0.f; }
 };
 template <bool UNIFORM>
 RPT_DEV void sample_light_leaf(const SceneView& scene_, uint32_t shape, uint32_t first, uint32_t count, const LightXf* xp,
@@ -954,7 +1014,7 @@
     const auto& sc = *kernarg_scene();
     V vl, nl;
     const LightXfRows<UNIFORM> x(xp);
-    const bool xf = x.nrm(1).w != 0.f;
+    const bool xf = x.has_transform();
     const bool mesh = shape == LS_MESH;
     if (mesh) {
         uint32_t idx = rng.index(count);
@@ -965,18 +1025,23 @@
         } else {
             tr = sc.ltris[first + idx];
         }
-        uint32_t ku = rng.next() >> 9, kv = rng.next() >> 9;
-        while (ku + kv >= (1u << 23)) {
-            ku = rng.next() >> 9;
-            kv = rng.next() >> 9;
-        }
+        uint32_t wu = rng.next() & ~511u, wv = rng.next() & ~511u, sum;
+        while (__builtin_add_overflow(wu, wv, &sum)) {
+            wu = rng.next() & ~511u;
+            wv = rng.next() & ~511u;
+        }
+        const uint32_t ku = wu >> 9, kv = wv >> 9;
         const float u = float((ku << 1) | 1u) * 0x1p-24f, vv = float((kv << 1) | 1u) * 0x1p-24f;
         float w = 1.f - u - vv;
         vl = u * xyz(tr.v1) + vv * xyz(tr.v2) + w * xyz(tr.v3);
         nl = normalize(u * xyz(tr.n1) + vv * xyz(tr.n2) + w * xyz(tr.n3));
         p = tr.v1.w * rcp(float(count));
     } else if (shape == LS_SPHERE) {
-        V tl = xf ? mk(dot3w(x.inv(0), pos), dot3w(x.inv(1), pos), dot3w(x.inv(2), pos)) : pos;
+        V tl = pos;
+        if (xf) {
+            const F4 i0 = x.inv(0), i1 = x.inv(1), i2 = x.inv(2);
+            tl = mk(dot3w(i0, pos), dot3w(i1, pos), dot3w(i2, pos));
+        }
         float dx, dy;
         rng.unit_disc(dx, dy);
         float z = sqrt1(fmaxf(1.f - dx * dx - dy * dy, 0.f));
@@ -1001,11 +1066,18 @@
         p = 1.f / 6.f;
     }
     if (xf) {
-        n = normalize(mk(dot3(x.nrm(0), nl), dot3(x.nrm(1), nl), dot3(x.nrm(2), nl)));
-        V ln = mk(dot3(x.lin(0), nl), dot3(x.lin(1), nl), dot3(x.lin(2), nl));
+        const F4 n0 = x.nrm(0), n1 = x.nrm(1), n2 = x.nrm(2);
+        n = normalize(mk(dot3(n0, nl), dot3(n1, nl), dot3(n2, nl)));
+        const F4 l0 = x.lin(0), l1 = x.lin(1), l2 = x.lin(2);
+        V ln = mk(dot3(l0, nl), dot3(l1, nl), dot3(l2, nl));
         float height = dot(ln, n);
-        float base = x.nrm(0).w * rcp(height);
-        v = mesh ? vl : mk(dot3w(x.fwd(0), vl), dot3w(x.fwd(1), vl), dot3w(x.fwd(2), vl));
+        float base = n0.w * rcp(height);
+        if (mesh) {
+            v = vl;
+        } else {
+            const F4 f0 = x.fwd(0), f1 = x.fwd(1), f2 = x.fwd(2);
+            v = mk(dot3w(f0, vl), dot3w(f1, vl), dot3w(f2, vl));
+        }
         p = p * rcp(base);
     } else {
         v = vl;
diff --git a/rpt_amd/csrc/kernels.h b/rpt_amd/csrc/kernels.h
--- a/rpt_amd/csrc/kernels.h
+++ b/rpt_amd/csrc/kernels.h
@@ -85,6 +85,17 @@
 __attribute__((weak)) hipError_t launch_debug_env_color(const SceneView& sc, uint64_t n, const float* d_dirs, float* d_rgb, hipStream_t s);
 __attribute__((weak)) hipError_t launch_debug_medium_distance(const SceneView& sc, uint64_t n, uint64_t seed_mixed, float* d_dmed,
                                                               float* d_limit, hipStream_t s);
+struct ShadowTestArgs {
+    uint32_t light;
+    uint32_t pad_;
+    uint64_t n;
+    const float *o, *d;
+    const float* dist;
+    int32_t* flag;
+    float* t;
+};
+__attribute__((weak)) hipError_t launch_debug_shadow_test(const SceneView& sc, const ShadowTestArgs& q, hipStream_t s);
+__attribute__((weak)) hipError_t launch_debug_distance_pair(float sigma_t, uint32_t k0, uint32_t n, float* d_new, float* d_guarded, hipStream_t s);
 struct BounceArgs {
     Material m;
     uint32_t max_bounces, depth;
diff --git a/rpt_amd/csrc/kernels.hip b/rpt_amd/csrc/kernels.hip
--- a/rpt_amd/csrc/kernels.hip
+++ b/rpt_amd/csrc/kernels.hip
@@ -116,12 +116,23 @@
 #else
 #define SECTK(k) SECT(k)
 #endif
+RPT_DEV float medium_distance_guarded(float xi, float inv_sigma_t) { return -__logf(xi) * inv_sigma_t; }
+RPT_DEV float medium_distance(float xi, float inv_sigma_t) {
+#pragma clang fp contract(off)
+    const float ln2_hi = 0x1.62e42ep-1f, ln2_lo = 0x1.efa39ep-25f;
+    const float y = __builtin_amdgcn_logf(xi);
+    const float r = y * ln2_hi;
+    const float e = __builtin_fmaf(y, ln2_hi, -r);
+    const float lo = __builtin_fmaf(y, ln2_lo, e);
+    const float ln = __builtin_fmaf(ln2_hi, y, lo);
+    return -ln * inv_sigma_t;
+}
 template <bool MEDIUM>
 RPT_DEV void stage_distance(Rng& rng, float inv_sigma_t, float& dmed, float& t) {
     dmed = kInf;
     if (MEDIUM) {
         float xi = rng.range(0.f, 1.f);
-        dmed = -__logf(xi) * inv_sigma_t;
+        dmed = medium_distance(xi, inv_sigma_t);
     }
     t = (MEDIUM && dmed < 400.f) ? dmed * (1.f + 1e-6f) : kInf;
 }
@@ -145,19 +156,37 @@
         E = (depth == 0) ? mat_emit(mat) * mat_color(mat) : mk(0, 0, 0);
     }
 }
+template <bool PIN_RD = false>
+RPT_DEV void stage_light_add(const SceneView& sc, float albedo_med, V rd, bool medium, V I, V wi, V n, V mcol, const Mat& mat, V& E) {
+    if (medium) {
+        E = fma3(albedo_med * sc.medium_phase, I * mcol, E);
+    } else {
+        if constexpr (PIN_RD) asm volatile("" : "+v"(rd.x), "+v"(rd.y), "+v"(rd.z));
+        V f = bsdf(mat, n, -normalize(rd), wi);
+        E = fma3(dot(wi, n), f * I, E);
+    }
+}
 template <bool MONO = false>
 RPT_DEV void stage_light_term(const SceneView& sc, const Light& L, float albedo_med, V rd, bool medium, float ts, uint32_t cs,
                               uint32_t is, float dist, V I, V wi, V n, V mcol, const Mat& mat, V& E) {
     const bool twin = (L.twin_lo <= L.twin_hi) ? (cs >= L.twin_lo && cs <= L.twin_hi)
                                                : (cs != CODE_MISS && code_object<MONO>(sc, cs, is) == uint32_t(L.twin_object));
-    if (cs != CODE_MISS && ts >= dist * (1.f - 1e-3f) && twin) {
-        if (medium) {
-            E = fma3(albedo_med * sc.medium_phase, I * mcol, E);
-        } else {
-            V f = bsdf(mat, n, -normalize(rd), wi);
-            E = fma3(dot(wi, n), f * I, E);
-        }
+    if (cs != CODE_MISS && ts >= dist * (1.f - 1e-3f) && twin) stage_light_add(sc, albedo_med, rd, medium, I, wi, n, mcol, mat, E);
+}
+template <bool MONO = false>
+RPT_DEV bool scan_light_visible(const SceneView& sc, const Light& L, V x, V wi, float dist, float& ts) {
+    ts = dist * (1.f + 1e-3f);
+    uint32_t cs = CODE_MISS;
+    if (__float_as_uint(L.color.w) != 0u) {
+        bool twin = false;
+        scan_prims<false, MONO, false, true>(sc, x, wi, ray_tmin(x), ts, cs, ~0ull, nullptr,
+                                             ShadowTwin{L.twin_lo >> 28, L.twin_lo & 0x0FFFFFFFu, L.twin_hi - L.twin_lo}, &twin);
+        return twin && ts >= dist * (1.f - 1e-3f);
     }
+    scan_prims<false, MONO>(sc, x, wi, ray_tmin(x), ts, cs);
+    const bool twin = (L.twin_lo <= L.twin_hi) ? (cs >= L.twin_lo && cs <= L.twin_hi)
+                                               : (cs != CODE_MISS && code_object<MONO>(sc, cs, 0u) == uint32_t(L.twin_object));
+    return cs != CODE_MISS && ts >= dist * (1.f - 1e-3f) && twin;
 }
 template <bool MEDIUM, bool COUNT>
 RPT_DEV bool stage_bounce(const RenderArgs& a, float albedo_med, V rd, uint32_t depth, bool medium, V n, V mcol, const Mat& mat,
@@ -1112,14 +1141,22 @@
                 illuminate_object<GROUPS>(sc, L, x, rng, I, wi, dist, tab);
                 if (L.twin_object >= 0) {
                     SECTK(8);
-                    float ts = dist * (1.f + 1e-3f);
-                    uint32_t cs = CODE_MISS, is = 0;
-                    const bool range = L.twin_lo <= L.twin_hi;
-                    closest_hit<BVH, COUNT, BVH != 0, MONO>(sc, x, wi, ray_tmin(x), ts, cs, is, stk, stride, c_nodes, c_btris,
-                                                     AnyHit{range ? dist * (1.f - 1e-3f) : -kInf, L.twin_lo, L.twin_hi});
-                    if (COUNT) c_rays++;
-                    SECTK(9);
-                    stage_light_term<MONO>(sc, L, albedo_med, rd, ev_medium, ts, cs, is, dist, I, wi, n, mcol, mat, E);
+                    if constexpr (BVH == 0) {
+                        float ts;
+                        const bool visible = scan_light_visible<MONO>(sc, L, x, wi, dist, ts);
+                        if (COUNT) c_rays++;
+                        SECTK(9);
+                        if (visible) stage_light_add<true>(sc, albedo_med, rd, ev_medium, I, wi, n, mcol, mat, E);
+                    } else {
+                        float ts = dist * (1.f + 1e-3f);
+                        uint32_t cs = CODE_MISS, is = 0;
+                        const bool range = L.twin_lo <= L.twin_hi;
+                        closest_hit<BVH, COUNT, true, MONO>(sc, x, wi, ray_tmin(x), ts, cs, is, stk, stride, c_nodes, c_btris,
+                                                            AnyHit{range ? dist * (1.f - 1e-3f) : -kInf, L.twin_lo, L.twin_hi});
+                        if (COUNT) c_rays++;
+                        SECTK(9);
+                        stage_light_term<MONO>(sc, L, albedo_med, rd, ev_medium, ts, cs, is, dist, I, wi, n, mcol, mat, E);
+                    }
                 }
             }
         }
@@ -1390,6 +1427,26 @@
     dmed[i] = d;
     limit[i] = t;
 }
+template <bool MONO>
+__global__ __launch_bounds__(256) void debug_shadow_test_kernel(const SceneView sc, const ShadowTestArgs q) {
+    const uint64_t i = uint64_t(blockIdx.x) * 256u + threadIdx.x;
+    if (i >= q.n) return;
+    const Light L = uload(&sc.lights[q.light]);
+    float ts;
+    const bool vis = scan_light_visible<MONO>(sc, L, mk(q.o[3 * i], q.o[3 * i + 1], q.o[3 * i + 2]), mk(q.d[3 * i], q.d[3 * i + 1], q.d[3 * i + 2]),
+                                              q.dist[i], ts);
+    q.flag[i] = vis ? 1 : 0;
+    q.t[i] = ts;
+}
+__global__ __launch_bounds__(256) void debug_distance_pair_kernel(float sigma_t, uint32_t k0, uint32_t n, float* __restrict__ out_new,
+                                                                  float* __restrict__ out_guarded) {
+    const uint32_t i = blockIdx.x * 256u + threadIdx.x;
+    if (i >= n) return;
+    const float inv_sigma_t = 1.f / sigma_t;
+    const float xi = float(((k0 + i) << 1) | 1u) * 0x1p-24f;
+    out_new[i] = medium_distance(xi, inv_sigma_t);
+    out_guarded[i] = medium_distance_guarded(xi, inv_sigma_t);
+}
 template <bool MEDIUM>
 __global__ __launch_bounds__(256) void debug_bounce_kernel(const RenderArgs a, const BounceArgs q) {
     const uint64_t i = uint64_t(blockIdx.x) * 256u + threadIdx.x;
@@ -1553,6 +1610,16 @@
     hipLaunchKernelGGL(debug_medium_distance_kernel, dim3(uint32_t((n + 255) / 256)), dim3(256), 0, s, sc, n, seed_mixed, d_dmed, d_limit);
     return hipGetLastError();
 }
+hipError_t launch_debug_shadow_test(const SceneView& sc, const ShadowTestArgs& q, hipStream_t s) {
+    const dim3 grid(uint32_t((q.n + 255) / 256));
+    if (sc.n_mono) hipLaunchKernelGGL(debug_shadow_test_kernel<true>, grid, dim3(256), 0, s, sc, q);
+    else hipLaunchKernelGGL(debug_shadow_test_kernel<false>, grid, dim3(256), 0, s, sc, q);
+    return hipGetLastError();
+}
+hipError_t launch_debug_distance_pair(float sigma_t, uint32_t k0, uint32_t n, float* d_new, float* d_guarded, hipStream_t s) {
+    hipLaunchKernelGGL(debug_distance_pair_kernel, dim3((n + 255u) / 256u), dim3(256), 0, s, sigma_t, k0, n, d_new, d_guarded);
+    return hipGetLastError();
+}
 hipError_t launch_debug_bounce(const BounceArgs& q, hipStream_t s) {
     RenderArgs a{};
     a.max_bounces = q.max_bounces;
diff --git a/rpt_amd/csrc/rpt_capi.cpp b/rpt_amd/csrc/rpt_capi.cpp
--- a/rpt_amd/csrc/rpt_capi.cpp
+++ b/rpt_amd/csrc/rpt_capi.cpp
@@ -55,6 +55,7 @@
     int64_t room_shell = 1;
     int64_t scan_specialise = 1;
     int64_t scan_cull = 1;
+    int64_t shadow_scan = 1;
     int64_t photon_skip = 0;
     int64_t photon_block_lists = 1;
     int64_t photon_coop_gather = 1;
@@ -93,6 +94,7 @@
     else if (s == "room_shell") o.room_shell = value;
     else if (s == "scan_specialise") o.scan_specialise = value;
     else if (s == "scan_cull") o.scan_cull = value;
+    else if (s == "shadow_scan") o.shadow_scan = value;
     else if (s == "photon_skip") o.photon_skip = value;
     else if (s == "photon_block_lists") o.photon_block_lists = value;
     else if (s == "photon_parts") o.photon_parts = value;
@@ -504,6 +506,7 @@
     int last_blocks = 0;
     uint64_t prims_per_ray = 0;
     uint32_t n_twin_lights = 0;
+    std::vector<Light> light_records;
     bool twins_scanned = false;
     uint64_t stats[16] = {0};
     void* photon = nullptr;
@@ -1245,6 +1248,14 @@
             for (size_t i = 1; i < codes.size(); i++) contiguous = contiguous && codes[i] == codes[i - 1] + 1u;
             if (contiguous) { L.twin_lo = codes.front(); L.twin_hi = codes.back(); }
         }
+        for (Light& L : lights) {
+            L.color.w = 0.f;
+            if (L.kind != L_OBJECT || L.twin_object < 0 || !(L.twin_lo <= L.twin_hi) || !s->opt.shadow_scan) continue;
+            const uint32_t kind = L.twin_lo >> 28, last = L.twin_hi & 0x0FFFFFFFu;
+            const bool one_kind = (L.twin_hi >> 28) == kind;
+            const bool scanned = kind == K_SPHERE || kind == K_CUBE || kind == K_AABB || kind == K_TRI || (kind == K_RECT && last < rect.size());
+            if (one_kind && scanned) L.color.w = bits_f(1u);
+        }
 
     }
     int build_scene_tree() {
@@ -1593,6 +1604,7 @@
         v.hdri_w = s->hdri_w;
         v.hdri_h = s->hdri_h;
         s->prims_per_ray = sph.size() + cub.size() + pln.size() + tri.size() + aabb.size() + rect.size() + (has_shell ? 1 : 0);
+        s->light_records = lights;
         s->twins_scanned = true;
         s->n_twin_lights = 0;
         for (const Light& L : lights) {
@@ -2749,6 +2761,61 @@
     HIP_TRY(hipMemcpy(t_limit, d_t.get(), n * 4, hipMemcpyDeviceToHost));
     return RPT_OK;
 }
+int rpt_debug_shadow_test(rpt_scene* s, uint32_t light, uint64_t n, const float* origins, const float* dirs, const float* dist,
+                          int32_t* out_flag, float* out_t) {
+    if (!s || !origins || !dirs || !dist || !out_flag || !out_t) return fail(RPT_ERR_INVALID, "null argument");
+    if (rpti::light_kind(s, light) != int(L_OBJECT)) return fail(RPT_ERR_INVALID, "rpt_debug_shadow_test: not a Light::Object");
+    if (!s->committed) return fail(RPT_ERR_STATE, "rpt_scene_commit must be called first");
+    if (s->dev.arena64) return fail(RPT_ERR_STATE, "rpt_debug_shadow_test: the scene was committed with epsilon_policy = 1");
+    if (s->view.n_nodes != 0 || s->view.scene_bvh || s->view.n_inst)
+        return fail(RPT_ERR_UNSUPPORTED, "rpt_debug_shadow_test: the scene has a tree (the query is the linear scan's)");
+    if (!launch_debug_shadow_test) return fail(RPT_ERR_UNSUPPORTED, "rpt_debug_shadow_test: built without the kernels");
+    if (n == 0) return RPT_OK;
+    HIP_TRY(hipSetDevice(s->device));
+    rpti::DevMem d_in, d_out;
+    HIP_TRY(hook_scratch(d_in, n * 28));
+    HIP_TRY(hook_scratch(d_out, n * 8));
+    float* const in = d_in.get<float>();
+    HIP_TRY(hipMemcpy(in, origins, n * 12, hipMemcpyHostToDevice));
+    HIP_TRY(hipMemcpy(in + 3 * n, dirs, n * 12, hipMemcpyHostToDevice));
+    HIP_TRY(hipMemcpy(in + 6 * n, dist, n * 4, hipMemcpyHostToDevice));
+    ShadowTestArgs q{};
+    q.light = light;
+    q.n = n;
+    q.o = in; q.d = in + 3 * n; q.dist = in + 6 * n;
+    q.flag = d_out.get<int32_t>();
+    q.t = d_out.get<float>() + n;
+    HIP_TRY(launch_debug_shadow_test(s->view, q, nullptr));
+    HIP_TRY(hipMemcpy(out_flag, q.flag, n * 4, hipMemcpyDeviceToHost));
+    HIP_TRY(hipMemcpy(out_t, q.t, n * 4, hipMemcpyDeviceToHost));
+    return RPT_OK;
+}
+int rpt_shadow_scan_info(rpt_scene* s, uint32_t light, uint32_t out[4]) {
+    if (!s || !out) return fail(RPT_ERR_INVALID, "null argument");
+    if (rpti::light_kind(s, light) != int(L_OBJECT)) return fail(RPT_ERR_INVALID, "rpt_shadow_scan_info: not a Light::Object");
+    if (!s->committed) return fail(RPT_ERR_STATE, "rpt_scene_commit must be called first");
+    if (s->dev.arena64) return fail(RPT_ERR_STATE, "rpt_shadow_scan_info: the scene was committed with epsilon_policy = 1");
+    if (light >= s->light_records.size()) return fail(RPT_ERR_STATE, "rpt_shadow_scan_info: the light was added after the commit");
+    const Light& L = s->light_records[light];
+    out[0] = L.twin_lo;
+    out[1] = L.twin_hi;
+    out[2] = (bits_u(L.color.w) != 0u && bvh_mode(s->view) == 0) ? 1u : 0u;
+    out[3] = uint32_t(L.twin_object);
+    return RPT_OK;
+}
+int rpt_debug_distance_pair(float sigma_t, uint32_t k0, uint32_t n, float* out_new, float* out_guarded) {
+    if (!out_new || !out_guarded) return fail(RPT_ERR_INVALID, "null argument");
+    if (!(sigma_t > 0.f) || !(sigma_t < INFINITY)) return fail(RPT_ERR_INVALID, "rpt_debug_distance_pair: sigma_t must be positive and finite");
+    if (k0 >= (1u << 23) || n > (1u << 23) - k0) return fail(RPT_ERR_INVALID, "rpt_debug_distance_pair: a draw has 23 bits (k0 + n <= 2^23)");
+    if (!launch_debug_distance_pair) return fail(RPT_ERR_UNSUPPORTED, "rpt_debug_distance_pair: built without the kernels");
+    if (n == 0) return RPT_OK;
+    rpti::DevMem d_out;
+    HIP_TRY(hook_scratch(d_out, size_t(n) * 8));
+    HIP_TRY(launch_debug_distance_pair(sigma_t, k0, n, d_out.get<float>(), d_out.get<float>() + n, nullptr));
+    HIP_TRY(hipMemcpy(out_new, d_out.get<float>(), size_t(n) * 4, hipMemcpyDeviceToHost));
+    HIP_TRY(hipMemcpy(out_guarded, d_out.get<float>() + n, size_t(n) * 4, hipMemcpyDeviceToHost));
+    return RPT_OK;
+}
 
 int rpt_debug_bounce(const rpt_material* m, uint32_t max_bounces, uint32_t depth, int32_t in_medium, int32_t medium_event,
                      float albedo_med, const float* medium_color, uint64_t n, const float* normals, const float* rds, uint64_t seed,
```
